# Eric-qi/RDO-PTQ

Measured on AMD Instinct MI355X. Metric: calibration images/sec (Cheng2020 W8A8 task-oriented RDO-PTQ, image-iterations over all units), higher is better.
Workload: dtype f32

## Files before the change

include/rdo_ptq_hip.h:

```cpp
#ifndef RDO_PTQ_HIP_H
#define RDO_PTQ_HIP_H

#include <stdint.h>

#ifdef __cplusplus
extern "C" {
#endif

#define RDO_OK 0
#define RDO_EINVAL (-22)
#define RDO_EHIP (-5)
#define RDO_ENOMEM (-12)

#define RDO_LOG_SLOTS 32

enum {
    RDO_EPI_NONE = 0,
    RDO_EPI_LRELU = 1,
    RDO_EPI_LRELU_BWD = 2,
    RDO_EPI_GDN = 3,
    RDO_EPI_IGDN = 4,
    RDO_EPI_RELU = 5,
    RDO_EPI_RELU_BWD = 6,
    RDO_EPI_GELU = 7,
    RDO_EPI_GELU_BWD = 8
};

typedef struct rdo_conv_desc {
    int32_t B, H, W, Cin;
    int32_t Ho, Wo, Cout;
    int32_t KH, KW, stride, pad;
    int32_t epilogue;
    int32_t square_input;
    int32_t add_residual;
} rdo_conv_desc;

const char* rdo_version(void);
const char* rdo_last_error(void);
int rdo_set_tuning(const char* key, int32_t value);
int rdo_get_tuning(const char* key);

int rdo_conv2d_fwd(const rdo_conv_desc* d, const float* x, const float* w, const float* bias, const float* aux,
                   const float* residual, float* out, float* pre, float* workspace, int64_t workspace_floats,
                   const void* wplanes , void* stream);
int rdo_conv2d_fwd_ksplit(const rdo_conv_desc* d, int has_planes, int64_t workspace_floats);
int rdo_conv2d_fwd_partials(const rdo_conv_desc* d, const float* x, const float* w, const void* wplanes ,
                            float* workspace, int64_t workspace_floats, void* stream);
int rdo_conv2d_fwd_uses_bf16x6(const rdo_conv_desc* d);
int rdo_split_bf16x3_conv(const float* w, int32_t Cout, int32_t KH, int32_t KW, int32_t Cin, void* planes ,
                          void* stream);
int rdo_split_bf16x3(const float* w, int64_t n, void* planes , void* stream);
int rdo_conv2d_fwd_bf16x6(const rdo_conv_desc* d, const float* x, const void* wplanes, const float* bias, const float* aux,
                          const float* residual, float* out, float* pre, float* workspace, int64_t workspace_floats, void* stream);
int rdo_conv2d_fwd_bf16x6_ksplit(const rdo_conv_desc* d);
int64_t rdo_conv2d_fwd_workspace(const rdo_conv_desc* d);

int rdo_conv2d_wgrad_nsplit(const rdo_conv_desc* d);
int rdo_conv2d_wgrad(const rdo_conv_desc* d, const float* x, const float* dy, float* slabs, int nsplit, void* stream);
int rdo_conv2d_wgrad_uses_bf16x6(const rdo_conv_desc* d);
int rdo_reduce_slabs(const float* slabs, int nsplit, int64_t numel, float* out, void* stream);

typedef struct rdo_ada_desc {
    int64_t numel;
    int32_t rows;
    int32_t n_levels;
    int32_t reparam;
    float reparam_bound, reparam_pedestal;
    int32_t KH, KW, Cin;
} rdo_ada_desc;

int rdo_adaround_init_alpha(const rdo_ada_desc* d, const float* w, const float* delta, float* alpha, void* stream);

int rdo_adaround_fwd(const rdo_ada_desc* d, const float* w, const float* alpha, const float* delta, const float* zp,
                     int soft, float* wq, float* wd, void* stream);

typedef struct rdo_sched_row {
    float b;
    float round_on;
    float step_size;
    float bc2_sqrt;
} rdo_sched_row;

int rdo_adaround_step(const rdo_ada_desc* d, const float* w, const float* delta, const float* zp, const float* slabs,
                      int nsplit, float grad_scale, float round_weight, const rdo_sched_row* sched, const int32_t* iter_ptr,
                      float* alpha, float* adam_m, float* adam_v, float* wq, float* wd, float* round_loss_out,
                      void* wq_planes, void* wd_planes, float wq_plane_scale, float wd_plane_scale, void* stream);

typedef struct rdo_ada_step_item {
    rdo_ada_desc d;
    const float *w, *delta, *zp, *slabs ;
    int32_t nsplit;
    float *alpha, *adam_m, *adam_v, *wq, *wd ;
    void *wq_planes , *wd_planes ;
    float* dalpha;
    float wq_plane_scale, wd_plane_scale;
    void *lin_fwd_planes, *lin_bwd_planes;
    float lin_plane_scale;
} rdo_ada_step_item;
int rdo_adaround_step_batch(const rdo_ada_step_item* items, int32_t n, int32_t mode, float grad_scale, float round_weight,
                            const rdo_sched_row* sched, const int32_t* iter_ptr, float* round_loss_out, int32_t* advance_iter,
                            int32_t* iter_shadow ,
                            void* stream);

typedef struct rdo_gather_desc {
    const float *cache_q, *cache_fp;
    const int32_t* idx_table;
    int32_t n_iters, B, batch_offset;
    int64_t per_image;
    int32_t C;
    float prob;
    uint32_t seed;
    float* out;
    void* out_planes;
    float out_scale;
    int32_t* overflow_flag;
} rdo_gather_desc;
int rdo_adaround_step_batch_gather(const rdo_ada_step_item* items, int32_t n, int32_t mode , float grad_scale, float round_weight,
                                   const rdo_sched_row* sched, const int32_t* iter_ptr, float* round_loss_out, int32_t* iter_shadow,
                                   const rdo_gather_desc* next, void* stream);
int rdo_iter_bind_publish(int32_t* publish);

int rdo_unit1x1_supported(int64_t M, int32_t K, int32_t N);
int rdo_unit1x1_nslab(int64_t M, int32_t N);
int rdo_unit1x1_form(int32_t form);
int rdo_unit1x1(const float* x, int64_t M, int32_t K, int32_t N, const float* w, const float* bias, const float* tgt_cache,
                const int32_t* idx_table, const int32_t* iter_ptr, int32_t B, float coef, int32_t act ,
                float* slabs, int32_t nslab, float* loss_out, void* stream);

int rdo_adaround_grad(const rdo_ada_desc* d, const float* w, const float* alpha, const float* delta, const float* zp,
                      const float* slabs, int nsplit, float* dalpha, void* stream);
int rdo_adaround_apply(const rdo_ada_desc* d, const float* w, const float* delta, const float* zp, const float* dalpha,
                       float grad_scale, float round_weight, const rdo_sched_row* sched, const int32_t* iter_ptr,
                       float* alpha, float* adam_m, float* adam_v, float* wq, float* wd, float* round_loss_out,
                       void* wq_planes, void* wd_planes, float wq_plane_scale, float wd_plane_scale, void* stream);

int rdo_uaq_fakequant(const rdo_ada_desc* d, const float* w, const float* delta, const float* zp, float* wq, float* wd,
                      void* stream);
int rdo_uaq_init_minmax(const float* w, int32_t rows, int64_t inner, int32_t n_levels, float* delta, float* zp,
                        void* stream);

int rdo_actquant_perchannel(const float* x, int64_t npix, int32_t C, int32_t n_bits, float* out,
                            float* ws_minmax , void* stream);
int64_t rdo_actquant_workspace(int32_t C);
int rdo_actquant_static(const float* x, int64_t npix, int32_t C, int32_t n_bits, const float* range , float* out,
                        void* stream);
int rdo_actquant_observe(const float* ws_minmax, int32_t C, float* range , void* stream);
int rdo_actquant_search(const float* x, int64_t npix, int32_t C, int32_t n_bits, const float* range ,
                        float* err , float* ws ,
                        void* stream);
int64_t rdo_actquant_search_workspace(int32_t C);
int rdo_actquant_static_bwd(const float* x, const float* g, int64_t npix, int32_t C, int32_t n_bits, const float* range ,
                            float* dx, float* drange ,
                            float* ws , void* stream);
int64_t rdo_actquant_static_bwd_workspace(int32_t C);
int rdo_act_range_step(float* range , const float* grad , const float* obs ,
                       float* m, float* v, int32_t C, int32_t step, float lr, void* stream);

int rdo_gather_qdrop(const float* cache_q, const float* cache_fp, const int32_t* idx_table, const int32_t* iter_ptr,
                     int32_t B, int32_t batch_offset, int64_t per_image, float prob, uint32_t seed, float* out,
                     int32_t* iter_publish , void* stream);

int rdo_lp2_loss_grad(const float* pred, const float* tgt_cache, const int32_t* idx_table, const int32_t* iter_ptr,
                      int32_t B, int64_t per_image, int32_t C, float coef, float* grad, float* loss_out, void* stream);

int rdo_lp_loss_grad(const float* pred, const float* tgt_cache, const int32_t* idx_table, const int32_t* iter_ptr,
                     int32_t B, int64_t per_image, int32_t C, float coef2, float coefp, float p, float* grad,
                     float* loss_out, float* loss_out_p, void* stream);

int rdo_lrelu_fwd(const float* x, int64_t n, float* out, void* stream);
int rdo_lrelu_bwd(const float* g, const float* y, int64_t n, float* out, void* stream);
int rdo_relu_fwd(const float* x, int64_t n, float* out, void* stream);
int rdo_relu_bwd(const float* g, const float* y, int64_t n, float* out, void* stream);
int rdo_pixel_shuffle(const float* x, int32_t B, int32_t H, int32_t W, int32_t C, int32_t r, int32_t inverse, float* out,
                      void* stream);
int rdo_add(const float* a, const float* b, int64_t n, float* out, void* stream);
int rdo_gdn_bwd_t(const float* g, const float* x, const float* norm, int64_t n, int32_t inverse, float* t, void* stream);
int rdo_gdn_bwd_dx(const float* g, const float* x, const float* norm, const float* acc, int64_t n, int32_t inverse,
                   float* dx, void* stream);
int rdo_nchw_to_nhwc(const float* x, int32_t B, int32_t C, int32_t H, int32_t W, int32_t inverse, float* out, void* stream);
int rdo_iter_advance(int32_t* iter_ptr, void* stream);
int rdo_zero_insert(const float* x, int32_t B, int32_t H, int32_t W, int32_t C, int32_t stride, int32_t pad_top, int32_t pad_left,
                    int32_t Ho, int32_t Wo, float* out, void* stream);
int rdo_tconv_expand(const float* w, const int32_t* map, int32_t Cout, int32_t taps, int32_t Cin, int32_t S2, int32_t KK2, float* wphase,
                     void* stream);
int rdo_tconv_fold(const float* slabs_phase, const int32_t* inv, int32_t nsplit, int32_t Cout, int32_t taps, int32_t Cin, int32_t S2,
                   int32_t KK2, float* slabs, void* stream);
int rdo_layer_norm(const float* x, const float* weight, const float* bias, int64_t rows, int32_t C, float eps, float* out,
                   void* stream);

typedef struct rdo_attn_desc {
    int32_t B, H, W, C;
    int32_t heads;
    int32_t window;
    int32_t shift;
    float scale;
} rdo_attn_desc;
int rdo_window_attention_fwd(const rdo_attn_desc* d, const float* qkv, const float* bias, float* out, float* probs, void* stream);
int rdo_window_attention_pv(const rdo_attn_desc* d, const float* qkv, const float* probs, float* out, void* stream);
int rdo_window_attention_bwd(const rdo_attn_desc* d, const float* qkv, const float* bias, const float* dout, float* dqkv, void* stream);
int rdo_layer_norm_bwd(const float* x, const float* gamma, const float* dy, int64_t rows, int32_t C, float eps, float* dx,
                       float* dgamma_slabs, int32_t nslabs, void* stream);
int rdo_add_layer_norm(const float* a, const float* b, const float* weight, const float* bias, int64_t rows, int32_t C, float eps,
                       float* sum_out, float* out, void* stream);
int rdo_layer_norm_bwd_add(const float* x, const float* gamma, const float* dy, const float* add1, const float* add2, int64_t rows,
                           int32_t C, float eps, float* dx, float* dgamma_slabs, int32_t nslabs, void* stream);
int rdo_add3(const float* a, const float* b, const float* c, int64_t n, float* out, void* stream);
int rdo_linear_h2_supported(int64_t M, int32_t K, int32_t N);
int rdo_split_h2_linear(const float* w, int32_t N, int32_t K, float scale, void* planes, void* stream);
int rdo_linear_h2(const float* x, int64_t M, int32_t K, int32_t N, const void* wplanes, float wscale, const float* bias,
                  int32_t square_input , float* out, void* stream);
int rdo_linear_h2_epi(const float* x, int64_t M, int32_t K, int32_t N, const void* wplanes, float wscale, const float* bias,
                      int32_t square_input, int32_t epilogue, float* pre, const float* aux, float* out, void* stream);
int rdo_gelu_fwd(const float* x, int64_t n, float* out, void* stream);
int rdo_gelu_bwd(const float* dy, const float* x, int64_t n, float* dx, void* stream);
int rdo_round(const float* x, int64_t n, float* out, void* stream);

int rdo_factorized_likelihood_fwd(const float* z, const float* params, const float* medians, int64_t n, int32_t C, float* zhat,
                                  float* lik, void* stream);
int rdo_factorized_likelihood_bwd(const float* zhat, const float* params, int64_t n, int32_t C, float grad_scale, float* dz, void* stream);
int rdo_gaussian_likelihood_fwd(const float* y, const float* scales, const float* means , int64_t n,
                                float scale_bound, float* yhat , float* lik, void* stream);
int rdo_gaussian_likelihood_bwd(const float* yhat, const float* scales, const float* means, int64_t n, float scale_bound,
                                float grad_scale, float* dscales, float* dmeans, void* stream);
int rdo_neg_log2_sum(const float* lik, int64_t n, float scale, float* out , void* stream);
int rdo_sq_diff_sum(const float* a, const float* b, int64_t n, float scale, int32_t clamp01_a, float* out ,
                    void* stream);
int rdo_neg_log2_sum_ordered(const float* lik, int64_t n, float scale, float* out , float* ws, void* stream);
int rdo_sq_diff_sum_ordered(const float* a, const float* b, int64_t n, float scale, int32_t clamp01_a, float* out , float* ws,
                            void* stream);
int64_t rdo_ordered_sum_workspace(void);

int rdo_h2_overflow(int reset);
int rdo_h2_bind_flag(int32_t* flag);
int rdo_split_h2(const float* x, int64_t npix, int32_t C, float scale, void* planes , void* stream);
int rdo_split_h2_conv(const float* w, int32_t Cout, int32_t KH, int32_t KW, int32_t Cin, float scale, void* planes ,
                      void* stream);
int rdo_conv2d_fwd_h2_supported(const rdo_conv_desc* d);
int64_t rdo_conv2d_fwd_h2_workspace(const rdo_conv_desc* d);
int rdo_conv2d_fwd_h2(const rdo_conv_desc* d, const void* x_planes, float x_scale, const void* wplanes, float w_scale, const float* bias,
                      const float* aux,
                      const void* aux_planes ,
                      const float* residual, float* out, float* pre, void* out_planes, float out_scale, float* workspace,
                      int64_t workspace_floats, void* stream);
int rdo_conv2d_fwd_h2_tail_supported(const rdo_conv_desc* d);
int rdo_conv2d_fwd_h2_tail(const rdo_conv_desc* d, const void* x_planes, float x_scale, const void* wplanes, float w_scale,
                           const float* bias, const void* residual_planes , float residual_scale, const float* tgt_cache,
                           const int32_t* idx_table, const int32_t* iter_ptr, int32_t B, float coef, int32_t act, void* dpre_planes,
                           float dpre_scale, float* loss_out, void* stream);
int rdo_conv2d_wgrad_h2_supported(const rdo_conv_desc* d);
int rdo_conv2d_wgrad_h2_layer_supported(const rdo_conv_desc* d);
int rdo_conv2d_wgrad_h2(const rdo_conv_desc* d, const void* x_planes, float x_scale, const void* dy_planes, float dy_scale, float* slabs,
                        int nsplit, void* stream);
int rdo_gather_qdrop_h2(const float* cache_q, const float* cache_fp, const int32_t* idx_table, const int32_t* iter_ptr, int32_t B,
                        int32_t batch_offset, int64_t per_image, int32_t C, float prob, uint32_t seed, float* out, void* out_planes,
                        float out_scale, int32_t* iter_publish, void* stream);
int rdo_loss_act_bwd(const float* pre, const float* residual, const void* residual_planes ,
                     float residual_scale, const float* tgt_cache, const int32_t* idx_table, const int32_t* iter_ptr, int32_t B,
                     int64_t per_image, int32_t C, float coef, int32_t act, float* out, float* grad_out, float* dpre, void* dpre_planes,
                     float dpre_scale, float* loss_out, void* stream);
int rdo_loss_act_bwd_splitk(const float* partial, int32_t ksplit, const float* bias , const float* residual,
                            const float* tgt_cache, const int32_t* idx_table, const int32_t* iter_ptr, int32_t B, int64_t per_image,
                            int32_t C, float coef, int32_t act, float* out, float* grad_out, float* dpre, float* loss_out, void* stream);
int rdo_loss_gdn_bwd(const float* x, const float* norm, const float* residual, const float* tgt_cache, const int32_t* idx_table,
                     const int32_t* iter_ptr, int32_t B, int64_t per_image, int32_t C, float coef, int32_t inverse, float* out,
                     float* grad_out, float* t, void* t_planes, float t_scale, float* loss_out, void* stream);
int rdo_gdn_bwd_dx_h2(const float* g, const float* x, const float* norm, const float* acc, int64_t n, int32_t C, int32_t inverse,
                      float* dx, void* dx_planes, float dx_scale, void* stream);
int rdo_pixel_shuffle_h2(const float* x, int32_t B, int32_t H, int32_t W, int32_t C, float* out, void* out_planes, float out_scale,
                         void* stream);
int rdo_pixel_unshuffle2(const float* x, int32_t B, int32_t H, int32_t W, int32_t C, float* out, void* out_planes, float out_scale,
                         void* stream);

typedef struct rdo_plan rdo_plan;
// ... 24 lines not shown
```

rdo-ptq_amd/csrc/adaround.hip:

```cpp
#include "rdo_common.h"
#include "gather_body.h"

namespace {

typedef float f32x4 __attribute__((ext_vector_type(4)));

constexpr float kGamma = -0.1f, kZeta = 1.1f;
constexpr float kBeta1 = 0.9f, kBeta2 = 0.999f, kAdamEps = 1e-8f;

__device__ __forceinline__ float sigmoidf_(float a) { return 1.0f / (1.0f + __expf(-a)); }

__device__ __forceinline__ float pow_u(float u, float p) {
    return (u > 0.f) ? __builtin_amdgcn_exp2f(__builtin_amdgcn_logf(u) * p) : 0.f;
}

struct AdaArgs {
    rdo_ada_desc d;
    const float* w;
    const float* delta;
    const float* zp;
    const float* slabs;
    int nsplit;
    const float* dalpha_in;
    float* dalpha_out;
// ... 110 lines not shown
                s += 4;
            }
            for (; s < a.nsplit; ++s) g4 += *reinterpret_cast<const vec_t*>(sp + (long)s * d.numel);
        }
        vec_t m4 = wv4 * 0.f, v4 = m4, o4 = m4;
        if (a.mode != 1 && !ADA_ABL(8)) {
            m4 = *reinterpret_cast<const vec_t*>(a.m + e0);
            v4 = *reinterpret_cast<const vec_t*>(a.v + e0);
        }
        int rows[W];
        if (inner >= W && d.numel < (1L << 31)) {
            const unsigned row0 = (unsigned)e0 / (unsigned)inner;
            const unsigned rem0 = (unsigned)e0 - row0 * (unsigned)inner;
#pragma unroll
            for (int k = 0; k < W; ++k) rows[k] = (int)(row0 + (rem0 + k >= (unsigned)inner ? 1u : 0u));
        } else {
#pragma unroll
            for (int k = 0; k < W; ++k) rows[k] = (int)((e0 + k) / inner);
        }
#pragma unroll
        for (int k = 0; k < W; ++k) {
            const int row = rows[k];
            const float dl = a.delta[row], z = a.zp[row], wv = wv4[k];
            float al = al4[k];
            const float xf = floorf(wv / dl);
            const float sg = sigmoidf_(al);
            const float hraw = sg * (kZeta - kGamma) + kGamma;
            const float h = fminf(fmaxf(hraw, 0.f), 1.f);
            const float xint = xf + h + z;
            const float pass_h = (hraw >= 0.f && hraw <= 1.f) ? 1.f : 0.f;
            const float dh_da = pass_h * ((kZeta - kGamma) * (sg * (1.f - sg)));
            float g_alpha = g4[k];
            if (a.mode != 2) {
                float g = g4[k];
                if (d.reparam) {
                    const float q = (fminf(fmaxf(xint, 0.f), Lm1) - z) * dl;
                    const float lb = fmaxf(q, d.reparam_bound);
                    const float go = g * (2.f * lb);
                    g = (q >= d.reparam_bound || go < 0.f) ? go : 0.f;
                }
                const float pass_q = (xint >= 0.f && xint <= Lm1) ? 1.f : 0.f;
                g_alpha = (g * dl) * pass_q * dh_da;
            }
            if (a.mode == 1) {
                o4[k] = g_alpha;
                continue;
            }
            float g_total = g_alpha * a.grad_scale;
            if (round_on != 0.f && !ADA_ABL(4)) {
                const float u = fabsf(h - 0.5f) * 2.f;
                const float ub1 = pow_u(u, b - 1.f);
                rl_local += a.round_weight * (1.f - u * ub1);
                const float sgn = (h > 0.5f) ? 1.f : ((h < 0.5f) ? -1.f : 0.f);
                g_total += (-a.round_weight * (b * ub1) * 2.f * sgn) * dh_da;
            }
            float mm = m4[k], vv = v4[k];
            mm = mm + (g_total - mm) * (1.f - kBeta1);
            vv = vv * kBeta2 + (1.f - kBeta2) * g_total * g_total;
            const float denom = sqrtf(vv) / bc2 + kAdamEps;
            al = al - step_size * (mm / denom);
            m4[k] = mm; v4[k] = vv; al4[k] = al;
            const float sg2 = sigmoidf_(al);
            const float h2 = fminf(fmaxf(sg2 * (kZeta - kGamma) + kGamma, 0.f), 1.f);
            float o = (fminf(fmaxf(xf + h2 + z, 0.f), Lm1) - z) * dl;
            if (d.reparam) {
                const float lb = fmaxf(o, d.reparam_bound);
                o = lb * lb - d.reparam_pedestal;
            }
            o4[k] = o;
        }
        if (a.mode == 1) {
            *reinterpret_cast<vec_t*>(a.dalpha_out + e0) = o4;
        } else {
            if (!ADA_ABL(8)) {
                *reinterpret_cast<vec_t*>(a.m + e0) = m4;
                *reinterpret_cast<vec_t*>(a.v + e0) = v4;
            }
            *reinterpret_cast<vec_t*>(a.alpha + e0) = al4;
            if (!ADA_ABL(32)) *reinterpret_cast<vec_t*>(a.wq + e0) = o4;
            if (ADA_ABL(2)) continue;
            if (a.lin_fwd || a.lin_bwd) {
                const int in_ = (int)inner, nr = d.rows;
                const long plane = (long)nr * in_;
                int bad = 0;
#pragma unroll
                for (int k = 0; k < W; ++k) {
                    const int n = rows[k], kk = (int)(e0 + k - (long)n * in_);
                    unsigned short hi, lo;
                    lin_split(o4[k], a.lin_pscale, hi, lo, bad);
                    if (a.lin_fwd) {
                        const long f = lin_frag_index(n, kk, nr >> 4);
                        a.lin_fwd[f] = hi; a.lin_fwd[plane + f] = lo;
                    }
                    if (a.lin_bwd) {
                        const long f = lin_frag_index(kk, n, in_ >> 4);
                        a.lin_bwd[f] = hi; a.lin_bwd[plane + f] = lo;
                    }
                }
                rdo::h2_report(bad, a.ovf);
            }
            if (a.wq_planes && a.wq_pscale > 0.f) {
                int bad = 0;
                if constexpr (W == 4) {
                    typedef unsigned u32x2 __attribute__((ext_vector_type(2)));
                    u32x2 ph, pl;
                    unsigned h, l;
                    rdo::h2_split_pk(o4[0], o4[1], a.wq_pscale, h, l, bad); ph[0] = h; pl[0] = l;
                    rdo::h2_split_pk(o4[2], o4[3], a.wq_pscale, h, l, bad); ph[1] = h; pl[1] = l;
                    const long f0 = d.Cin > 0 ? rdo::frag_index(e0, d.rows, d.KH, d.KW, d.Cin) : e0;
                    *reinterpret_cast<u32x2*>(a.wq_planes + f0) = ph;
                    *reinterpret_cast<u32x2*>(a.wq_planes + d.numel + f0) = pl;
                } else {
#pragma unroll
                    for (int k = 0; k < W; ++k)
                        rdo::h2_split_store(o4[k], a.wq_pscale, a.wq_planes, d.numel,
                                            d.Cin > 0 ? rdo::frag_index(e0 + k, d.rows, d.KH, d.KW, d.Cin) : e0 + k, bad);
                }
                rdo::h2_report(bad, a.ovf);
            } else if (a.wq_planes) {
                if constexpr (W == 4) {
                    typedef unsigned short u16x4 __attribute__((ext_vector_type(4)));
                    u16x4 ph, pm, pl;
#pragma unroll
                    for (int k = 0; k < 4; ++k) {
                        const __bf16 h = (__bf16)o4[k];
                        const float r1 = o4[k] - (float)h;
                        const __bf16 m = (__bf16)r1;
                        const __bf16 l = (__bf16)(r1 - (float)m);
                        ph[k] = __builtin_bit_cast(unsigned short, h);
                        pm[k] = __builtin_bit_cast(unsigned short, m);
                        pl[k] = __builtin_bit_cast(unsigned short, l);
                    }
                    const long f0 = d.Cin > 0 ? rdo::frag_index(e0, d.rows, d.KH, d.KW, d.Cin) : e0;
                    *reinterpret_cast<u16x4*>(a.wq_planes + f0) = ph;
                    *reinterpret_cast<u16x4*>(a.wq_planes + d.numel + f0) = pm;
                    *reinterpret_cast<u16x4*>(a.wq_planes + 2 * d.numel + f0) = pl;
                } else {
#pragma unroll
                    for (int k = 0; k < W; ++k)
                        split3_store(o4[k], a.wq_planes, d.numel, d.Cin > 0 ? rdo::frag_index(e0 + k, d.rows, d.KH, d.KW, d.Cin) : e0 + k);
                }
            }
        }
    }
    if (a.mode != 1 && a.round_loss_out && round_on != 0.f) {
        const float t = rdo::block_sum(rl_local);
        if (threadIdx.x == 0) {
            if (t != 0.f) atomicAdd(a.round_loss_out + (long)it * RDO_LOG_SLOTS + (bid & (RDO_LOG_SLOTS - 1)), t);
        }
    }
}


__device__ __forceinline__ void ada_step_tile_body(const AdaArgs& a, int bid) {
    typedef float vec_t __attribute__((ext_vector_type(4)));
    typedef unsigned u32x2 __attribute__((ext_vector_type(2)));
    typedef unsigned short u16x4 __attribute__((ext_vector_type(4)));
    const rdo_ada_desc d = a.d;
    const int Cin = d.Cin, taps = d.KH * d.KW, nrows = d.rows;
    const int ctiles = (Cin + 31) >> 5;
    const int bid0 = bid;
    const int ct = bid % ctiles; bid /= ctiles;
    const int tap = bid % taps;
    const int rt = bid / taps;
    const int q = threadIdx.x & 7, r = threadIdx.x >> 3;
    const int row = rt * 32 + r, ci = ct * 32 + 4 * q;
    const bool live = row < nrows && ci < Cin;
    const float Lm1 = (float)(d.n_levels - 1);
    const int it = *a.iter_ptr;
    const rdo_sched_row sc = a.sched[it];
    const float b = sc.b, round_on = sc.round_on, step_size = sc.step_size, bc2 = sc.bc2_sqrt;
    float rl_local = 0.f;
    vec_t o4 = {0.f, 0.f, 0.f, 0.f};
    const long e0 = ((long)row * taps + tap) * Cin + ci;
    if (live) {
        const vec_t wv4 = *reinterpret_cast<const vec_t*>(a.w + e0);
        vec_t al4 = *reinterpret_cast<const vec_t*>(a.alpha + e0);
        vec_t g4 = {0.f, 0.f, 0.f, 0.f};
        if (a.mode == 2) {
            g4 = *reinterpret_cast<const vec_t*>(a.dalpha_in + e0);
        } else if (!ADA_ABL(1)) {
            const float* sp = a.slabs + e0;
            int s = 0;
            for (; s + 16 <= a.nsplit; s += 16) {
                vec_t t[16];
#pragma unroll
                for (int u = 0; u < 16; ++u) t[u] = *reinterpret_cast<const vec_t*>(sp + (long)(s + u) * d.numel);
                g4 += (((t[0] + t[1]) + (t[2] + t[3])) + ((t[4] + t[5]) + (t[6] + t[7]))) +
                      (((t[8] + t[9]) + (t[10] + t[11])) + ((t[12] + t[13]) + (t[14] + t[15])));
            }
            for (; s + 8 <= a.nsplit; s += 8) {
                vec_t t[8];
#pragma unroll
                for (int u = 0; u < 8; ++u) t[u] = *reinterpret_cast<const vec_t*>(sp + (long)(s + u) * d.numel);
                g4 += ((t[0] + t[1]) + (t[2] + t[3])) + ((t[4] + t[5]) + (t[6] + t[7]));
            }
            if (s + 4 <= a.nsplit) {
                vec_t t[4];
#pragma unroll
                for (int u = 0; u < 4; ++u) t[u] = *reinterpret_cast<const vec_t*>(sp + (long)(s + u) * d.numel);
                g4 += (t[0] + t[1]) + (t[2] + t[3]);
                s += 4;
            }
            for (; s < a.nsplit; ++s) g4 += *reinterpret_cast<const vec_t*>(sp + (long)s * d.numel);
        }
        vec_t m4 = {0.f, 0.f, 0.f, 0.f}, v4 = m4;
        if (!ADA_ABL(8)) {
            m4 = *reinterpret_cast<const vec_t*>(a.m + e0);
            v4 = *reinterpret_cast<const vec_t*>(a.v + e0);
        }
        const float dl = a.delta[row], z = a.zp[row];
#pragma unroll
        for (int k = 0; k < 4; ++k) {
            float al = al4[k];
            const float xf = floorf(wv4[k] / dl);
            const float sg = sigmoidf_(al);
            const float hraw = sg * (kZeta - kGamma) + kGamma;
            const float h = fminf(fmaxf(hraw, 0.f), 1.f);
            const float xint = xf + h + z;
            const float pass_h = (hraw >= 0.f && hraw <= 1.f) ? 1.f : 0.f;
            const float dh_da = pass_h * ((kZeta - kGamma) * (sg * (1.f - sg)));
            float g_alpha = g4[k];
            if (a.mode != 2) {
                float g = g4[k];
                if (d.reparam) {
                    const float qv = (fminf(fmaxf(xint, 0.f), Lm1) - z) * dl;
                    const float lb = fmaxf(qv, d.reparam_bound);
                    const float go = g * (2.f * lb);
                    g = (qv >= d.reparam_bound || go < 0.f) ? go : 0.f;
                }
                const float pass_q = (xint >= 0.f && xint <= Lm1) ? 1.f : 0.f;
                g_alpha = (g * dl) * pass_q * dh_da;
            }
            float g_total = g_alpha * a.grad_scale;
            if (round_on != 0.f && !ADA_ABL(4)) {
                const float u = fabsf(h - 0.5f) * 2.f;
                const float ub1 = pow_u(u, b - 1.f);
                rl_local += a.round_weight * (1.f - u * ub1);
                const float sgn = (h > 0.5f) ? 1.f : ((h < 0.5f) ? -1.f : 0.f);
                g_total += (-a.round_weight * (b * ub1) * 2.f * sgn) * dh_da;
            }
            float mm = m4[k], vv = v4[k];
            mm = mm + (g_total - mm) * (1.f - kBeta1);
            vv = vv * kBeta2 + (1.f - kBeta2) * g_total * g_total;
            const float denom = sqrtf(vv) / bc2 + kAdamEps;
            al = al - step_size * (mm / denom);
            m4[k] = mm; v4[k] = vv; al4[k] = al;
            const float sg2 = sigmoidf_(al);
            const float h2 = fminf(fmaxf(sg2 * (kZeta - kGamma) + kGamma, 0.f), 1.f);
            float o = (fminf(fmaxf(xf + h2 + z, 0.f), Lm1) - z) * dl;
            if (d.reparam) {
                const float lb = fmaxf(o, d.reparam_bound);
                o = lb * lb - d.reparam_pedestal;
            }
            o4[k] = o;
        }
        if (!ADA_ABL(8)) {
            *reinterpret_cast<vec_t*>(a.m + e0) = m4;
            *reinterpret_cast<vec_t*>(a.v + e0) = v4;
        }
        *reinterpret_cast<vec_t*>(a.alpha + e0) = al4;
        if (!ADA_ABL(32)) *reinterpret_cast<vec_t*>(a.wq + e0) = o4;
        if (!ADA_ABL(2)) {
            int bad = 0;
            if (a.lin_fwd) {
                unsigned hh, ll;
                u32x2 ph, pl;
                rdo::h2_split_pk(o4[0], o4[1], a.lin_pscale, hh, ll, bad); ph[0] = hh; pl[0] = ll;
                rdo::h2_split_pk(o4[2], o4[3], a.lin_pscale, hh, ll, bad); ph[1] = hh; pl[1] = ll;
                const long f = lin_frag_index(row, ci, nrows >> 4);
                *reinterpret_cast<u32x2*>(a.lin_fwd + f) = ph;
                *reinterpret_cast<u32x2*>(a.lin_fwd + (long)nrows * Cin + f) = pl;
            }
            if (a.wq_planes) {
                const long f0 = (Cin & 15) ? e0 : (((((long)(ci >> 4) * taps + tap) * nrows + row) << 4) + (ci & 15));
                if (a.wq_pscale > 0.f) {
                    unsigned hh, ll;
                    u32x2 ph, pl;
                    rdo::h2_split_pk(o4[0], o4[1], a.wq_pscale, hh, ll, bad); ph[0] = hh; pl[0] = ll;
                    rdo::h2_split_pk(o4[2], o4[3], a.wq_pscale, hh, ll, bad); ph[1] = hh; pl[1] = ll;
                    *reinterpret_cast<u32x2*>(a.wq_planes + f0) = ph;
                    *reinterpret_cast<u32x2*>(a.wq_planes + d.numel + f0) = pl;
                } else {
                    u16x4 ph, pm, pl;
#pragma unroll
                    for (int k = 0; k < 4; ++k) {
                        const __bf16 hb = (__bf16)o4[k];
                        const float r1 = o4[k] - (float)hb;
                        const __bf16 mb = (__bf16)r1;
                        const __bf16 lb = (__bf16)(r1 - (float)mb);
                        ph[k] = __builtin_bit_cast(unsigned short, hb);
                        pm[k] = __builtin_bit_cast(unsigned short, mb);
                        pl[k] = __builtin_bit_cast(unsigned short, lb);
                    }
                    *reinterpret_cast<u16x4*>(a.wq_planes + f0) = ph;
                    *reinterpret_cast<u16x4*>(a.wq_planes + d.numel + f0) = pm;
                    *reinterpret_cast<u16x4*>(a.wq_planes + 2 * d.numel + f0) = pl;
                }
            }
            rdo::h2_report(bad, a.ovf);
        }
    }
    __shared__ float tile[32][33];
    if ((a.wd || a.lin_bwd) && !ADA_ABL(16)) {
#pragma unroll
        for (int k = 0; k < 4; ++k) tile[r][4 * q + k] = o4[k];
        __syncthreads();
        const int ci2 = ct * 32 + r, co2 = rt * 32 + 4 * q;
        if (ci2 < Cin && co2 < nrows) {
            vec_t t4;
#pragma unroll
            for (int k = 0; k < 4; ++k) t4[k] = tile[4 * q + k][r];
            const int kh = tap / d.KW, kw = tap - kh * d.KW;
            const int tapf = (d.KH - 1 - kh) * d.KW + (d.KW - 1 - kw);
            const long o = ((long)ci2 * taps + tapf) * nrows + co2;
            if (a.wd) *reinterpret_cast<vec_t*>(a.wd + o) = t4;
            int bad = 0;
            if (a.lin_bwd && !ADA_ABL(2)) {
                unsigned hh, ll;
                u32x2 ph, pl;
                rdo::h2_split_pk(t4[0], t4[1], a.lin_pscale, hh, ll, bad); ph[0] = hh; pl[0] = ll;
                rdo::h2_split_pk(t4[2], t4[3], a.lin_pscale, hh, ll, bad); ph[1] = hh; pl[1] = ll;
                const long f = lin_frag_index(ci2, co2, Cin >> 4);
                *reinterpret_cast<u32x2*>(a.lin_bwd + f) = ph;
                *reinterpret_cast<u32x2*>(a.lin_bwd + (long)nrows * Cin + f) = pl;
            }
            if (a.wd && a.wd_planes && !ADA_ABL(2)) {
                const long f0 = (nrows & 15) ? o : (((((long)(co2 >> 4) * taps + tapf) * Cin + ci2) << 4) + (co2 & 15));
                if (a.wd_pscale > 0.f) {
                    unsigned hh, ll;
                    u32x2 ph, pl;
                    rdo::h2_split_pk(t4[0], t4[1], a.wd_pscale, hh, ll, bad); ph[0] = hh; pl[0] = ll;
                    rdo::h2_split_pk(t4[2], t4[3], a.wd_pscale, hh, ll, bad); ph[1] = hh; pl[1] = ll;
                    *reinterpret_cast<u32x2*>(a.wd_planes + f0) = ph;
                    *reinterpret_cast<u32x2*>(a.wd_planes + d.numel + f0) = pl;
                } else {
                    u16x4 ph, pm, pl;
#pragma unroll
                    for (int k = 0; k < 4; ++k) {
                        const __bf16 hb = (__bf16)t4[k];
                        const float r1 = t4[k] - (float)hb;
                        const __bf16 mb = (__bf16)r1;
                        const __bf16 lb = (__bf16)(r1 - (float)mb);
                        ph[k] = __builtin_bit_cast(unsigned short, hb);
                        pm[k] = __builtin_bit_cast(unsigned short, mb);
                        pl[k] = __builtin_bit_cast(unsigned short, lb);
                    }
                    *reinterpret_cast<u16x4*>(a.wd_planes + f0) = ph;
                    *reinterpret_cast<u16x4*>(a.wd_planes + d.numel + f0) = pm;
                    *reinterpret_cast<u16x4*>(a.wd_planes + 2 * d.numel + f0) = pl;
                }
            }
            rdo::h2_report(bad, a.ovf);
        }
    }
    if (a.round_loss_out && round_on != 0.f) {
        const float t = rdo::block_sum(rl_local);
        if (threadIdx.x == 0) {
            if (t != 0.f) atomicAdd(a.round_loss_out + (long)it * RDO_LOG_SLOTS + (bid0 & (RDO_LOG_SLOTS - 1)), t);
        }
    }
}

inline bool tile_ok(const rdo_ada_desc& d, int mode) {
    return mode != 1 && d.Cin > 0 && d.Cin % 4 == 0 && d.rows % 4 == 0 && (long)d.rows * d.KH * d.KW * d.Cin == d.numel && d.numel < (1L << 31);
}
inline long tile_blocks(const rdo_ada_desc& d) { return rdo::ceil_div(d.rows, 32) * d.KH * d.KW * rdo::ceil_div(d.Cin, 32); }

template <int W>
__global__ __launch_bounds__(256) void ada_step_kernel(AdaArgs a) {
    ada_step_body<W>(a, blockIdx.x, gridDim.x);
}

constexpr int kMaxBatch = 8;
struct AdaBatch {
    int w1_min;
    int32_t* iter_shadow;
    AdaArgs a[kMaxBatch];
    int blk_end[kMaxBatch];
    unsigned char tile[kMaxBatch];
    int n;
    int gather_beg;
    rdo::gq::Gather g;
};
__global__ __launch_bounds__(256) void ada_step_batch_kernel(AdaBatch b) {
    if (b.iter_shadow && blockIdx.x == 0 && threadIdx.x == 0) *b.iter_shadow = *b.a[0].iter_ptr + 1;
    if ((int)blockIdx.x >= b.gather_beg) {
        const int it1 = *b.a[0].iter_ptr + 1;
        if (it1 < b.g.n_iters) {
            if (b.g.planes.p) rdo::gq::gather_h2_body(b.g, it1, (long)blockIdx.x - b.gather_beg, (long)gridDim.x - b.gather_beg);
            else rdo::gq::gather_fp32_body(b.g, it1, (long)blockIdx.x - b.gather_beg, (long)gridDim.x - b.gather_beg);
        }
        return;
    }
    int t = 0;
    while (t + 1 < b.n && (int)blockIdx.x >= b.blk_end[t]) ++t;
    const int beg = t ? b.blk_end[t - 1] : 0;
    if (b.tile[t]) { ada_step_tile_body(b.a[t], (int)blockIdx.x - beg); return; }
    if (b.a[t].nsplit >= b.w1_min && b.a[t].mode != 2) ada_step_body<1>(b.a[t], (long)blockIdx.x - beg, (long)b.blk_end[t] - beg);
    else ada_step_body<4>(b.a[t], (long)blockIdx.x - beg, (long)b.blk_end[t] - beg);
}

__device__ __forceinline__ void wd_transpose_body(const rdo_ada_desc& d, const float* wq, float* wd, unsigned short* wd_planes, float pscale,
                                                  int* ovf, int bid) {
    const int taps = d.KH * d.KW, cdim = d.Cin;
    const int ctiles = (cdim + 31) / 32;
    const int ct = bid % ctiles; bid /= ctiles;
    const int tap = bid % taps;
    const int rt = bid / taps;
    const int tx = threadIdx.x & 31, ty = threadIdx.x >> 5;
    __shared__ float tile[32][33];
#pragma unroll
    for (int k = 0; k < 4; ++k) {
        const int row = rt * 32 + ty + 8 * k, c = ct * 32 + tx;
        if (row < d.rows && c < cdim) tile[ty + 8 * k][tx] = wq[((long)row * taps + tap) * cdim + c];
    }
    __syncthreads();
    const int kh = tap / d.KW, kw = tap - kh * d.KW;
    const int tapf = (d.KH - 1 - kh) * d.KW + (d.KW - 1 - kw);
#pragma unroll
    for (int k = 0; k < 4; ++k) {
        const int ci = ct * 32 + ty + 8 * k, co = rt * 32 + tx;
        if (ci < cdim && co < d.rows) {
            const long o = ((long)ci * taps + tapf) * d.rows + co;
            wd[o] = tile[tx][ty + 8 * k];
            if (wd_planes && pscale > 0.f) {
                int bad = 0;
                rdo::h2_split_store(tile[tx][ty + 8 * k], pscale, wd_planes, d.numel, rdo::frag_index(o, d.Cin, d.KH, d.KW, d.rows), bad);
                rdo::h2_report(bad, ovf);
            } else if (wd_planes) {
                split3_store(tile[tx][ty + 8 * k], wd_planes, d.numel, rdo::frag_index(o, d.Cin, d.KH, d.KW, d.rows));
            }
        }
    }
}
__global__ __launch_bounds__(256) void wd_transpose_kernel(rdo_ada_desc d, const float* wq, float* wd, unsigned short* wd_planes, float pscale,
                                                           int* ovf) {
    wd_transpose_body(d, wq, wd, wd_planes, pscale, ovf, blockIdx.x);
}
__global__ __launch_bounds__(256) void wd_transpose_batch_kernel(AdaBatch b, int32_t* advance) {
    int t = 0;
    while (t + 1 < b.n && (int)blockIdx.x >= b.blk_end[t]) ++t;
    const int beg = t ? b.blk_end[t - 1] : 0;
    if (!ADA_ABL(16)) wd_transpose_body(b.a[t].d, b.a[t].wq, b.a[t].wd, b.a[t].wd_planes, b.a[t].wd_pscale, b.a[t].ovf, (int)blockIdx.x - beg);
    if (advance && blockIdx.x == 0 && threadIdx.x == 0) *advance += 1;
}

__global__ void iter_advance1_kernel(int32_t* it) { *it += 1; }

__global__ __launch_bounds__(256) void ada_fwd_kernel(rdo_ada_desc d, const float* w, const float* alpha, const float* delta,
                                                      const float* zp, int mode , float* wq,
                                                      float* wd) {
    const long inner = d.numel / d.rows;
    const float Lm1 = (float)(d.n_levels - 1);
    for (long e = (long)blockIdx.x * blockDim.x + threadIdx.x; e < d.numel; e += (long)gridDim.x * blockDim.x) {
        const int row = (int)(e / inner);
        const float dl = delta[row], z = zp[row], wv = w[e];
        float xint;
        if (mode == 2) {
            xint = rintf(wv / dl) + z;
        } else {
            const float xf = floorf(wv / dl);
            float h;
            if (mode == 1) {
                h = fminf(fmaxf(sigmoidf_(alpha[e]) * (kZeta - kGamma) + kGamma, 0.f), 1.f);
            } else {
                h = alpha[e] >= 0.f ? 1.f : 0.f;
            }
            xint = xf + h + z;
        }
        emit(d, e, (fminf(fmaxf(xint, 0.f), Lm1) - z) * dl, wq, wd);
    }
}

__global__ __launch_bounds__(256) void ada_init_kernel(rdo_ada_desc d, const float* w, const float* delta, float* alpha) {
    const long inner = d.numel / d.rows;
    for (long e = (long)blockIdx.x * blockDim.x + threadIdx.x; e < d.numel; e += (long)gridDim.x * blockDim.x) {
        const float dl = delta[e / inner];
        const float r = w[e] / dl;
        const float rest = r - floorf(r);
        alpha[e] = -logf((kZeta - kGamma) / (rest - kGamma) - 1.f);
    }
}

__global__ __launch_bounds__(256) void uaq_minmax_kernel(const float* w, long inner, int n_levels, float* delta, float* zp) {
    const float* p = w + (long)blockIdx.x * inner;
    float mn = 0.f, mx = 0.f;
    for (long i = threadIdx.x; i < inner; i += blockDim.x) {
        const float v = p[i];
        mn = fminf(mn, v);
        mx = fmaxf(mx, v);
    }
    for (int o = 32; o > 0; o >>= 1) {
        mn = fminf(mn, __shfl_down(mn, o, 64));
        mx = fmaxf(mx, __shfl_down(mx, o, 64));
    }
    __shared__ float smn[4], smx[4];
    if ((threadIdx.x & 63) == 0) { smn[threadIdx.x >> 6] = mn; smx[threadIdx.x >> 6] = mx; }
    __syncthreads();
    if (threadIdx.x == 0) {
        mn = fminf(fminf(smn[0], smn[1]), fminf(smn[2], smn[3]));
        mx = fmaxf(fmaxf(smx[0], smx[1]), fmaxf(smx[2], smx[3]));
        float dl = (float)(((double)mx - (double)mn) / (double)(n_levels - 1));
        dl = fmaxf(dl, 1e-8f);
        delta[blockIdx.x] = dl;
        zp[blockIdx.x] = rintf(__fmul_rn(__frcp_rn(dl), -mn));
    }
}

__global__ __launch_bounds__(256) void reduce_slabs_kernel(const float* slabs, int nsplit, long numel, float* out) {
    for (long e = (long)blockIdx.x * blockDim.x + threadIdx.x; e < numel; e += (long)gridDim.x * blockDim.x) {
        float g = 0.f;
        for (int s = 0; s < nsplit; ++s) g += slabs[(long)s * numel + e];
        out[e] = g;
    }
}

using rdo::grid_for;

int check_desc(const rdo_ada_desc* d, const char* who) {
    RDO_REQUIRE(d != nullptr, "%s: null descriptor", who);
    RDO_REQUIRE(d->numel > 0 && d->rows > 0 && d->numel % d->rows == 0, "%s: numel %ld not divisible by rows %d", who,
                (long)d->numel, d->rows);
    RDO_REQUIRE(d->n_levels >= 4 && d->n_levels <= 65536, "%s: n_levels %d unsupported", who, d->n_levels);
    if (d->Cin > 0)
        RDO_REQUIRE(d->KH > 0 && d->KW > 0 && (long)d->rows * d->KH * d->KW * d->Cin == d->numel,
                    "%s: conv layout [%d][%d][%d][%d] does not match numel %ld", who, d->rows, d->KH, d->KW, d->Cin,
                    (long)d->numel);
    return RDO_OK;
}

int run_step(AdaArgs a, void* stream) {

    return rdo::dispatch(
        [a](hipStream_t s) {
            if (a.d.numel % 4 == 0)
                hipLaunchKernelGGL(ada_step_kernel<4>, dim3(grid_for(a.d.numel / 4)), dim3(256), 0, s, a);
            else
                hipLaunchKernelGGL(ada_step_kernel<1>, dim3(grid_for(a.d.numel)), dim3(256), 0, s, a);
            if (a.mode != 1 && a.wd && a.d.Cin > 0) {
                const long blocks = rdo::ceil_div(a.d.rows, 32) * a.d.KH * a.d.KW * rdo::ceil_div(a.d.Cin, 32);
                hipLaunchKernelGGL(wd_transpose_kernel, dim3((unsigned)blocks), dim3(256), 0, s, a.d, (const float*)a.wq, a.wd, a.wd_planes, a.wd_pscale,
                                   a.ovf);
            }
            return rdo::check_launch("ada_step");
        },
        stream, "ada_step", 0.0, 4.0 * a.d.numel * ((a.mode == 2 ? 1 : a.nsplit) + 9.0));
}

}

extern "C" {

#ifdef RDO_DIAG
int rdo_diag_ada_ablate(int mask) {
    return hipMemcpyToSymbol(HIP_SYMBOL(g_ada_abl), &mask, sizeof mask) == hipSuccess ? RDO_OK : rdo::set_error(RDO_EHIP, "rdo_diag_ada_ablate");
}
#endif

int rdo_adaround_init_alpha(const rdo_ada_desc* d, const float* w, const float* delta, float* alpha, void* stream) {
    if (int rc = check_desc(d, "rdo_adaround_init_alpha")) return rc;
    RDO_REQUIRE(w && delta && alpha, "rdo_adaround_init_alpha: null pointer");
    const rdo_ada_desc dd = *d;
    return rdo::dispatch(
        [=](hipStream_t s) {
            hipLaunchKernelGGL(ada_init_kernel, dim3(grid_for(dd.numel)), dim3(256), 0, s, dd, w, delta, alpha);
            return rdo::check_launch("ada_init");
        },
        stream);
}

int rdo_adaround_fwd(const rdo_ada_desc* d, const float* w, const float* alpha, const float* delta, const float* zp, int soft,
                     float* wq, float* wd, void* stream) {
    if (int rc = check_desc(d, "rdo_adaround_fwd")) return rc;
    RDO_REQUIRE(w && alpha && delta && zp && wq, "rdo_adaround_fwd: null pointer");
    const rdo_ada_desc dd = *d;
    const int mode = soft ? 1 : 0;
    return rdo::dispatch(
        [=](hipStream_t s) {
            hipLaunchKernelGGL(ada_fwd_kernel, dim3(grid_for(dd.numel)), dim3(256), 0, s, dd, w, alpha, delta, zp, mode, wq, wd);
            return rdo::check_launch("ada_fwd");
        },
        stream);
}

int rdo_uaq_fakequant(const rdo_ada_desc* d, const float* w, const float* delta, const float* zp, float* wq, float* wd,
                      void* stream) {
    if (int rc = check_desc(d, "rdo_uaq_fakequant")) return rc;
    RDO_REQUIRE(w && delta && zp && wq, "rdo_uaq_fakequant: null pointer");
    const rdo_ada_desc dd = *d;
    return rdo::dispatch(
        [=](hipStream_t s) {
            hipLaunchKernelGGL(ada_fwd_kernel, dim3(grid_for(dd.numel)), dim3(256), 0, s, dd, w, (const float*)nullptr, delta, zp,
                               2, wq, wd);
            return rdo::check_launch("uaq_fakequant");
        },
        stream);
}

int rdo_uaq_init_minmax(const float* w, int32_t rows, int64_t inner, int32_t n_levels, float* delta, float* zp, void* stream) {
    RDO_REQUIRE(w && delta && zp && rows > 0 && inner > 0 && n_levels >= 4, "rdo_uaq_init_minmax: bad argument");
    return rdo::dispatch(
        [=](hipStream_t s) {
            hipLaunchKernelGGL(uaq_minmax_kernel, dim3(rows), dim3(256), 0, s, w, (long)inner, n_levels, delta, zp);
            return rdo::check_launch("uaq_minmax");
        },
        stream);
}

int rdo_reduce_slabs(const float* slabs, int nsplit, int64_t numel, float* out, void* stream) {
    RDO_REQUIRE(slabs && out && nsplit >= 1 && numel > 0, "rdo_reduce_slabs: bad argument");
    return rdo::dispatch(
        [=](hipStream_t s) {
            hipLaunchKernelGGL(reduce_slabs_kernel, dim3(grid_for(numel)), dim3(256), 0, s, slabs, nsplit, (long)numel, out);
            return rdo::check_launch("reduce_slabs");
        },
        stream);
}

int rdo_adaround_step(const rdo_ada_desc* d, const float* w, const float* delta, const float* zp, const float* slabs, int nsplit,
                      float grad_scale, float round_weight, const rdo_sched_row* sched, const int32_t* iter_ptr, float* alpha,
                      float* adam_m, float* adam_v, float* wq, float* wd, float* round_loss_out, void* wq_planes, void* wd_planes,
                      float wq_plane_scale, float wd_plane_scale, void* stream) {
    if (int rc = check_desc(d, "rdo_adaround_step")) return rc;
    RDO_REQUIRE(w && delta && zp && slabs && nsplit >= 1 && sched && iter_ptr && alpha && adam_m && adam_v && wq,
                "rdo_adaround_step: null pointer");
    AdaArgs a{};
    a.d = *d; a.w = w; a.delta = delta; a.zp = zp; a.slabs = slabs; a.nsplit = nsplit; a.grad_scale = grad_scale;
    a.round_weight = round_weight; a.sched = sched; a.iter_ptr = iter_ptr; a.alpha = alpha; a.m = adam_m; a.v = adam_v;
    a.wq = wq; a.wd = wd; a.round_loss_out = round_loss_out; a.mode = 0;
    a.wq_planes = static_cast<unsigned short*>(wq_planes);
    a.wd_planes = wd ? static_cast<unsigned short*>(wd_planes) : nullptr;
    a.wq_pscale = wq_plane_scale; a.wd_pscale = wd_plane_scale; a.ovf = rdo::h2_overflow_flag();
    return run_step(a, stream);
}

static int step_batch_impl(const rdo_ada_step_item* items, int32_t n, int32_t mode, float grad_scale, float round_weight,
                           const rdo_sched_row* sched, const int32_t* iter_ptr, float* round_loss_out, int32_t* advance_iter,
                           int32_t* iter_shadow, const rdo_gather_desc* next, void* stream) {
    RDO_REQUIRE(items && n >= 1 && n <= kMaxBatch, "rdo_adaround_step_batch: bad argument (1 <= n <= %d)", kMaxBatch);
    RDO_REQUIRE(mode >= 0 && mode <= 2, "rdo_adaround_step_batch: mode %d (0 fused step, 1 gradient only, 2 apply)", mode);
    RDO_REQUIRE(mode == 1 || (sched && iter_ptr), "rdo_adaround_step_batch: schedule / iteration counter missing");
    RDO_REQUIRE(!(advance_iter && iter_shadow), "rdo_adaround_step_batch: advance_iter and iter_shadow are alternatives");
    RDO_REQUIRE(!iter_shadow || iter_ptr, "rdo_adaround_step_batch: iter_shadow needs iter_ptr");
    AdaBatch b{}, bw{};
    const int w1_min = rdo::tuning(rdo::T_ADA_W1_MIN);
    b.w1_min = bw.w1_min = w1_min;
    int blocks = 0, wblocks = 0;
    double bytes = 0.0;
    for (int i = 0; i < n; ++i) {
        const rdo_ada_step_item& it = items[i];
        if (int rc = check_desc(&it.d, "rdo_adaround_step_batch")) return rc;
        RDO_REQUIRE(it.d.numel % 4 == 0, "rdo_adaround_step_batch: numel %ld of item %d is not a multiple of 4", (long)it.d.numel, i);
        RDO_REQUIRE(it.w && it.delta && it.zp && it.alpha, "rdo_adaround_step_batch: null pointer in item %d", i);
        RDO_REQUIRE(mode == 2 || (it.slabs && it.nsplit >= 1), "rdo_adaround_step_batch: item %d has no gradient slabs", i);
        RDO_REQUIRE(mode == 0 || it.dalpha, "rdo_adaround_step_batch: item %d has no dalpha buffer", i);
        RDO_REQUIRE(mode == 1 || (it.adam_m && it.adam_v && it.wq), "rdo_adaround_step_batch: null optimiser state in item %d", i);
        AdaArgs& a = b.a[i];
        a.d = it.d; a.w = it.w; a.delta = it.delta; a.zp = it.zp; a.slabs = it.slabs; a.nsplit = it.nsplit;
        a.dalpha_in = it.dalpha; a.dalpha_out = it.dalpha;
        a.grad_scale = grad_scale; a.round_weight = round_weight; a.sched = sched; a.iter_ptr = iter_ptr;
        a.alpha = it.alpha; a.m = it.adam_m; a.v = it.adam_v; a.wq = it.wq; a.wd = it.wd; a.round_loss_out = round_loss_out; a.mode = mode;
        a.wq_planes = static_cast<unsigned short*>(it.wq_planes);
        a.wd_planes = it.wd ? static_cast<unsigned short*>(it.wd_planes) : nullptr;
        a.wq_pscale = it.wq_plane_scale; a.wd_pscale = it.wd_plane_scale; a.ovf = rdo::h2_overflow_flag();
        if (mode != 1 && (it.lin_fwd_planes || it.lin_bwd_planes)) {
            RDO_REQUIRE(it.d.rows % 32 == 0 && (it.d.numel / it.d.rows) % 32 == 0 && it.lin_plane_scale > 0.f,
                        "rdo_adaround_step_batch: item %d: Linear planes need rows and inner in blocks of 32 and a positive scale", i);
            a.lin_fwd = static_cast<unsigned short*>(it.lin_fwd_planes);
            a.lin_bwd = static_cast<unsigned short*>(it.lin_bwd_planes);
            a.lin_pscale = it.lin_plane_scale;
        }
        b.tile[i] = tile_ok(it.d, mode) ? 1 : 0;
        blocks += b.tile[i] ? (int)tile_blocks(it.d) : (int)grid_for((it.nsplit >= w1_min && mode != 2) ? it.d.numel : it.d.numel / 4);
        b.blk_end[i] = blocks;
        bytes += 4.0 * it.d.numel * ((mode == 2 ? 1 : it.nsplit) + (mode == 1 ? 3.0 : 9.0));
        if (mode != 1 && it.wd && it.d.Cin > 0 && !b.tile[i]) {
            bw.a[bw.n] = a;
            wblocks += (int)(rdo::ceil_div(it.d.rows, 32) * it.d.KH * it.d.KW * rdo::ceil_div(it.d.Cin, 32));
            bw.blk_end[bw.n++] = wblocks;
        }
    }
    b.n = n;
    b.iter_shadow = iter_shadow;
    b.gather_beg = blocks;
    if (next) {
        RDO_REQUIRE(mode != 1 && iter_ptr, "rdo_adaround_step_batch_gather: the gather rides on a fused step or an apply launch");
        RDO_REQUIRE(next->cache_q && next->cache_fp && next->idx_table && (next->out || next->out_planes) && next->n_iters > 0,
                    "rdo_adaround_step_batch_gather: null pointer in the gather descriptor");
        RDO_REQUIRE(next->B > 0 && next->batch_offset >= 0 && next->per_image > 0 && next->per_image % 4 == 0 &&
                    (long)(next->batch_offset + next->B) * next->per_image < (1L << 32), "rdo_adaround_step_batch_gather: bad gather shape");
        RDO_REQUIRE(!next->out_planes || (next->C > 0 && next->C % 16 == 0 && next->per_image % next->C == 0 && next->out_scale > 0.f),
                    "rdo_adaround_step_batch_gather: the plane form needs C %% 16 == 0 and a positive power-of-two scale");
        RDO_REQUIRE(next->out_planes || next->out, "rdo_adaround_step_batch_gather: no destination");
        RDO_REQUIRE(next->prob >= 0.f && next->prob <= 1.f, "rdo_adaround_step_batch_gather: prob out of [0,1]");
        const double t = floor((double)next->prob * 4294967296.0);
        const unsigned long long thr = (unsigned long long)(t > 4294967296.0 ? 4294967296.0 : t);
        b.g = rdo::gq::Gather{next->cache_q, next->cache_fp, next->idx_table, next->n_iters, next->B, next->batch_offset, (long)next->per_image,
                              next->C, thr, next->seed, next->out,
                              rdo::gq::H2Out{static_cast<unsigned short*>(next->out_planes), next->out_scale,
                                             next->overflow_flag ? reinterpret_cast<int*>(next->overflow_flag) : rdo::h2_overflow_flag()}};
        long gb = rdo::gq::gather_blocks(b.g);
        const long cap = b.g.planes.p ? 8192 : 2048;
        blocks += (int)(gb > cap ? cap : gb);
        bytes += (8.0 + (next->out ? 4.0 : 0.0) + (next->out_planes ? 4.0 : 0.0)) * next->B * (double)next->per_image;
    }
    const char* tag = next ? "ada_step_gather" : "ada_step";
    return rdo::dispatch(
        [=](hipStream_t s) {
            hipLaunchKernelGGL(ada_step_batch_kernel, dim3((unsigned)blocks), dim3(256), 0, s, b);
            if (bw.n > 0)
                hipLaunchKernelGGL(wd_transpose_batch_kernel, dim3((unsigned)wblocks), dim3(256), 0, s, bw, advance_iter);
            else if (advance_iter)
                hipLaunchKernelGGL(iter_advance1_kernel, dim3(1), dim3(1), 0, s, advance_iter);
            return rdo::check_launch("ada_step_batch");
        },
        stream, tag, 0.0, bytes);
}

int rdo_adaround_step_batch(const rdo_ada_step_item* items, int32_t n, int32_t mode, float grad_scale, float round_weight,
                            const rdo_sched_row* sched, const int32_t* iter_ptr, float* round_loss_out, int32_t* advance_iter,
                            int32_t* iter_shadow, void* stream) {
    return step_batch_impl(items, n, mode, grad_scale, round_weight, sched, iter_ptr, round_loss_out, advance_iter, iter_shadow, nullptr, stream);
}

int rdo_adaround_step_batch_gather(const rdo_ada_step_item* items, int32_t n, int32_t mode, float grad_scale, float round_weight,
                                   const rdo_sched_row* sched, const int32_t* iter_ptr, float* round_loss_out, int32_t* iter_shadow,
                                   const rdo_gather_desc* next, void* stream) {
    RDO_REQUIRE(next != nullptr, "rdo_adaround_step_batch_gather: null gather descriptor");
    return step_batch_impl(items, n, mode, grad_scale, round_weight, sched, iter_ptr, round_loss_out, nullptr, iter_shadow, next, stream);
}

int rdo_adaround_grad(const rdo_ada_desc* d, const float* w, const float* alpha, const float* delta, const float* zp,
                      const float* slabs, int nsplit, float* dalpha, void* stream) {
    if (int rc = check_desc(d, "rdo_adaround_grad")) return rc;
    RDO_REQUIRE(w && alpha && delta && zp && slabs && nsplit >= 1 && dalpha, "rdo_adaround_grad: null pointer");
    AdaArgs a{};
    a.d = *d; a.w = w; a.delta = delta; a.zp = zp; a.slabs = slabs; a.nsplit = nsplit; a.alpha = const_cast<float*>(alpha);
    a.dalpha_out = dalpha; a.mode = 1;
    return run_step(a, stream);
}

int rdo_adaround_apply(const rdo_ada_desc* d, const float* w, const float* delta, const float* zp, const float* dalpha,
                       float grad_scale, float round_weight, const rdo_sched_row* sched, const int32_t* iter_ptr, float* alpha,
                       float* adam_m, float* adam_v, float* wq, float* wd, float* round_loss_out, void* wq_planes, void* wd_planes,
                       float wq_plane_scale, float wd_plane_scale, void* stream) {
    if (int rc = check_desc(d, "rdo_adaround_apply")) return rc;
    RDO_REQUIRE(w && delta && zp && dalpha && sched && iter_ptr && alpha && adam_m && adam_v && wq,
                "rdo_adaround_apply: null pointer");
    AdaArgs a{};
    a.d = *d; a.w = w; a.delta = delta; a.zp = zp; a.dalpha_in = dalpha; a.grad_scale = grad_scale;
    a.round_weight = round_weight; a.sched = sched; a.iter_ptr = iter_ptr; a.alpha = alpha; a.m = adam_m; a.v = adam_v;
    a.wq = wq; a.wd = wd; a.round_loss_out = round_loss_out; a.mode = 2;
    a.wq_planes = static_cast<unsigned short*>(wq_planes);
    a.wd_planes = wd ? static_cast<unsigned short*>(wd_planes) : nullptr;
    a.wq_pscale = wq_plane_scale; a.wd_pscale = wd_plane_scale; a.ovf = rdo::h2_overflow_flag();
    return run_step(a, stream);
}

}
```

rdo-ptq_amd/csrc/conv_wgrad.hip:

```cpp
#include <utility>

#include "rdo_common.h"

namespace {

typedef float f32x16 __attribute__((ext_vector_type(16)));
typedef float f32x4 __attribute__((ext_vector_type(4)));

constexpr int PK = 32;

struct WgArgs {
    const float* x;
    const float* dy;
    float* slabs;
    int B, H, W, Cin, Ho, Wo, Cout, KH, KW, stride, pad;
    int M, mchunk, nsplit;
    int tiles_co, tiles_ci;
    int square_input;
};

template <int TCO, int TCI, bool VEC>
__global__ __launch_bounds__(256) void conv_wgrad_kernel(WgArgs a) {
    constexpr int WCO = TCO / 2, WCI = TCI / 2;
    constexpr int TM = WCO / 32, TN = WCI / 32;
// ... 84 lines not shown
            if (a.square_input) v = v * v;
            *reinterpret_cast<f32x4*>(Xs + buf * PK * TCI + srow * TCI + 4 * (sq + 8 * (j - YQ))) = v;
        }
    };
    auto for_each_quad = [&](auto&& f) {
        [&]<int... J>(std::integer_sequence<int, J...>) { (f(std::integral_constant<int, J>{}), ...); }
        (std::make_integer_sequence<int, NQ>{});
    };

    if (nsteps > 0) {
        decode(0);
        for_each_quad([&](auto jc) { load_quad(jc); });
        for_each_quad([&](auto jc) { store_quad(jc, 0); });
        decode(nsteps > 1 ? 1 : 0);
        for_each_quad([&](auto jc) { load_quad(jc); });
    }
    __syncthreads();

    for (int s = 0; s < nsteps; ++s) {
        const int buf = s & 1;
        const float* Y = Ys + buf * PK * TCO;
        const float* X = Xs + buf * PK * TCI;
        float fa[2][TM], fb[2][TN];
        auto read_frags = [&](int kk, int set) {
            const int prow = 2 * kk + lh;
#pragma unroll
            for (int i = 0; i < TM; ++i) fa[set][i] = Y[prow * TCO + wco0 + i * 32 + li];
#pragma unroll
            for (int j = 0; j < TN; ++j) fb[set][j] = X[prow * TCI + wci0 + j * 32 + li];
        };
        read_frags(0, 0);
        decode(s + 2 < nsteps ? s + 2 : nsteps - 1);
        [&]<int... SL>(std::integer_sequence<int, SL...>) {
            (([&] {
                 if constexpr (SL + 1 < PK / 2) read_frags(SL + 1, (SL + 1) & 1);
#pragma unroll
                 for (int i = 0; i < TM; ++i)
#pragma unroll
                     for (int j = 0; j < TN; ++j)
                         acc[i][j] = __builtin_amdgcn_mfma_f32_32x32x2f32(fa[SL & 1][i], fb[SL & 1][j], acc[i][j], 0, 0, 0);
                 if constexpr (SL < NQ) {
                     store_quad(std::integral_constant<int, SL>{}, buf ^ 1);
                     load_quad(std::integral_constant<int, SL>{});
                 }
                 __builtin_amdgcn_sched_barrier(0);
             }()),
             ...);
        }
        (std::make_integer_sequence<int, PK / 2>{});
        __syncthreads();
    }

    const long wsize = (long)a.Cout * a.KH * a.KW * a.Cin;
    float* slab = a.slabs + (long)chunk * wsize;
    const int taps = a.KH * a.KW;
#pragma unroll
    for (int j = 0; j < TN; ++j) {
        const int ci = ci0 + wci0 + j * 32 + li;
        if (ci >= a.Cin) continue;
#pragma unroll
        for (int i = 0; i < TM; ++i)
#pragma unroll
            for (int r = 0; r < 16; ++r) {
                const int co = co0 + wco0 + i * 32 + (r & 3) + 8 * (r >> 2) + 4 * lh;
                if (co < a.Cout) slab[((long)co * taps + tap) * a.Cin + ci] = acc[i][j][r];
            }
    }
}

template <int TCO, int TCI, bool VEC>
int launch(WgArgs a, hipStream_t s) {
    constexpr size_t lds = (size_t)2 * PK * (TCO + TCI) * sizeof(float);
    auto kern = conv_wgrad_kernel<TCO, TCI, VEC>;
    static rdo::PerDevice attr_set;
    if (!attr_set.done()) {
        if (hipFuncSetAttribute(reinterpret_cast<const void*>(kern), hipFuncAttributeMaxDynamicSharedMemorySize, (int)lds) !=
            hipSuccess)
            return rdo::set_error(RDO_EHIP, "hipFuncSetAttribute(conv_wgrad, %zu B LDS) failed", lds);
        attr_set.mark();
    }
    a.tiles_co = (int)rdo::ceil_div(a.Cout, TCO);
    a.tiles_ci = (int)rdo::ceil_div(a.Cin, TCI);
    dim3 grid((unsigned)a.nsplit, (unsigned)(a.KH * a.KW * a.tiles_co * a.tiles_ci));
    hipLaunchKernelGGL(kern, grid, dim3(256), lds, s, a);
    return rdo::check_launch("conv_wgrad");
}

int g_force_big = -1, g_force_ns = -1;

inline bool one_tile_many_pixels(const rdo_conv_desc* d) {
    return d->KH == 1 && d->KW == 1 && d->Cout >= 160 && d->Cout <= 192 && d->Cin >= 160 && d->Cin <= 192 &&
           (long)d->B * d->Ho * d->Wo >= 16384;
}

inline bool big_tiles(const rdo_conv_desc* d) {
    if (g_force_big >= 0) return g_force_big != 0;
    const long M = (long)d->B * d->Ho * d->Wo;
    const long big_tiles_total = (long)d->KH * d->KW * rdo::ceil_div(d->Cout, 192) * rdo::ceil_div(d->Cin, 192);
    const long min_m = big_tiles_total >= 32 ? 1024 : 4096;
    if (d->Cout >= 160 && d->Cin >= 160 && M >= min_m && big_tiles_total >= 3) return true;
    if (d->Cout >= 160 && d->Cin >= 160 && M >= 16384 && big_tiles_total == 2) return true;
    return one_tile_many_pixels(d);
}

inline int tiles_total(const rdo_conv_desc* d) {
    const int t = big_tiles(d) ? 192 : 64;
    return d->KH * d->KW * (int)rdo::ceil_div(d->Cout, t) * (int)rdo::ceil_div(d->Cin, t);
}

}

int rdo_launch_wgrad_x6(const rdo_conv_desc* d, const float* x, const float* dy, float* slabs, int nsplit, int mchunk, hipStream_t s);
bool rdo_linear_wgrad_h2_ok(const rdo_conv_desc* d, const float* x, const float* dy);
int rdo_launch_linear_wgrad_h2(const rdo_conv_desc* d, const float* x, const float* dy, float* slabs, int nsplit, int mchunk, hipStream_t s);
bool rdo_conv_is_thin(const rdo_conv_desc* d, bool forward);
int rdo_launch_thin_wgrad(const rdo_conv_desc* d, const float* x, const float* dy, float* slabs, int nsplit, hipStream_t s);
bool rdo_conv_is_thincout(const rdo_conv_desc* d, bool forward);
int rdo_thincout_patches(const rdo_conv_desc* d);
int rdo_launch_thincout_wgrad(const rdo_conv_desc* d, const float* x, const float* dy, float* slabs, hipStream_t s);

extern "C" int rdo_conv2d_wgrad_uses_bf16x6(const rdo_conv_desc* d) {
    const bool enabled = rdo::tuning(rdo::T_CONV_X6) != 0;
    if (!d || !enabled || g_force_big == 0) return 0;
    const bool fits = (double)d->B * d->H * d->W * d->Cin * 4.0 < 4.0e9 && (double)d->B * d->Ho * d->Wo * d->Cout * 4.0 < 4.0e9;
    return big_tiles(d) && fits && d->Wo % 4 == 0 && d->Wo >= 16 && d->Cin % 4 == 0 && d->Cout % 4 == 0;
}

extern "C" void rdo_debug_force_wgrad_choice(int big, int nsplit) {
    g_force_big = big;
    g_force_ns = nsplit;
}

extern "C" int rdo_conv2d_wgrad_nsplit(const rdo_conv_desc* d) {
    if (!d) return 1;
    if (g_force_big < 0 && rdo_conv_is_thincout(d, false)) return rdo_thincout_patches(d);
    if (g_force_ns >= 1) return g_force_ns;
    const long M = (long)d->B * d->Ho * d->Wo;
    if (rdo_conv_is_thin(d, false)) {
        const long per = d->KH * d->KW * d->Cin > 4 ? 256 : 512;
        const long cap = d->KH * d->KW * d->Cin > 4 ? 256 : 128;
        const long ns = M / per;
        return (int)(ns < 1 ? 1 : (ns > cap ? cap : ns));
    }
    const long target = big_tiles(d) ? 256 : 1024;
    long ns = target / tiles_total(d);
    const long max_by_m = rdo::ceil_div(M, 128);
    if (ns > max_by_m) ns = max_by_m;
    if (ns < 1) ns = 1;
    const long cap = (g_force_big < 0 && one_tile_many_pixels(d)) ? 256 : ((g_force_big != 0 && rdo_linear_wgrad_h2_ok(d, nullptr, nullptr)) ? 128 : 64);
    if (ns > cap) ns = cap;
    return (int)ns;
}

extern "C" int rdo_conv2d_wgrad(const rdo_conv_desc* d, const float* x, const float* dy, float* slabs, int nsplit,
                                void* stream) {
    RDO_REQUIRE(d && x && dy && slabs, "rdo_conv2d_wgrad: null argument");
    RDO_REQUIRE(nsplit >= 1, "rdo_conv2d_wgrad: nsplit < 1");
    RDO_REQUIRE((long)d->B * d->H * d->W * d->Cin < (1L << 31) && (long)d->B * d->Ho * d->Wo * d->Cout < (1L << 31),
                "rdo_conv2d_wgrad: tensors of 2^31 or more elements are not supported (32-bit staging offsets)");
    WgArgs a;
    a.x = x; a.dy = dy; a.slabs = slabs;
    a.B = d->B; a.H = d->H; a.W = d->W; a.Cin = d->Cin; a.Ho = d->Ho; a.Wo = d->Wo; a.Cout = d->Cout;
    a.KH = d->KH; a.KW = d->KW; a.stride = d->stride; a.pad = d->pad;
    a.M = d->B * d->Ho * d->Wo;
    a.nsplit = nsplit;
    a.mchunk = (int)(rdo::ceil_div(rdo::ceil_div(a.M, nsplit), PK) * PK);
    a.square_input = d->square_input;
    a.tiles_co = a.tiles_ci = 0;
    const bool vec = (d->Cin % 4 == 0) && (d->Cout % 4 == 0) &&
                     ((reinterpret_cast<uintptr_t>(x) | reinterpret_cast<uintptr_t>(dy)) % 16 == 0);
    const bool big = big_tiles(d);
    if (g_force_big < 0 && rdo_conv_is_thincout(d, false) && nsplit == rdo_thincout_patches(d)) {
        const rdo_conv_desc dd = *d;
        return rdo::dispatch([=](hipStream_t s) { return rdo_launch_thincout_wgrad(&dd, x, dy, slabs, s); }, stream, "conv_thincout_wgrad",
                             2.0 * a.M * (double)a.Cout * a.Cin * 9.0,
                             4.0 * ((double)a.B * a.H * a.W * a.Cin + (double)a.M * a.Cout + (double)nsplit * a.Cout * 9.0 * a.Cin));
    }
    if (rdo_conv_is_thin(d, false)) {
        const rdo_conv_desc dd = *d;
        return rdo::dispatch([=](hipStream_t s) { return rdo_launch_thin_wgrad(&dd, x, dy, slabs, nsplit, s); }, stream,
                             "conv_thin_wgrad", 2.0 * a.M * (double)a.Cout * a.Cin * a.KH * a.KW,
                             4.0 * ((double)a.B * a.H * a.W * a.Cin + (double)a.M * a.Cout + (double)nsplit * a.Cout * a.KH * a.KW * a.Cin));
    }
    if (g_force_big != 0 && rdo_linear_wgrad_h2_ok(d, x, dy) && (long)nsplit * a.mchunk >= a.M) {
        const rdo_conv_desc dd = *d;
        const int mchunk = a.mchunk;
        return rdo::dispatch([=](hipStream_t s) { return rdo_launch_linear_wgrad_h2(&dd, x, dy, slabs, nsplit, mchunk, s); }, stream,
                             "linear_wgrad_h2", 2.0 * a.M * (double)a.Cout * a.Cin,
                             4.0 * ((double)a.M * a.Cin + (double)a.M * a.Cout + (double)nsplit * a.Cout * a.Cin));
    }
    if (vec && rdo_conv2d_wgrad_uses_bf16x6(d)) {
        const rdo_conv_desc dd = *d;
        const int mchunk = a.mchunk;
        return rdo::dispatch([=](hipStream_t s) { return rdo_launch_wgrad_x6(&dd, x, dy, slabs, nsplit, mchunk, s); }, stream,
                             "conv_wgrad_x6_192x192", 2.0 * a.M * (double)a.Cout * a.Cin * a.KH * a.KW,
                             4.0 * ((double)a.B * a.H * a.W * a.Cin + (double)a.M * a.Cout + (double)nsplit * a.Cout * a.KH * a.KW * a.Cin));
    }
    return rdo::dispatch(
        [a, vec, big](hipStream_t s) {
            if (big) return vec ? launch<192, 192, true>(a, s) : launch<192, 192, false>(a, s);
            return vec ? launch<64, 64, true>(a, s) : launch<64, 64, false>(a, s);
        },
        stream, big ? "conv_wgrad_192x192" : "conv_wgrad_64x64", 2.0 * a.M * (double)a.Cout * a.Cin * a.KH * a.KW,
        4.0 * ((double)a.B * a.H * a.W * a.Cin + (double)a.M * a.Cout + (double)nsplit * a.Cout * a.KH * a.KW * a.Cin));
}
```

rdo-ptq_amd/hipops/_lib.py:

```python
import ctypes as C
import os

_HERE = os.path.dirname(os.path.abspath(__file__))
LIB_PATH = os.path.join(os.path.dirname(_HERE), "lib", "librdoptq_hip.so")

EPI_NONE, EPI_LRELU, EPI_LRELU_BWD, EPI_GDN, EPI_IGDN, EPI_RELU, EPI_RELU_BWD, EPI_GELU, EPI_GELU_BWD = range(9)
LOG_SLOTS = 32


class ConvDesc(C.Structure):
    _fields_ = [(n, C.c_int32) for n in ("B", "H", "W", "Cin", "Ho", "Wo", "Cout", "KH", "KW", "stride", "pad", "epilogue",
                                         "square_input", "add_residual")]


class AdaDesc(C.Structure):
    _fields_ = [("numel", C.c_int64), ("rows", C.c_int32), ("n_levels", C.c_int32), ("reparam", C.c_int32),
                ("reparam_bound", C.c_float), ("reparam_pedestal", C.c_float), ("KH", C.c_int32), ("KW", C.c_int32),
                ("Cin", C.c_int32)]


class AdaStepItem(C.Structure):
    _fields_ = [("d", AdaDesc), ("w", C.c_void_p), ("delta", C.c_void_p), ("zp", C.c_void_p), ("slabs", C.c_void_p),
                ("nsplit", C.c_int32), ("alpha", C.c_void_p), ("adam_m", C.c_void_p), ("adam_v", C.c_void_p), ("wq", C.c_void_p),
                ("wd", C.c_void_p), ("wq_planes", C.c_void_p), ("wd_planes", C.c_void_p), ("dalpha", C.c_void_p),
                ("wq_plane_scale", C.c_float), ("wd_plane_scale", C.c_float),
                ("lin_fwd_planes", C.c_void_p), ("lin_bwd_planes", C.c_void_p), ("lin_plane_scale", C.c_float)]


class GatherDesc(C.Structure):
    _fields_ = [("cache_q", C.c_void_p), ("cache_fp", C.c_void_p), ("idx_table", C.c_void_p), ("n_iters", C.c_int32), ("B", C.c_int32),
                ("batch_offset", C.c_int32), ("per_image", C.c_int64), ("C", C.c_int32), ("prob", C.c_float), ("seed", C.c_uint32),
                ("out", C.c_void_p), ("out_planes", C.c_void_p), ("out_scale", C.c_float), ("overflow_flag", C.c_void_p)]


class AttnDesc(C.Structure):
    _fields_ = [(n, C.c_int32) for n in ("B", "H", "W", "C", "heads", "window", "shift")] + [("scale", C.c_float)]


class SchedRow(C.Structure):
    _fields_ = [("b", C.c_float), ("round_on", C.c_float), ("step_size", C.c_float), ("bc2_sqrt", C.c_float)]


P = C.c_void_p
_SIGS = {
    "rdo_version": (C.c_char_p, []),
    "rdo_last_error": (C.c_char_p, []),
    "rdo_set_tuning": (C.c_int, [C.c_char_p, C.c_int32]),
    "rdo_get_tuning": (C.c_int, [C.c_char_p]),
    "rdo_conv2d_fwd": (C.c_int, [C.POINTER(ConvDesc), P, P, P, P, P, P, P, P, C.c_int64, P, P]),
    "rdo_conv2d_fwd_uses_bf16x6": (C.c_int, [C.POINTER(ConvDesc)]),
    "rdo_split_bf16x3": (C.c_int, [P, C.c_int64, P, P]),
    "rdo_split_bf16x3_conv": (C.c_int, [P, C.c_int32, C.c_int32, C.c_int32, C.c_int32, P, P]),
    "rdo_conv2d_fwd_bf16x6": (C.c_int, [C.POINTER(ConvDesc), P, P, P, P, P, P, P, P, C.c_int64, P]),
    "rdo_conv2d_fwd_bf16x6_ksplit": (C.c_int, [C.POINTER(ConvDesc)]),
    "rdo_conv2d_fwd_workspace": (C.c_int64, [C.POINTER(ConvDesc)]),
    "rdo_conv2d_wgrad_nsplit": (C.c_int, [C.POINTER(ConvDesc)]),
    "rdo_conv2d_wgrad": (C.c_int, [C.POINTER(ConvDesc), P, P, P, C.c_int, P]),
    "rdo_conv2d_wgrad_uses_bf16x6": (C.c_int, [C.POINTER(ConvDesc)]),
    "rdo_reduce_slabs": (C.c_int, [P, C.c_int, C.c_int64, P, P]),
    "rdo_adaround_init_alpha": (C.c_int, [C.POINTER(AdaDesc), P, P, P, P]),
    "rdo_adaround_fwd": (C.c_int, [C.POINTER(AdaDesc), P, P, P, P, C.c_int, P, P, P]),
    "rdo_adaround_step": (C.c_int, [C.POINTER(AdaDesc), P, P, P, P, C.c_int, C.c_float, C.c_float, P, P, P, P, P, P, P, P, P, P, C.c_float, C.c_float, P]),
    "rdo_adaround_step_batch": (C.c_int, [C.POINTER(AdaStepItem), C.c_int32, C.c_int32, C.c_float, C.c_float, P, P, P, P, P, P]),
    "rdo_adaround_step_batch_gather": (C.c_int, [C.POINTER(AdaStepItem), C.c_int32, C.c_int32, C.c_float, C.c_float, P, P, P, P, C.POINTER(GatherDesc), P]),
    "rdo_iter_bind_publish": (C.c_int, [P]),
    "rdo_unit1x1_supported": (C.c_int, [C.c_int64, C.c_int32, C.c_int32]),
    "rdo_unit1x1_nslab": (C.c_int, [C.c_int64, C.c_int32]),
    "rdo_unit1x1_form": (C.c_int, [C.c_int32]),
    "rdo_unit1x1": (C.c_int, [P, C.c_int64, C.c_int32, C.c_int32, P, P, P, P, P, C.c_int32, C.c_float, C.c_int32, P, C.c_int32, P, P]),
    "rdo_adaround_grad": (C.c_int, [C.POINTER(AdaDesc), P, P, P, P, P, C.c_int, P, P]),
    "rdo_adaround_apply": (C.c_int, [C.POINTER(AdaDesc), P, P, P, P, C.c_float, C.c_float, P, P, P, P, P, P, P, P, P, P, C.c_float, C.c_float, P]),
    "rdo_uaq_fakequant": (C.c_int, [C.POINTER(AdaDesc), P, P, P, P, P, P]),
    "rdo_uaq_init_minmax": (C.c_int, [P, C.c_int32, C.c_int64, C.c_int32, P, P, P]),
    "rdo_actquant_perchannel": (C.c_int, [P, C.c_int64, C.c_int32, C.c_int32, P, P, P]),
    "rdo_actquant_workspace": (C.c_int64, [C.c_int32]),
    "rdo_actquant_static": (C.c_int, [P, C.c_int64, C.c_int32, C.c_int32, P, P, P]),
    "rdo_actquant_observe": (C.c_int, [P, C.c_int32, P, P]),
    "rdo_actquant_search": (C.c_int, [P, C.c_int64, C.c_int32, C.c_int32, P, P, P, P]),
    "rdo_actquant_search_workspace": (C.c_int64, [C.c_int32]),
    "rdo_actquant_static_bwd": (C.c_int, [P, P, C.c_int64, C.c_int32, C.c_int32, P, P, P, P, P]),
    "rdo_actquant_static_bwd_workspace": (C.c_int64, [C.c_int32]),
    "rdo_act_range_step": (C.c_int, [P, P, P, P, P, C.c_int32, C.c_int32, C.c_float, P]),
    "rdo_gather_qdrop": (C.c_int, [P, P, P, P, C.c_int32, C.c_int32, C.c_int64, C.c_float, C.c_uint32, P, P, P]),
    "rdo_lp2_loss_grad": (C.c_int, [P, P, P, P, C.c_int32, C.c_int64, C.c_int32, C.c_float, P, P, P]),
    "rdo_lp_loss_grad": (C.c_int, [P, P, P, P, C.c_int32, C.c_int64, C.c_int32, C.c_float, C.c_float, C.c_float, P, P, P, P]),
    "rdo_lrelu_fwd": (C.c_int, [P, C.c_int64, P, P]),
    "rdo_lrelu_bwd": (C.c_int, [P, P, C.c_int64, P, P]),
    "rdo_relu_fwd": (C.c_int, [P, C.c_int64, P, P]),
    "rdo_window_attention_fwd": (C.c_int, [C.POINTER(AttnDesc), P, P, P, P, P]),
    "rdo_window_attention_pv": (C.c_int, [C.POINTER(AttnDesc), P, P, P, P]),
    "rdo_window_attention_bwd": (C.c_int, [C.POINTER(AttnDesc), P, P, P, P, P]),
    "rdo_layer_norm_bwd": (C.c_int, [P, P, P, C.c_int64, C.c_int32, C.c_float, P, P, C.c_int32, P]),
    "rdo_add_layer_norm": (C.c_int, [P, P, P, P, C.c_int64, C.c_int32, C.c_float, P, P, P]),
    "rdo_layer_norm_bwd_add": (C.c_int, [P, P, P, P, P, C.c_int64, C.c_int32, C.c_float, P, P, C.c_int32, P]),
    "rdo_add3": (C.c_int, [P, P, P, C.c_int64, P, P]),
    "rdo_linear_h2_supported": (C.c_int, [C.c_int64, C.c_int32, C.c_int32]),
    "rdo_split_h2_linear": (C.c_int, [P, C.c_int32, C.c_int32, C.c_float, P, P]),
    "rdo_linear_h2": (C.c_int, [P, C.c_int64, C.c_int32, C.c_int32, P, C.c_float, P, C.c_int32, P, P]),
    "rdo_linear_h2_epi": (C.c_int, [P, C.c_int64, C.c_int32, C.c_int32, P, C.c_float, P, C.c_int32, C.c_int32, P, P, P, P]),
    "rdo_gelu_fwd": (C.c_int, [P, C.c_int64, P, P]),
    "rdo_gelu_bwd": (C.c_int, [P, P, C.c_int64, P, P]),
    "rdo_round": (C.c_int, [P, C.c_int64, P, P]),
    "rdo_ssim_level": (C.c_int, [P, P, C.c_int32, C.c_int32, C.c_int32, C.POINTER(C.c_float), C.c_float, C.c_float, P, P, P]),
    "rdo_avg_pool2": (C.c_int, [P, C.c_int32, C.c_int32, C.c_int32, P, P]),
    "rdo_ssim_level_bwd": (C.c_int, [P, P, C.c_int32, C.c_int32, C.c_int32, C.POINTER(C.c_float), C.c_float, C.c_float, P, P, P, P]),
    "rdo_avg_pool2_bwd": (C.c_int, [P, C.c_int32, C.c_int32, C.c_int32, P, P]),
    "rdo_relu_bwd": (C.c_int, [P, P, C.c_int64, P, P]),
    "rdo_pixel_shuffle": (C.c_int, [P, C.c_int32, C.c_int32, C.c_int32, C.c_int32, C.c_int32, C.c_int32, P, P]),
    "rdo_add": (C.c_int, [P, P, C.c_int64, P, P]),
    "rdo_gdn_bwd_t": (C.c_int, [P, P, P, C.c_int64, C.c_int32, P, P]),
    "rdo_gdn_bwd_dx": (C.c_int, [P, P, P, P, C.c_int64, C.c_int32, P, P]),
    "rdo_nchw_to_nhwc": (C.c_int, [P, C.c_int32, C.c_int32, C.c_int32, C.c_int32, C.c_int32, P, P]),
    "rdo_iter_advance": (C.c_int, [P, P]),
    "rdo_zero_insert": (C.c_int, [P] + [C.c_int32] * 9 + [P, P]),
    "rdo_tconv_expand": (C.c_int, [P, P, C.c_int32, C.c_int32, C.c_int32, C.c_int32, C.c_int32, P, P]),
    "rdo_tconv_fold": (C.c_int, [P, P, C.c_int32, C.c_int32, C.c_int32, C.c_int32, C.c_int32, C.c_int32, P, P]),
    "rdo_layer_norm": (C.c_int, [P, P, P, C.c_int64, C.c_int32, C.c_float, P, P]),
    "rdo_factorized_likelihood_fwd": (C.c_int, [P, P, P, C.c_int64, C.c_int32, P, P, P]),
    "rdo_factorized_likelihood_bwd": (C.c_int, [P, P, C.c_int64, C.c_int32, C.c_float, P, P]),
    "rdo_gaussian_likelihood_fwd": (C.c_int, [P, P, P, C.c_int64, C.c_float, P, P, P]),
    "rdo_gaussian_likelihood_bwd": (C.c_int, [P, P, P, C.c_int64, C.c_float, C.c_float, P, P, P]),
    "rdo_neg_log2_sum": (C.c_int, [P, C.c_int64, C.c_float, P, P]),
    "rdo_sq_diff_sum": (C.c_int, [P, P, C.c_int64, C.c_float, C.c_int32, P, P]),
    "rdo_neg_log2_sum_ordered": (C.c_int, [P, C.c_int64, C.c_float, P, P, P]),
    "rdo_sq_diff_sum_ordered": (C.c_int, [P, P, C.c_int64, C.c_float, C.c_int32, P, P, P]),
    "rdo_ordered_sum_workspace": (C.c_int64, []),
    "rdo_h2_overflow": (C.c_int, [C.c_int]),
    "rdo_h2_bind_flag": (C.c_int, [C.c_void_p]),
    "rdo_split_h2": (C.c_int, [P, C.c_int64, C.c_int32, C.c_float, P, P]),
    "rdo_split_h2_conv": (C.c_int, [P, C.c_int32, C.c_int32, C.c_int32, C.c_int32, C.c_float, P, P]),
    "rdo_conv2d_fwd_h2_workspace": (C.c_int64, [C.POINTER(ConvDesc)]),
    "rdo_conv2d_fwd_h2_supported": (C.c_int, [C.POINTER(ConvDesc)]),
    "rdo_conv2d_fwd_h2": (C.c_int, [C.POINTER(ConvDesc), P, C.c_float, P, C.c_float, P, P, P, P, P, P, P, C.c_float, P, C.c_int64, P]),
    "rdo_conv2d_wgrad_h2_supported": (C.c_int, [C.POINTER(ConvDesc)]),
    "rdo_conv2d_wgrad_h2_layer_supported": (C.c_int, [C.POINTER(ConvDesc)]),
    "rdo_conv2d_wgrad_h2": (C.c_int, [C.POINTER(ConvDesc), P, C.c_float, P, C.c_float, P, C.c_int, P]),
    "rdo_conv2d_fwd_h2_tail_supported": (C.c_int, [C.POINTER(ConvDesc)]),
    "rdo_conv2d_fwd_h2_tail": (C.c_int, [C.POINTER(ConvDesc), P, C.c_float, P, C.c_float, P, P, C.c_float, P, P, P, C.c_int32, C.c_float, C.c_int32, P,
                                         C.c_float, P, P]),
    "rdo_conv2d_fwd_ksplit": (C.c_int, [C.POINTER(ConvDesc), C.c_int, C.c_int64]),
    "rdo_conv2d_fwd_partials": (C.c_int, [C.POINTER(ConvDesc), P, P, P, P, C.c_int64, P]),
    "rdo_loss_act_bwd_splitk": (C.c_int, [P, C.c_int32, P, P, P, P, P, C.c_int32, C.c_int64, C.c_int32, C.c_float, C.c_int32, P, P, P, P, P]),
    "rdo_gather_qdrop_h2": (C.c_int, [P, P, P, P, C.c_int32, C.c_int32, C.c_int64, C.c_int32, C.c_float, C.c_uint32, P, P, C.c_float, P, P]),
    "rdo_loss_act_bwd": (C.c_int, [P, P, P, C.c_float, P, P, P, C.c_int32, C.c_int64, C.c_int32, C.c_float, C.c_int32, P, P, P, P, C.c_float, P, P]),
    "rdo_loss_gdn_bwd": (C.c_int, [P, P, P, P, P, P, C.c_int32, C.c_int64, C.c_int32, C.c_float, C.c_int32, P, P, P, P, C.c_float, P, P]),
    "rdo_gdn_bwd_dx_h2": (C.c_int, [P, P, P, P, C.c_int64, C.c_int32, C.c_int32, P, P, C.c_float, P]),
    "rdo_pixel_shuffle_h2": (C.c_int, [P, C.c_int32, C.c_int32, C.c_int32, C.c_int32, P, P, C.c_float, P]),
    "rdo_pixel_unshuffle2": (C.c_int, [P, C.c_int32, C.c_int32, C.c_int32, C.c_int32, P, P, C.c_float, P]),
    "rdo_plan_create": (P, []),
    "rdo_plan_destroy": (None, [P]),
    "rdo_plan_begin_record": (C.c_int, [P]),
    "rdo_plan_end_record": (C.c_int, [P]),
    "rdo_plan_suspend_record": (C.c_int, [C.c_int]),
    "rdo_plan_num_ops": (C.c_int, [P]),
    "rdo_plan_run": (C.c_int, [P, C.c_int, C.c_int, P]),
    "rdo_plan_prepare": (C.c_int, [P, C.c_int]),
    "rdo_plan_run_then": (C.c_int, [P, P, C.c_int, P]),
    "rdo_plan_op_info": (C.c_int, [P, C.c_int, C.POINTER(C.c_char_p), C.POINTER(C.c_double), C.POINTER(C.c_double)]),
    "rdo_plan_profile": (C.c_int, [P, C.POINTER(C.c_float), P]),
}
EXPORTS = tuple(_SIGS)

_lib = None


def lib():
    global _lib
    if _lib is None:
        if not os.path.exists(LIB_PATH):
            raise RuntimeError(f"{LIB_PATH} not found: build it with `python __graft_entry__.py` or "
                               f"`make -C rdo-ptq_amd/csrc` (no CPU fallback exists)")
        import torch
        h = C.CDLL(LIB_PATH)
        for name, (res, args) in _SIGS.items():
            fn = getattr(h, name)
            fn.restype, fn.argtypes = res, args
        _lib = h
    return _lib


def check(rc, what=""):
    if rc != 0:
        raise RuntimeError(f"librdoptq_hip {what} failed ({rc}): {lib().rdo_last_error().decode()}")
```

rdo-ptq_amd/hipops/ops.py:

```python
import ctypes as C
import math
import threading

import torch

from . import _lib as L


class H2:
    __slots__ = ("t", "scale", "flag")

    def __init__(self, t, scale, flag=None):
        self.t, self.scale = t, float(scale)
        self.flag = flag
        m, e = math.frexp(self.scale)
        if not (self.scale > 0 and m == 0.5):
            raise ValueError(f"H2 scale must be a positive power of two, got {scale}")

    @property
    def device(self):
        return self.t.device


def _ptr(t):
# ... 50 lines not shown
    co, kh, kw, ci = w.shape
    L.check(L.lib().rdo_split_bf16x3_conv(_ptr(w), co, kh, kw, ci, _ptr(planes), _stream()), "rdo_split_bf16x3_conv")
    return planes


def split_bf16x3_linear(w, planes=None):
    planes = torch.empty((3,) + tuple(w.shape), device=w.device, dtype=torch.int16) if planes is None else planes
    L.check(L.lib().rdo_split_bf16x3(_ptr(w), w.numel(), _ptr(planes), _stream()), "rdo_split_bf16x3")
    return planes


def conv2d_fwd(x, w, bias=None, stride=1, pad=0, epilogue=L.EPI_NONE, aux=None, residual=None, square_input=False,
               out=None, pre=None, wplanes=None):
    d = conv_desc(x.shape, w.shape, stride, pad, epilogue, square_input, residual is not None)
    if out is None:
        out = torch.empty((d.B, d.Ho, d.Wo, d.Cout), device=x.device, dtype=torch.float32)
    need = int(L.lib().rdo_conv2d_fwd_workspace(C.byref(d)))
    ws = _scratch(x.device, need) if need else None
    L.check(L.lib().rdo_conv2d_fwd(C.byref(d), _ptr(x), _ptr(w), _ptr(bias), _ptr(aux), _ptr(residual), _ptr(out), _ptr(pre),
                                   _ptr(ws), ws.numel() if ws is not None else 0, _ptr(wplanes), _stream()), "rdo_conv2d_fwd")
    return out


SCRATCH_FLOATS = 1 << 22


def conv_fwd_ksplit(x_shape, w_shape, stride, pad, has_planes, device):
    d = conv_desc(x_shape, w_shape, stride, pad)
    need = int(L.lib().rdo_conv2d_fwd_workspace(C.byref(d)))
    return int(L.lib().rdo_conv2d_fwd_ksplit(C.byref(d), int(bool(has_planes)), max(need, SCRATCH_FLOATS))), need


def conv2d_fwd_partials(x, w, stride=1, pad=0, wplanes=None):
    d = conv_desc(x.shape, w.shape, stride, pad)
    ks, need = conv_fwd_ksplit(tuple(x.shape), tuple(w.shape), stride, pad, wplanes is not None, x.device)
    ws = _scratch(x.device, need)
    L.check(L.lib().rdo_conv2d_fwd_partials(C.byref(d), _ptr(x), _ptr(w), _ptr(wplanes), _ptr(ws), ws.numel(), _stream()),
            "rdo_conv2d_fwd_partials")
    return ws, ks


def loss_act_bwd_splitk(partial, ksplit, bias, out_shape, residual, tgt_cache, idx_table, iter_ptr, coef, act, loss_log, out=None, grad_out=None,
                        dpre=None):
    B = out_shape[0]
    per_image = 1
    for v in out_shape[1:]:
        per_image *= int(v)
    L.check(L.lib().rdo_loss_act_bwd_splitk(_ptr(partial), int(ksplit), _ptr(bias), _ptr(residual), _ptr(tgt_cache), _ptr(idx_table),
                                            _ptr(iter_ptr), B, per_image, int(out_shape[-1]), coef, int(act), _ptr(out), _ptr(grad_out),
                                            _ptr(dpre), _ptr(loss_log), _stream()), "rdo_loss_act_bwd_splitk")


def wgrad_nsplit(x_shape, w_shape, stride, pad):
    d = conv_desc(x_shape, w_shape, stride, pad)
    return int(L.lib().rdo_conv2d_wgrad_nsplit(C.byref(d)))


def wgrad_uses_bf16x6(x_shape, w_shape, stride, pad):
    d = conv_desc(x_shape, w_shape, stride, pad)
    return bool(L.lib().rdo_conv2d_wgrad_uses_bf16x6(C.byref(d)))


def conv2d_wgrad(x, dy, w_shape, stride=1, pad=0, square_input=False, slabs=None):
    d = conv_desc(x.shape, w_shape, stride, pad, square_input=square_input)
    ns = int(L.lib().rdo_conv2d_wgrad_nsplit(C.byref(d))) if slabs is None else slabs.shape[0]
    if slabs is None:
        slabs = torch.empty((ns,) + tuple(w_shape), device=x.device, dtype=torch.float32)
    L.check(L.lib().rdo_conv2d_wgrad(C.byref(d), _ptr(x), _ptr(dy), _ptr(slabs), ns, _stream()), "rdo_conv2d_wgrad")
    return slabs


def reduce_slabs(slabs, out=None):
    ns = slabs.shape[0]
    numel = slabs[0].numel()
    if out is None:
        out = torch.empty(slabs.shape[1:], device=slabs.device, dtype=torch.float32)
    L.check(L.lib().rdo_reduce_slabs(_ptr(slabs), ns, numel, _ptr(out), _stream()), "rdo_reduce_slabs")
    return out


def ada_desc(w, n_levels=256, reparam=None, conv_layout=True):
    if w.dim() == 4:
        rows, KH, KW, Cin = w.shape
    else:
        rows, Cin = w.shape
        KH = KW = 1
    if not conv_layout:
        KH = KW = Cin = 0
    bound, ped = (reparam if reparam is not None else (0.0, 0.0))
    return L.AdaDesc(w.numel(), rows, n_levels, int(reparam is not None), bound, ped, KH, KW, Cin)


def adaround_init_alpha(d, w, delta, alpha=None):
    alpha = torch.empty_like(w) if alpha is None else alpha
    L.check(L.lib().rdo_adaround_init_alpha(C.byref(d), _ptr(w), _ptr(delta), _ptr(alpha), _stream()), "rdo_adaround_init_alpha")
    return alpha


def adaround_fwd(d, w, alpha, delta, zp, soft, wq=None, wd=None):
    wq = torch.empty_like(w) if wq is None else wq
    L.check(L.lib().rdo_adaround_fwd(C.byref(d), _ptr(w), _ptr(alpha), _ptr(delta), _ptr(zp), int(soft), _ptr(wq), _ptr(wd),
                                     _stream()), "rdo_adaround_fwd")
    return wq


def uaq_fakequant(d, w, delta, zp, wq=None, wd=None):
    wq = torch.empty_like(w) if wq is None else wq
    L.check(L.lib().rdo_uaq_fakequant(C.byref(d), _ptr(w), _ptr(delta), _ptr(zp), _ptr(wq), _ptr(wd), _stream()),
            "rdo_uaq_fakequant")
    return wq


def uaq_init_minmax(w, n_levels):
    rows = w.shape[0]
    delta = torch.empty(rows, device=w.device, dtype=torch.float32)
    zp = torch.empty_like(delta)
    L.check(L.lib().rdo_uaq_init_minmax(_ptr(w), rows, w.numel() // rows, n_levels, _ptr(delta), _ptr(zp), _stream()),
            "rdo_uaq_init_minmax")
    return delta, zp


def adaround_step(d, w, delta, zp, slabs, grad_scale, round_weight, sched, iter_ptr, alpha, m, v, wq, wd, round_log,
                  wq_planes=None, wd_planes=None):
    _bind_out(None)
    L.check(L.lib().rdo_adaround_step(C.byref(d), _ptr(w), _ptr(delta), _ptr(zp), _ptr(slabs), slabs.shape[0], grad_scale,
                                      round_weight, _ptr(sched), _ptr(iter_ptr), _ptr(alpha), _ptr(m), _ptr(v), _ptr(wq),
                                      _ptr(wd), _ptr(round_log), _ptr(wq_planes), _ptr(wd_planes), _pscale(wq_planes), _pscale(wd_planes),
                                      _stream()), "rdo_adaround_step")


def unit1x1_supported(M, K, N):
    return bool(L.lib().rdo_unit1x1_supported(int(M), int(K), int(N)))


def unit1x1_nslab(M, N):
    return int(L.lib().rdo_unit1x1_nslab(int(M), int(N)))


def unit1x1_form(form):
    return int(L.lib().rdo_unit1x1_form(int(form)))


def unit1x1(x, w, bias, tgt_cache, idx_table, iter_ptr, coef, act, loss_log, slabs):
    K, N = int(x.shape[-1]), int(w.shape[0])
    M = x.numel() // K
    L.check(L.lib().rdo_unit1x1(_ptr(x), M, K, N, _ptr(w), _ptr(bias), _ptr(tgt_cache), _ptr(idx_table), _ptr(iter_ptr), int(x.shape[0]),
                                float(coef), int(act), _ptr(slabs), int(slabs.shape[0]), _ptr(loss_log), _stream()), "rdo_unit1x1")


def iter_bind_publish(word):
    return bool(L.lib().rdo_iter_bind_publish(_ptr(word)))


def adaround_step_batch(items, grad_scale, round_weight, sched, iter_ptr, round_log, advance_iter=None, mode=0, iter_shadow=None, gather=None):
    _bind_out(None)
    arr = (L.AdaStepItem * len(items))()
    dp = lambda t: None if t is None else _ptr(t).value
    for k, it in enumerate(items):
        a = arr[k]
        a.d = it["d"]
        a.w, a.delta, a.zp, a.slabs = dp(it["w"]), dp(it["delta"]), dp(it["zp"]), dp(it["slabs"])
        a.nsplit = it["slabs"].shape[0] if it.get("slabs") is not None else 0
        a.alpha, a.adam_m, a.adam_v, a.wq, a.wd = dp(it["alpha"]), dp(it["m"]), dp(it["v"]), dp(it["wq"]), dp(it.get("wd"))
        a.wq_planes, a.wd_planes = dp(it.get("wq_planes")), dp(it.get("wd_planes"))
        a.wq_plane_scale, a.wd_plane_scale = _pscale(it.get("wq_planes")), _pscale(it.get("wd_planes"))
        a.dalpha = dp(it.get("dalpha"))
        lf, lb = it.get("lin_fwd"), it.get("lin_bwd")
        a.lin_fwd_planes, a.lin_bwd_planes = dp(lf), dp(lb)
        a.lin_plane_scale = float((lf if lf is not None else lb).scale) if (lf is not None or lb is not None) else 0.0
    if gather is not None:
        if advance_iter is not None:
            raise ValueError("adaround_step_batch: the gather form moves the counter by hand-over (iter_shadow), not advance_iter")
        cq, pl = gather["cache_q"], gather.get("out_planes")
        g = L.GatherDesc()
        g.cache_q, g.cache_fp, g.idx_table = dp(cq), dp(gather["cache_fp"]), dp(gather["idx_table"])
        g.n_iters, g.B, g.batch_offset = int(gather["idx_table"].shape[0]), int(gather["B"]), int(gather.get("batch_offset", 0))
        g.per_image, g.C, g.prob, g.seed = cq[0].numel(), int(cq.shape[-1]), float(gather["prob"]), int(gather["seed"])
        g.out, g.out_planes, g.out_scale = dp(gather.get("out")), dp(pl), (float(pl.scale) if pl is not None else 0.0)
        g.overflow_flag = dp(getattr(pl, "flag", None))
        L.check(L.lib().rdo_adaround_step_batch_gather(arr, len(items), int(mode), grad_scale, round_weight, _ptr(sched), _ptr(iter_ptr),
                                                       _ptr(round_log), _ptr(iter_shadow), C.byref(g), _stream()), "rdo_adaround_step_batch_gather")
        return
    L.check(L.lib().rdo_adaround_step_batch(arr, len(items), int(mode), grad_scale, round_weight, _ptr(sched), _ptr(iter_ptr), _ptr(round_log),
                                            _ptr(advance_iter), _ptr(iter_shadow), _stream()), "rdo_adaround_step_batch")


def adaround_grad(d, w, alpha, delta, zp, slabs, dalpha):
    L.check(L.lib().rdo_adaround_grad(C.byref(d), _ptr(w), _ptr(alpha), _ptr(delta), _ptr(zp), _ptr(slabs), slabs.shape[0],
                                      _ptr(dalpha), _stream()), "rdo_adaround_grad")


def adaround_apply(d, w, delta, zp, dalpha, grad_scale, round_weight, sched, iter_ptr, alpha, m, v, wq, wd, round_log,
                   wq_planes=None, wd_planes=None):
    _bind_out(None)
    L.check(L.lib().rdo_adaround_apply(C.byref(d), _ptr(w), _ptr(delta), _ptr(zp), _ptr(dalpha), grad_scale, round_weight,
                                       _ptr(sched), _ptr(iter_ptr), _ptr(alpha), _ptr(m), _ptr(v), _ptr(wq), _ptr(wd),
                                       _ptr(round_log), _ptr(wq_planes), _ptr(wd_planes), _pscale(wq_planes), _pscale(wd_planes), _stream()),
            "rdo_adaround_apply")


def set_tuning(key, value):
    prev = int(L.lib().rdo_get_tuning(key.encode()))
    L.check(L.lib().rdo_set_tuning(key.encode(), int(value)), f"rdo_set_tuning({key})")
    return prev


def actquant_perchannel(x, out=None, ws=None, n_bits=8):
    Cc = x.shape[-1]
    npix = x.numel() // Cc
    out = torch.empty_like(x) if out is None else out
    need = int(L.lib().rdo_actquant_workspace(Cc))
    if ws is None or ws.numel() < need:
        ws = torch.empty(need, device=x.device, dtype=torch.float32)
    L.check(L.lib().rdo_actquant_perchannel(_ptr(x), npix, Cc, int(n_bits), _ptr(out), _ptr(ws), _stream()), "rdo_actquant_perchannel")
    return out


ACT_SEARCH_CANDIDATES = 10


def _act_range_check(x, rng, what):
    Cc = x.shape[-1]
    if rng.numel() != 2 * Cc:
        raise ValueError(f"{what}: the range holds {rng.numel() // 2} channels, the tensor has {Cc}")
    return Cc, x.numel() // Cc


def act_range_init(channels, device):
    r = torch.empty(2 * int(channels), device=device, dtype=torch.float32)
    r[:channels] = float("inf")
    r[channels:] = float("-inf")
    return r


def actquant_observe(x, rng, out=None, n_bits=8):
    Cc, npix = _act_range_check(x, rng, "actquant_observe")
    ws = torch.empty(int(L.lib().rdo_actquant_workspace(Cc)), device=x.device, dtype=torch.float32)
    out = actquant_perchannel(x, out=out, ws=ws, n_bits=n_bits)
    L.check(L.lib().rdo_actquant_observe(_ptr(ws), Cc, _ptr(rng), _stream()), "rdo_actquant_observe")
    return out


def actquant_static(x, rng, out=None, n_bits=8):
    Cc, npix = _act_range_check(x, rng, "actquant_static")
    out = torch.empty_like(x) if out is None else out
    L.check(L.lib().rdo_actquant_static(_ptr(x), npix, Cc, int(n_bits), _ptr(rng), _ptr(out), _stream()), "rdo_actquant_static")
    return out


def actquant_search(x, rng, err, n_bits=8, ws=None):
    Cc, npix = _act_range_check(x, rng, "actquant_search")
    if tuple(err.shape) != (Cc, ACT_SEARCH_CANDIDATES):
        raise ValueError(f"actquant_search: err must be [{Cc}, {ACT_SEARCH_CANDIDATES}], got {tuple(err.shape)}")
    need = int(L.lib().rdo_actquant_search_workspace(Cc))
    if ws is None or ws.numel() < need:
        ws = torch.empty(need, device=x.device, dtype=torch.float32)
    L.check(L.lib().rdo_actquant_search(_ptr(x), npix, Cc, int(n_bits), _ptr(rng), _ptr(err), _ptr(ws), _stream()), "rdo_actquant_search")
    return err


def actquant_static_bwd(x, g, rng, drange, dx=None, n_bits=8, ws=None):
    Cc, npix = _act_range_check(x, rng, "actquant_static_bwd")
    if g.shape != x.shape or drange.numel() != 2 * Cc:
        raise ValueError(f"actquant_static_bwd: g {tuple(g.shape)} / drange [{drange.numel()}] do not match x {tuple(x.shape)}")
    dx = torch.empty_like(x) if dx is None else dx
    need = int(L.lib().rdo_actquant_static_bwd_workspace(Cc))
    if ws is None or ws.numel() < need:
        ws = torch.empty(need, device=x.device, dtype=torch.float32)
    L.check(L.lib().rdo_actquant_static_bwd(_ptr(x), _ptr(g), npix, Cc, int(n_bits), _ptr(rng), _ptr(dx), _ptr(drange), _ptr(ws), _stream()),
            "rdo_actquant_static_bwd")
    return dx


def act_range_step(rng, grad, obs, m, v, step, lr):
    n = rng.numel()
    if n % 2 or any(t.numel() != n for t in (grad, obs, m, v)):
        raise ValueError(f"act_range_step: range, grad, obs, m and v must all hold 2C = {n} floats")
    L.check(L.lib().rdo_act_range_step(_ptr(rng), _ptr(grad), _ptr(obs), _ptr(m), _ptr(v), n // 2, int(step), float(lr), _stream()),
            "rdo_act_range_step")
    return rng


def gather_qdrop(cache_q, cache_fp, idx_table, iter_ptr, B, prob, seed, out, batch_offset=0, iter_publish=None):
    per_image = cache_q[0].numel()
    L.check(L.lib().rdo_gather_qdrop(_ptr(cache_q), _ptr(cache_fp), _ptr(idx_table), _ptr(iter_ptr), B, int(batch_offset), per_image,
                                     prob, seed,
                                     _ptr(out), _ptr(iter_publish), _stream()), "rdo_gather_qdrop")
    return out


def lp2_loss_grad(pred, tgt_cache, idx_table, iter_ptr, coef, grad, loss_log):
    B = pred.shape[0]
    per_image = pred[0].numel()
    L.check(L.lib().rdo_lp2_loss_grad(_ptr(pred), _ptr(tgt_cache), _ptr(idx_table), _ptr(iter_ptr), B, per_image,
                                      pred.shape[-1], coef, _ptr(grad), _ptr(loss_log), _stream()), "rdo_lp2_loss_grad")
    return grad


def lp_loss_grad(pred, tgt_cache, idx_table, iter_ptr, coef2, coefp, p, grad, loss_log, loss_log_p=None):
    B = pred.shape[0]
    per_image = pred[0].numel()
    L.check(L.lib().rdo_lp_loss_grad(_ptr(pred), _ptr(tgt_cache), _ptr(idx_table), _ptr(iter_ptr), B, per_image,
                                     pred.shape[-1], coef2, coefp, p, _ptr(grad), _ptr(loss_log), _ptr(loss_log_p), _stream()),
            "rdo_lp_loss_grad")
    return grad


def lrelu(x, out=None):
    out = torch.empty_like(x) if out is None else out
    L.check(L.lib().rdo_lrelu_fwd(_ptr(x), x.numel(), _ptr(out), _stream()), "rdo_lrelu_fwd")
    return out


def lrelu_bwd(g, y, out=None):
    out = torch.empty_like(g) if out is None else out
    L.check(L.lib().rdo_lrelu_bwd(_ptr(g), _ptr(y), g.numel(), _ptr(out), _stream()), "rdo_lrelu_bwd")
    return out


def relu(x, out=None):
    out = torch.empty_like(x) if out is None else out
    L.check(L.lib().rdo_relu_fwd(_ptr(x), x.numel(), _ptr(out), _stream()), "rdo_relu_fwd")
    return out


def relu_bwd(g, y, out=None):
    out = torch.empty_like(g) if out is None else out
    L.check(L.lib().rdo_relu_bwd(_ptr(g), _ptr(y), g.numel(), _ptr(out), _stream()), "rdo_relu_bwd")
    return out


def add(a, b, out=None):
# ... 631 lines not shown
```

rdo-ptq_amd/quantization/engine.py:

```python
import math
import os
from collections import OrderedDict

import torch

from hipops import _lib as L
from hipops import ops
from hipops.plan import Plan

from . import dp
from .quant_layer import QuantModule
from .quantizer import AdaRoundQuantizer, from_rows, to_rows

UNIT_KINDS = ("layer", "rb", "rbws", "rbu", "rstb")


class DpStallError(RuntimeError):
    """The captured data-parallel loop stopped making progress (`UnitEngine._hb_wait`): a collective inside the graph hangs."""


class IdxStream:
    _spec = None

    @classmethod
# ... 66 lines not shown
        elif qm.kind == "tconv":
            self.w = to_rows(w, tconv=True).flip(1, 2).contiguous()
        else:
            self.w = to_rows(w)
        dev = self.w.device
        self.rows = self.w.shape[0]
        self.channel_wise = bool(wq.channel_wise)
        self.delta = wq.delta.reshape(-1).to(dev).expand(self.rows).contiguous()
        self.zp = wq.zero_point.reshape(-1).to(dev).expand(self.rows).contiguous()
        self.n_levels = wq.n_levels
        if self.is_ln:
            self.desc = ops.ada_desc(self.w, self.n_levels, conv_layout=False)
            self.stride, self.pad, self.K = 1, 0, 1
            self.w4 = tuple(self.w.shape)
            self.bias = None if qm.bias is None else qm.bias.detach().contiguous()
        elif qm.kind == "linear":
            self.stride, self.pad, self.K = 1, 0, 1
            self.desc = ops.ada_desc(self.w, self.n_levels)
            self.w4 = tuple(self.w.shape)
            self.bias = None if qm.bias is None else qm.bias.detach().contiguous()
        elif self.is_gdn:
            self.inverse = bool(qm.fwd_kwargs["inverse"])
            self.beta, reparam = qm.gdn_constants()
            self.beta = self.beta.to(dev).contiguous()
            self.desc = ops.ada_desc(self.w, self.n_levels, reparam=reparam)
            self.stride, self.pad, self.K = 1, 0, 1
            self.w4 = (self.rows, 1, 1, self.rows)
            self.bias = None
        else:
            if qm.kind == "tconv":
                kw = qm.fwd_kwargs
                if kw["groups"] != 1 or tuple(kw["dilation"]) != (1, 1):
                    raise NotImplementedError("calibration engine: grouped / dilated transposed convolutions")
                self.tconv = (int(kw["stride"][0]), int(kw["padding"][0]), int(kw["output_padding"][0]))
                self.stride, self.pad = 1, 0
            else:
                self.stride, self.pad = qm.conv_geometry()
            self.K = self.w.shape[1]
            self.desc = ops.ada_desc(self.w, self.n_levels)
            self.w4 = tuple(self.w.shape)
            self.bias = None if qm.bias is None else qm.bias.detach().contiguous()
        lv = torch.maximum(self.zp.abs(), (self.n_levels - 1 - self.zp).abs()) * self.delta
        wb = float(lv.max())
        if self.is_gdn:
            wb = max(wb, float(self.desc.reparam_bound)) ** 2
        self.wscale = ops.pow2_scale(wb)
        self.alpha = torch.empty_like(self.w)
        self.m = torch.zeros_like(self.w)
        self.v = torch.zeros_like(self.w)
        self.wq = torch.empty_like(self.w)
        self.wd = torch.empty_like(self.w) if (need_dgrad or self.is_gdn) else None
        ops.adaround_init_alpha(self.desc, self.w, self.delta, self.alpha)
        ops.adaround_fwd(self.desc, self.w, self.alpha, self.delta, self.zp, True, self.wq, self.wd)
        self.slabs = None
        self.tc_phase = self.wp = self.wp_planes = self.wp_h2 = self.slabs_p = self.bias_p = None
        if self.tconv is not None:
            s_, p_, op_ = self.tconv
            self.tc_phase = ops.TconvPhase.get(self.K, s_, p_, op_, True, dev) if os.environ.get("RDO_TCONV_PHASE", "1") != "0" else None
            if self.tc_phase is not None:
                self.wp4 = self.tc_phase.w_shape(self.rows, self.w4[3])
                self.wp = torch.empty(self.wp4, device=dev, dtype=torch.float32)
                self.bias_p = None if self.bias is None else self.bias.repeat_interleave(self.tc_phase.S2).contiguous()
                self.expand_phase()
        self.wq_planes = self.wd_planes = None
        self.lin_fwd = self.lin_bwd = None

    def lin_planes(self, fwd: bool):
        if self.qm.kind not in ("linear", "gdn") and not (self.qm.kind == "conv" and self.K == 1):
            raise RuntimeError("lin_planes: a Linear, a 1x1 conv or the 1x1 pool of a GDN")
        co, _, _, ci = self.w4
        if fwd:
            if self.lin_fwd is None:
                self.lin_fwd = ops.H2(torch.empty((2, ci // 32, co // 16, 64, 8), device=self.w.device, dtype=torch.int16), self.wscale)
            return self.lin_fwd
        if self.lin_bwd is None:
            self.lin_bwd = ops.H2(torch.empty((2, co // 32, ci // 16, 64, 8), device=self.w.device, dtype=torch.int16), self.wscale)
        return self.lin_bwd

    def enable_planes(self, fwd: bool, dgrad: bool, h2: bool = False):
        def alloc(like, cur):
            if cur is not None:
                if isinstance(cur, ops.H2) != h2:
                    raise RuntimeError(f"calibration engine: op '{self.name}' needs its weight planes in two formats")
                return cur
            if h2:
                return ops.H2(torch.empty((2,) + tuple(like.shape), device=like.device, dtype=torch.int16), self.wscale)
            return torch.empty((3,) + tuple(like.shape), device=like.device, dtype=torch.int16)
        if fwd:
            self.wq_planes = alloc(self.wq, self.wq_planes)
        if dgrad and self.wd is not None:
            self.wd_planes = alloc(self.wd, self.wd_planes)

    def expand_phase(self):
        ops.tconv_expand(self.wq4(), self.tc_phase, out=self.wp)
        if self.wp_planes is not None:
            ops.split_bf16x3(self.wp, self.wp_planes)
        if self.wp_h2 is not None:
            ops.split_h2_conv(self.wp, planes=self.wp_h2)

    def refresh_planes(self):
        if self.lin_fwd is not None:
            ops.split_h2_linear(self.wq4(), planes=self.lin_fwd)
        if self.lin_bwd is not None:
            ops.split_h2_linear(self.wd4(), planes=self.lin_bwd)
        if self.wp_planes is not None:
            ops.split_bf16x3(self.wp, self.wp_planes)
        if self.wp_h2 is not None:
            ops.split_h2_conv(self.wp, planes=self.wp_h2)
        for planes, w4 in ((self.wq_planes, self.wq4), (self.wd_planes, self.wd4)):
            if isinstance(planes, ops.H2):
                ops.split_h2_conv(w4(), planes=planes)
            elif planes is not None:
                ops.split_bf16x3(w4(), planes)

    def wq4(self):
        return self.wq.reshape(self.w4)

    def wd4(self):
        co, kh, kw, ci = self.w4
        return self.wd.reshape(ci, kh, kw, co)

    def numel(self):
        return self.w.numel()


class UnitEngine:
    def __init__(self, kind, modules, cache_q, cache_fp, cache_out, *, batch_size, iters, weight=0.01, b_range=(20, 2),
                 warmup=0.2, input_prob=0.5, lr=1e-3, seed=0, idx_table=None, include_act_func=True, group=None,
                 use_graph=True, force_dp_split=False, task_p=2.0, batch_offset=0, dp_overlap=None, fuse_tail=True, batch_step=True, use_h2=True, rd=None):
        if kind not in UNIT_KINDS:
            raise NotImplementedError(f"calibration engine: unit kind '{kind}'")
        for t in (cache_q, cache_fp, cache_out):
            if not (t.is_cuda and t.dtype == torch.float32 and t.is_contiguous() and t.dim() == 4):
                raise RuntimeError("calibration engine: caches must be contiguous fp32 NHWC CUDA tensors")
        self.kind, self.mods = kind, modules
        self.cq, self.cf, self.co = cache_q, cache_fp, cache_out
        self.B, self.iters = int(batch_size), int(iters)
        self.task_p = float(task_p)
        self.weight, self.input_prob, self.seed = float(weight), float(input_prob), int(seed) & 0xFFFFFFFF
        self.include_act = include_act_func
        self.use_graph = use_graph
        self.batch_offset = int(batch_offset)
        self.dp_overlap = None if dp_overlap is None else bool(dp_overlap)
        if os.environ.get("RDO_USE_H2") is not None:
            use_h2 = os.environ["RDO_USE_H2"] != "0"
        self.use_h2 = bool(use_h2)
        self.P = {}
        self.batch_step = bool(batch_step)
        self.fuse_splitk = os.environ.get("RDO_FUSE_SPLITK", "1") != "0"
        self.fuse_h2_tail = os.environ.get("RDO_H2_TAIL", "1") != "0"
        self.fold_iter = os.environ.get("RDO_FOLD_ITER", "1") != "0"
        self.fold_gather = os.environ.get("RDO_GATHER_IN_STEP", "1") != "0"
        self._next_gather = None
        self.rd = rd
        if rd is not None:
            metric = rd.get("metric", "mse")
            if metric not in ("mse", "ms-ssim"):
                raise ValueError(f"loss_mode='rd': unknown metric {metric!r} ('mse' or 'ms-ssim')")
            if metric == "ms-ssim" and min(rd["cali"].shape[-2:]) <= 160:
                raise ValueError(f"loss_mode='rd' with metric 'ms-ssim' needs calibration crops with both sides above 160 pixels (five "
                                 f"scales of an 11-tap window); got {tuple(rd['cali'].shape[-2:])}")
            if not include_act_func:
                raise NotImplementedError("calibration engine: loss_mode='rd' substitutes the unit's module OUTPUT (after its fused "
                                          "activation); include_act_func=False optimises the pre-activation and cannot be combined with it")
            fuse_tail = use_h2 = False
            self.use_h2 = False
        self.fuse_tail = bool(fuse_tail)
        self.dev = cache_q.device
        n = cache_q.shape[0]
        if idx_table is None and self.B > n:
            self.B = n
        if idx_table is None:
            idx_table = IdxStream.take(n, self.B, self.iters)
        idx_table = torch.as_tensor(idx_table).to(torch.int32)
        if tuple(idx_table.shape) != (self.iters, self.B):
            raise ValueError(f"idx_table must be [{self.iters},{self.B}], got {tuple(idx_table.shape)}")
        if int(idx_table.max()) >= n or int(idx_table.min()) < 0:
            raise ValueError("idx_table refers to images outside the cache")
        self.idx = idx_table.to(self.dev).contiguous()
        self.sched = ops.make_sched(self.iters, warmup, b_range, lr, self.dev)
        self._it2 = torch.zeros(2, dtype=torch.int32, device=self.dev)
        self.it, self.it_shadow = self._it2[0:1], self._it2[1:2]
        self.loss_log = torch.zeros(self.iters, L.LOG_SLOTS, device=self.dev)
        self.task_log = torch.zeros(self.iters, L.LOG_SLOTS, device=self.dev)
        self._task_is_rec = False
        self.round_log = torch.zeros(self.iters, L.LOG_SLOTS, device=self.dev)
        self.group = group
        self.world = 1
        if group is not None or (torch.distributed.is_available() and torch.distributed.is_initialized()):
            self.world = torch.distributed.get_world_size(group)
        self.split = self.world > 1 or force_dp_split
        self.dp_path = None
        self._dp_graph, self._dp_graph_failed = None, False
        self.dp_fallbacks = 0
        self._hb_dev = self._hb_host = None
        self._hb_issued = 0
        self.rd_path = None
        self._rd_graph, self._rd_graph_failed = None, False
        self._ovf = torch.zeros(2 * self.OVF_PAIRS, dtype=torch.int32, device=self.dev)
        self._ovf_slot = {}
        self.h2_restarts = 0
        self._done = 0
        self._ovf_checked = -1
        with ops.h2_flag(self._ovf[0:2]):
            self._build_ops()
            self._alloc()
            self.forms = {}
            self.scales = {}
            self._amax = {}
            self._probing = False
            self._probe_scales()
            self._record()
            for op in self.ops.values():
                op.refresh_planes()
            self._prime()

    def _build_ops(self):
        m, k = self.mods, self.kind
        o = OrderedDict()
        if k == "layer":
            o["layer"] = _Op("layer", m["layer"], False)
        elif k == "rb":
            o["conv1"] = _Op("conv1", m["conv1"], False)
            o["conv2"] = _Op("conv2", m["conv2"], True)
            if m.get("skip") is not None:
                o["skip"] = _Op("skip", m["skip"], False)
        elif k == "rbws":
            o["conv1"] = _Op("conv1", m["conv1"], False)
            o["conv2"] = _Op("conv2", m["conv2"], True)
            o["gdn"] = _Op("gdn", m["gdn"], False)
            if m.get("skip") is not None:
                o["skip"] = _Op("skip", m["skip"], False)
        elif k == "rbu":
            o["subpel_conv"] = _Op("subpel_conv", m["subpel_conv"], False)
            o["conv"] = _Op("conv", m["conv"], True)
            o["igdn"] = _Op("igdn", m["igdn"], False)
            o["upsample"] = _Op("upsample", m["upsample"], False)
        for op in o.values():
            if op.need_dgrad and (op.stride != 1 or 2 * op.pad != op.K - 1):
                raise NotImplementedError("calibration engine: dgrad is built for stride-1 'same' convolutions only")
        self.ops = o
        late = {"rb": "conv1", "rbws": "conv1", "rbu": "subpel_conv"}.get(k)
        overlap = self.dp_overlap
        if overlap is None and late is not None:
            lo = o[late]
            ho, wo = self._out_hw(lo, self.cq.shape[1], self.cq.shape[2])
            overlap = 2.0 * self.B * ho * wo * lo.numel() >= self.DP_OVERLAP_MIN_FLOP
        self._late = late if (self.split and overlap and self.rd is None) else None
        if self.split:
            self.bucket = dp.GradBucket(OrderedDict((n, op.numel()) for n, op in o.items()), late=self._late, device=self.dev, group=self.group)
            for n, op in o.items():
                op.dalpha = self.bucket.view(n)

    def _buf(self, *shape):
        return torch.empty(shape, device=self.dev, dtype=torch.float32)

    def _out_hw(self, op, H, W):
        return (H + 2 * op.pad - op.K) // op.stride + 1, (W + 2 * op.pad - op.K) // op.stride + 1

    def _alloc(self):
        B = self.B
        _, H, W, Cin = self.cq.shape
        self.x_in = self._buf(B, H, W, Cin)
        o, t = self.ops, {}
        if self.kind == "layer":
            op = o["layer"]
            if op.tc_phase is not None:
                s_ = op.tc_phase.stride
                Ho, Wo = H * s_, W * s_
                t["yp"] = self._buf(B, H, W, op.wp4[0])
                t["dyp"] = self._buf(B, H, W, op.wp4[0])
            elif op.tconv is not None:
                s_, p_, op_ = op.tconv
                q_ = op.K - 1 - p_
                if q_ < 0:
                    raise NotImplementedError("calibration engine: transposed conv with padding > kernel_size - 1")
                Hu, Wu = (H - 1) * s_ + 1 + 2 * q_ + op_, (W - 1) * s_ + 1 + 2 * q_ + op_
                t["xu"] = self._buf(B, Hu, Wu, Cin)
                self.tc_geom = (s_, q_, Hu, Wu)
                Ho, Wo = Hu - op.K + 1, Wu - op.K + 1
            elif op.is_gdn:
                Ho, Wo = H, W
                t["norm"] = self._buf(B, H, W, Cin)
                t["t"] = self._buf(B, H, W, Cin)
            else:
                Ho, Wo = self._out_hw(op, H, W)
            t["y"] = self._buf(B, Ho, Wo, op.rows)
            t["dy"] = self._buf(B, Ho, Wo, op.rows)
            t["dpre"] = self._buf(B, Ho, Wo, op.rows)
        elif self.kind == "rb":
            C = o["conv1"].rows
            for n_ in ("h1", "pre2", "out", "dout", "dpre2", "dh1"):
                t[n_] = self._buf(B, H, W, C)
            if "skip" in o:
                t["sk"] = self._buf(B, H, W, C)
        elif self.kind == "rbws":
            c1 = o["conv1"]
            Ho, Wo = self._out_hw(c1, H, W)
            C = c1.rows
            for n_ in ("h1", "c2", "norm", "out", "dout", "t", "acc", "dc2", "dh1"):
                t[n_] = self._buf(B, Ho, Wo, C)
            if "skip" in o:
                t["sk"] = self._buf(B, Ho, Wo, C)
        elif self.kind == "rbu":
            sp = o["subpel_conv"]
            C4 = sp.rows
            r = int(self.mods["upscale"])
            C = C4 // (r * r)
            t["sp"] = self._buf(B, H, W, C4)
            t["h1"] = self._buf(B, H * r, W * r, C)
            t["up"] = self._buf(B, H, W, C4)
            t["ups"] = self._buf(B, H * r, W * r, C)
            for n_ in ("c", "norm", "out", "dout", "t", "acc", "dc", "dh1"):
                t[n_] = self._buf(B, H * r, W * r, C)
            t["dsp"] = self._buf(B, H, W, C4)
            t["dup"] = self._buf(B, H, W, C4)
            self.r = r
        self.t = t
        for op in self.ops.values():
            op.slabs = None

    def _slabs(self, op, x_shape):
        ns = ops.wgrad_nsplit(tuple(x_shape), op.w4, op.stride, op.pad)
        op.slabs = self._buf(ns, *op.w4)
        return op.slabs

    lin_conv = os.environ.get("RDO_CONV1X1_LIN_H2", "1") != "0"

    def _lin_conv_ok(self, op, x):
        if not (self.lin_conv and not self._probing and op.qm.kind == "conv" and op.K == 1 and op.stride == 1 and op.pad == 0 and op.tconv is None):
            return False
        C = x.shape[-1]
        rows = math.prod(x.shape[:-1])
        return rows >= self.LIN_GDN_MIN_ROWS and ops.linear_h2_supported(rows, C, op.w4[0])

    unit1x1 = int(os.environ.get("RDO_UNIT1X1", "2"))

    def _unit1x1_ok(self, op, x):
        if not (self.unit1x1 and self.fused and self.include_act and self.kind == "layer" and op.qm.kind == "conv" and op.K == 1
                and op.stride == 1 and op.pad == 0 and op.tconv is None and not op.is_gdn):
            return False
        M, K = math.prod(x.shape[:-1]), x.shape[-1]
        return (self.unit1x1 == 2 or M <= 4096 or K <= 96) and ops.unit1x1_supported(M, K, op.w4[0])

    def _conv(self, op, x, out, epilogue=L.EPI_NONE, aux=None, residual=None, pre=None, square=False, bias=True):
        x, out = _act_of(x), _act_of(out)
        b = (op.beta if op.is_gdn else op.bias) if bias else None
        if x.planes is not None:
            op.enable_planes(True, False, h2=True)
            return ops.conv2d_fwd_h2(x.planes, x.shape, op.w4, op.wq_planes, b, op.stride, op.pad, epilogue=epilogue, aux=_f32(aux),
                                     residual=_f32(residual), out=out.f32, pre=_f32(pre), out_planes=out.planes)
        if epilogue == L.EPI_NONE and aux is None and residual is None and pre is None and not square and self._lin_conv_ok(op, x):
            return ops.linear_h2(x.f32.view(-1, x.shape[-1]), op.lin_planes(True), b, out=out.f32.view(-1, out.shape[-1]))
        if ops.uses_bf16x6(x.shape, op.w4, op.stride, op.pad):
            op.enable_planes(True, False)
        y = ops.conv2d_fwd(x.f32, op.wq4(), b, op.stride, op.pad, epilogue=epilogue, aux=_f32(aux), residual=_f32(residual),
                           square_input=square, out=out.f32, pre=_f32(pre), wplanes=op.wq_planes)
        if out.planes is not None:
            ops.split_h2(out.f32, out.planes)
        return y

    def _wgrad_into(self, slabs, x, dy, w4, stride, pad, square=False):
        x, dy = _act_of(x), _act_of(dy)
        if x.planes is not None and dy.planes is not None:
            ops.conv2d_wgrad_h2(x.planes, x.shape, dy.planes, w4, stride, pad, slabs=slabs)
        else:
            ops.conv2d_wgrad(x.f32, dy.f32, w4, stride, pad, square_input=square, slabs=slabs)

    def _wgrad(self, op, x, dy, square=False):
        if op.slabs is None:
            self._slabs(op, x.shape)
        self._wgrad_into(op.slabs, x, dy, op.w4, op.stride, op.pad, square)

    def _dgrad(self, op, dy, out, epilogue=L.EPI_NONE, aux=None):
        dy, out = _act_of(dy), _act_of(out)
        wd4, pad = tuple(op.wd4().shape), op.K - 1 - op.pad
        if dy.planes is not None:
            op.enable_planes(False, True, h2=True)
            return ops.conv2d_fwd_h2(dy.planes, dy.shape, wd4, op.wd_planes, None, 1, pad, epilogue=epilogue, aux=_f32(aux),
                                     aux_planes=_planes_only(aux), out=out.f32, out_planes=out.planes)
        if ops.uses_bf16x6(dy.shape, wd4, 1, pad):
            op.enable_planes(False, True)
        return ops.conv2d_fwd(dy.f32, op.wd4(), None, 1, pad, epilogue=epilogue, aux=_f32(aux), out=out.f32, wplanes=op.wd_planes)

    LIN_GDN_MIN_ROWS = int(os.environ.get("RDO_GDN_LIN_MIN_ROWS", 4096))
    lin_gdn = os.environ.get("RDO_GDN_LIN_H2", "1") != "0"

    def _gdn_lin_ok(self, g, x):
        C = x.shape[-1]
        rows = math.prod(x.shape[:-1])
        return (self.lin_gdn and not self._probing and rows >= self.LIN_GDN_MIN_ROWS and g.w4[0] == C and ops.linear_h2_supported(rows, C, C))

    def _gdn_pool(self, g, x, norm):
        if self._gdn_lin_ok(g, x):
            C = x.shape[-1]
            return ops.linear_h2(x.view(-1, C), g.lin_planes(True), g.beta, out=norm.view(-1, C), square_input=True)
        return self._conv(g, x, norm, square=True)

    def _gdn_acc(self, g, tbuf, acc):
        tbuf = _act_of(tbuf)
        if tbuf.planes is None and self._gdn_lin_ok(g, tbuf):
            C = tbuf.shape[-1]
            return ops.linear_h2(tbuf.f32.view(-1, C), g.lin_planes(False), None, out=acc.view(-1, C))
        return self._dgrad(g, tbuf, acc)

    def _tconv_forward(self, op, x, y, epilogue=L.EPI_NONE):
        ph, x = op.tc_phase, _act_of(x)
        if x.planes is not None:
            if op.wp_h2 is None:
                op.wp_h2 = ops.H2(torch.empty((2,) + tuple(op.wp4), device=self.dev, dtype=torch.int16), op.wscale)
            ops.conv2d_fwd_h2(x.planes, x.shape, op.wp4, op.wp_h2, op.bias_p, 1, ph.pad, epilogue=epilogue, out=self.t["yp"])
        else:
            if ops.uses_bf16x6(x.shape, op.wp4, 1, ph.pad) and op.wp_planes is None:
                op.wp_planes = torch.empty((3,) + tuple(op.wp4), device=self.dev, dtype=torch.int16)
            ops.conv2d_fwd(x.f32, op.wp, op.bias_p, 1, ph.pad, epilogue=epilogue, out=self.t["yp"], wplanes=op.wp_planes)
        self._shuffle(self.t["yp"], ph.stride, y)

    def _tconv_wgrad(self, op, x, dy):
        ph, dyp = op.tc_phase, self._act("dyp")
        self._unshuffle(dy, ph.stride, dyp)
        if op.slabs is None:
            ns = ops.wgrad_nsplit(tuple(x.shape), op.wp4, 1, ph.pad)
            op.slabs_p = self._buf(ns, *op.wp4)
            op.slabs = self._buf(ns, *op.w4)
        self._wgrad_into(op.slabs_p, x, dyp, op.wp4, 1, ph.pad)
        ops.tconv_fold(op.slabs_p, ph, op.rows, op.w4[3], out=op.slabs)

    def _after_step(self, lin_done=False):
        for op in self.ops.values():
            if op.tc_phase is not None:
                op.expand_phase()
            if lin_done:
                continue
            if op.lin_fwd is not None:
                ops.split_h2_linear(op.wq4(), planes=op.lin_fwd)
            if op.lin_bwd is not None:
                ops.split_h2_linear(op.wd4(), planes=op.lin_bwd)

    def _loss(self, pred, grad):
        if self.rd is not None:
            ops.lp2_loss_grad(pred, self.co, self.idx, self.it, 1.0, grad, self.loss_log)
            self._rd_pred = pred
            self.g_task = torch.zeros_like(pred)
            self.plan_rd = self._next_plan()
            ops.add(grad, self.g_task, out=grad)
            return
        if self.task_p == 2.0:
            self._task_is_rec = True
            ops.lp2_loss_grad(pred, self.co, self.idx, self.it, 2.0, grad, self.loss_log)
        else:
            ops.lp_loss_grad(pred, self.co, self.idx, self.it, 1.0, 1.0, self.task_p, grad, self.loss_log, self.task_log)

    @property
    def fused(self):
        return self.task_p == 2.0 and self.fuse_tail

    def _shuffle(self, x, r, out):
        out = _act_of(out)
        if out.planes is not None or (r == 2 and x.shape[-1] % 16 == 0):
            return ops.pixel_shuffle_h2(x, out=out.f32, out_planes=out.planes)
        return ops.pixel_shuffle(x, r, out.f32)

    def _unshuffle(self, x, r, out):
        x, out = _f32(x), _act_of(out)
        if out.planes is not None or (r == 2 and x.shape[-1] % 4 == 0):
            return ops.pixel_unshuffle2(x, out.f32, out_planes=out.planes)
        return ops.pixel_unshuffle(x, r, out.f32)

    def _tail_act(self, pre, res, act, dpre, gout=None):
        dpre = _act_of(dpre)
        self._task_is_rec = True
        ops.loss_act_bwd(_f32(pre), _f32(res), self.co, self.idx, self.it, 2.0, act, self.loss_log, grad_out=gout, dpre=dpre.f32, dpre_planes=dpre.planes,
                         residual_planes=_planes_only(res))

    def _conv_tail(self, op, x, pre, res, act, dpre, gout=None):
        x = _act_of(x)
        if x.planes is not None and pre is None:
            op.enable_planes(True, False, h2=True)
            self._task_is_rec = True
            ops.conv2d_fwd_h2_tail(x.planes, x.shape, op.w4, op.wq_planes, op.bias, op.stride, op.pad, res.planes, self.co, self.idx, self.it,
                                   2.0, act, dpre.planes, self.loss_log)
            return
        if x.planes is not None or self._lin_conv_ok(op, x):
            self._conv(op, x, pre)
            self._tail_act(pre, res, act, dpre, gout=gout)
            return
        x, res = x.f32, _f32(res)
        if ops.uses_bf16x6(tuple(x.shape), op.w4, op.stride, op.pad):
            op.enable_planes(True, False)
        ks, _ = ops.conv_fwd_ksplit(tuple(x.shape), op.w4, op.stride, op.pad, op.wq_planes is not None, self.dev)
        if self.fuse_splitk and ks >= 2 and not op.is_gdn and pre.shape[-1] % 4 == 0:
            ws, ks = ops.conv2d_fwd_partials(x, op.wq4(), op.stride, op.pad, wplanes=op.wq_planes)
            self._task_is_rec = True
            ops.loss_act_bwd_splitk(ws, ks, op.bias, tuple(pre.shape), res, self.co, self.idx, self.it, 2.0, act, self.loss_log,
                                    grad_out=gout, dpre=_f32(dpre))
            return
        self._conv(op, x, pre)
        self._tail_act(pre, res, act, dpre, gout=gout)

    def _tail_gdn(self, x, norm, res, inverse, gout, tbuf):
        tbuf = _act_of(tbuf)
        self._task_is_rec = True
        ops.loss_gdn_bwd(x, norm, _f32(res), self.co, self.idx, self.it, 2.0, inverse, self.loss_log, gout, t=tbuf.f32, t_planes=tbuf.planes)

    DP_OVERLAP_MIN_FLOP = 30e9
    H2_MIN_OUT = int(os.environ.get("RDO_H2_MIN_OUT", 4096 * 192))
    h2_lean = os.environ.get("RDO_H2_LEAN", "1") != "0"
    layer_h2 = os.environ.get("RDO_LAYER_H2", "1") != "0"

    OVF_PAIRS = 8

    PLANES_AS = {"dyp": "dpre"}

    def _act(self, name):
        buf = self.x_in if name == "x" else self.t[name]
        form = self.forms.get(name, F32)
        if form == ABSENT:
            return None
        planes = None
        if form & PLANES:
            pname = self.PLANES_AS.get(name, name)
            if pname not in self.P:
                k = self._ovf_slot.setdefault(pname, 1 + len(self._ovf_slot))
                self.P[pname] = ops.h2_empty(buf.shape, self.dev, self.scales[pname], flag=self._ovf[2 * k:2 * k + 2])
            planes = self.P[pname]
        return Act(name, buf.shape, buf if form & F32 else None, planes)

    def _conv_ok_h2(self, op, x_shape, dgrad=False):
        if dgrad:
            w4, stride, pad = tuple(op.wd4().shape), 1, op.K - 1 - op.pad
        else:
            w4, stride, pad = op.w4, op.stride, op.pad
        if not ops.conv_h2_supported(tuple(x_shape), w4, stride, pad):
            return False
        d = ops.conv_desc(tuple(x_shape), w4, stride, pad)
        return d.B * d.Ho * d.Wo * d.Cout >= self.H2_MIN_OUT

    def _plan_h2(self):
        o, k = self.ops, self.kind
        if not (self.use_h2 and self.fused):
            return None
        xs = tuple(self.x_in.shape)
        if k == "layer":
            op = o["layer"]
            if (op.tc_phase is not None and op.tc_phase.stride == 2 and xs[-1] % 16 == 0 and ops.conv_h2_supported(xs, op.wp4, 1, op.tc_phase.pad)
                    and ops.wgrad_h2_supported(xs, op.wp4, 1, op.tc_phase.pad) and xs[0] * xs[1] * xs[2] * op.wp4[0] >= self.H2_MIN_OUT):
                return "tconv"
            if (self.layer_h2 and op.tconv is None and not op.is_gdn and op.qm.kind == "conv" and op.K > 1 and xs[-1] % 16 == 0
                    and "dpre" in self.t and self._conv_ok_h2(op, xs) and ops.wgrad_h2_layer_supported(xs, op.w4, op.stride, op.pad)):
                return "layer"
            return None
        if k == "rb" and "skip" not in o:
            c1, c2 = o["conv1"], o["conv2"]
            hs = tuple(self.t["h1"].shape)
            if (self._conv_ok_h2(c1, xs) and self._conv_ok_h2(c2, hs) and self._conv_ok_h2(c2, hs, dgrad=True)
                    and ops.wgrad_h2_supported(xs, c1.w4, c1.stride, c1.pad) and ops.wgrad_h2_supported(hs, c2.w4, 1, c2.pad)):
                return "rb"
        if k in ("rbws", "rbu"):
            cv, g = (o["conv2"], o["gdn"]) if k == "rbws" else (o["conv"], o["igdn"])
            hs = tuple(self.t["h1"].shape)
            if (hs[-1] % 16 == 0 and (k != "rbu" or self.r == 2) and self._conv_ok_h2(cv, hs) and self._conv_ok_h2(cv, hs, dgrad=True)
                    and ops.wgrad_h2_supported(hs, cv.w4, 1, cv.pad)):
                return k
        return None

    def _forms(self, plan, widest=False):
        o, t = self.ops, self.t
        lean = PLANES if self.h2_lean else BOTH
        if plan == "layer":
            return {"x": PLANES, "dpre": PLANES}
        if plan == "tconv":
            return {"x": PLANES, "dyp": PLANES}
        if plan == "rb":
            c2 = o["conv2"]
            one = self.fuse_h2_tail and ops.conv_h2_tail_supported(tuple(t["h1"].shape), c2.w4, c2.stride, c2.pad)
            return {"x": lean, "h1": lean, "pre2": ABSENT if one else F32, "dpre2": PLANES, "dh1": PLANES}
        rbu = plan == "rbu"
        xs, hs = tuple(self.x_in.shape), tuple(t["h1"].shape)
        first, g = ((o["subpel_conv"], o["upsample"]), o["igdn"]) if rbu else ((o["conv1"],), o["gdn"])
        x_h2 = widest or (xs[-1] % 16 == 0 and all(self._conv_ok_h2(c, xs) and ops.wgrad_h2_supported(xs, c.w4, c.stride, c.pad) for c in first))
        g_h2 = widest or (self._conv_ok_h2(g, hs, dgrad=True) and not self._gdn_lin_ok(g, t["h1"]))
        f = {"x": BOTH if x_h2 else F32, "h1": lean if (rbu or x_h2) else BOTH, "t": BOTH if g_h2 else F32, "dc" if rbu else "dc2": PLANES}
        if rbu:
            f.update(dup=PLANES if x_h2 else F32, dsp=PLANES if x_h2 else F32)
        else:
            f["dh1"] = PLANES if x_h2 else F32
        return f

    def _fb_layer(self):
        op, t = self.ops["layer"], self.t
        x, dpre = self._act("x"), self._act("dpre")
        self._gather(x)
        if op.is_gdn:
            x = x.f32
            if self.fused:
                self._gdn_pool(op, x, t["norm"])
                self._tail_gdn(x, t["norm"], None, op.inverse, t["dy"], t["t"])
            else:
                self._conv(op, x, t["y"], epilogue=L.EPI_IGDN if op.inverse else L.EPI_GDN, aux=x, pre=t["norm"], square=True)
                self._loss(t["y"], t["dy"])
                ops.gdn_bwd_t(t["dy"], x, t["norm"], op.inverse, t["t"])
            self._wgrad(op, x, t["t"], square=True)
            return
        if op.tconv is not None and op.tc_phase is None:
            s_, q_, Hu, Wu = self.tc_geom
            x = _act_of(ops.zero_insert(x.f32, s_, q_, q_, Hu, Wu, out=t["xu"]))
        epi = op.qm.fused_epilogue() if self.include_act else None
        if epi is None and self.include_act and type(op.qm.activation_function).__name__ != "StraightThrough":
            raise NotImplementedError("calibration engine: only LeakyReLU(0.01) or ReLU may be fused into a layer unit")
        act = {None: ops.ACT_NONE, L.EPI_LRELU: ops.ACT_LRELU, L.EPI_RELU: ops.ACT_RELU}[epi]
        phase = op.tc_phase is not None
        if self._unit1x1_ok(op, x):
            if op.slabs is None:
                op.slabs = self._buf(ops.unit1x1_nslab(math.prod(x.shape[:-1]), op.w4[0]), *op.w4)
            self._task_is_rec = True
            ops.unit1x1(x.f32, op.wq4(), op.bias, self.co, self.idx, self.it, 2.0, act, self.loss_log, op.slabs)
        elif self.fused and phase:
            self._tconv_forward(op, x, t["y"])
            self._tail_act(t["y"], None, act, t["dpre"])
            self._tconv_wgrad(op, x, t["dpre"])
        elif self.fused:
            self._conv_tail(op, x, t["y"], None, act, dpre)
            self._wgrad(op, x, dpre)
        else:
            if phase:
                self._tconv_forward(op, x, t["y"], epilogue=L.EPI_NONE if epi is None else epi)
            else:
                self._conv(op, x, t["y"], epilogue=L.EPI_NONE if epi is None else epi)
            self._loss(t["y"], t["dy"])
            g = t["dy"]
            if epi is not None:
                (ops.lrelu_bwd if epi == L.EPI_LRELU else ops.relu_bwd)(t["dy"], t["y"], t["dpre"])
                g = t["dpre"]
            (self._tconv_wgrad if phase else self._wgrad)(op, x, g)

    def _fb_rb(self):
        o, t = self.ops, self.t
        c1, c2, skip = o["conv1"], o["conv2"], o.get("skip")
        x, h1, dpre2, dh1 = self._act("x"), self._act("h1"), self._act("dpre2"), self._act("dh1")
        self._gather(x)
        self._conv(c1, x, h1, epilogue=L.EPI_LRELU)
        res = x
        if skip is not None:
            self._conv(skip, x, t["sk"])
            res = t["sk"]
        if self.fused:
            self._conv_tail(c2, h1, self._act("pre2"), res, ops.ACT_LRELU, dpre2, gout=t["dout"] if skip is not None else None)
        else:
            self._conv(c2, h1, t["out"], epilogue=L.EPI_LRELU, residual=res, pre=t["pre2"])
            self._loss(t["out"], t["dout"])
            ops.lrelu_bwd(t["dout"], t["pre2"], t["dpre2"])
        if skip is not None:
            self._wgrad(skip, x, t["dout"])
        self._wgrad(c2, h1, dpre2)
        self._dgrad(c2, dpre2, dh1, epilogue=L.EPI_LRELU_BWD, aux=h1)
        self._split_point()
        self._wgrad(c1, x, dh1)

    def _fb_gdn_block(self):
        o, t = self.ops, self.t
        rbu = self.kind == "rbu"
        if rbu:
            first, cv, g, side, r = o["subpel_conv"], o["conv"], o["igdn"], o["upsample"], self.r
        else:
            first, cv, g, side = o["conv1"], o["conv2"], o["gdn"], o.get("skip")
        h1, dc, tt, x = self._act("h1"), self._act("dc" if rbu else "dc2"), self._act("t"), self._act("x")
        c = t["c" if rbu else "c2"]
        side_first = self.h2_plan is not None
        self._gather(x)
        if rbu:
            self._conv(first, x, t["sp"], epilogue=L.EPI_LRELU)
            if side_first:
                self._conv(side, x, t["up"])
            self._shuffle(t["sp"], r, h1)
            if side_first:
                self._shuffle(t["up"], r, t["ups"])
            self._conv(cv, h1, c)
            if not side_first:
                self._conv(side, x, t["up"])
                self._shuffle(t["up"], r, t["ups"])
            res = t["ups"]
        else:
            self._conv(first, x, h1, epilogue=L.EPI_LRELU)
            if side is not None and side_first:
                self._conv(side, x.f32, t["sk"])
            self._conv(cv, h1, c)
            if side is not None and not side_first:
                self._conv(side, x.f32, t["sk"])
            res = x if side is None else t["sk"]
        if self.fused:
            self._gdn_pool(g, c, t["norm"])
            self._tail_gdn(c, t["norm"], res, rbu, t["dout"], tt)
        else:
            self._conv(g, c, t["out"], epilogue=L.EPI_IGDN if rbu else L.EPI_GDN, aux=c, residual=res, pre=t["norm"], square=True)
            self._loss(t["out"], t["dout"])
        if rbu:
            dup = self._act("dup")
            self._unshuffle(t["dout"], r, dup)
            self._wgrad(side, x, dup)
        elif side is not None:
            self._wgrad(side, x.f32, t["dout"])
        if not self.fused:
            ops.gdn_bwd_t(t["dout"], c, t["norm"], rbu, tt.f32)
        self._gdn_acc(g, tt, t["acc"])
        if dc.planes is not None or c.numel() % 4 == 0:
            ops.gdn_bwd_dx_h2(t["dout"], c, t["norm"], t["acc"], rbu, dx=dc.f32, dx_planes=dc.planes)
        else:
            ops.gdn_bwd_dx(t["dout"], c, t["norm"], t["acc"], rbu, dc.f32)
        self._wgrad(g, c, tt.f32, square=True)
        self._wgrad(cv, h1, dc)
        dh1 = self._act("dh1")
        self._dgrad(cv, dc, dh1, epilogue=L.EPI_LRELU_BWD, aux=h1)
        if rbu:
            dsp = self._act("dsp")
            self._unshuffle(dh1, r, dsp)
            self._split_point()
            self._wgrad(first, x, dsp)
        else:
            self._split_point()
            self._wgrad(first, x, dh1)

    def _probe_amax(self, names):
        saved = ops.set_tuning("conv_x6", 0)
        self._probing = True
        try:
            self._forward_backward()
        finally:
            self._probing = False
            ops.set_tuning("conv_x6", saved)
        return torch.stack([(self.x_in if n == "x" else self.t[n]).abs().max() for n in names]).cpu()

    def _set_weights(self, soft):
        for op in self.ops.values():
            ops.adaround_fwd(op.desc, op.w, op.alpha, op.delta, op.zp, bool(soft), op.wq, op.wd)
            if op.tc_phase is not None:
                op.expand_phase()

    def _probe_scales(self):
        plan = self._plan_h2()
        if plan is None:
            return
        names = [self.PLANES_AS.get(n, n) for n, f in self._forms(plan, widest=True).items() if f & PLANES]
        amax = self._probe_amax(names)
        self._set_weights(soft=False)
        try:
            amax = torch.maximum(amax, self._probe_amax(names))
        finally:
            self._set_weights(soft=True)
        self._clear_probe()
        if self.world > 1:
            a = amax.to(self.dev)
            a = torch.where(torch.isfinite(a), a, torch.full_like(a, float("inf")))
            torch.distributed.all_reduce(a, op=torch.distributed.ReduceOp.MAX, group=self.group)
            amax = a.cpu()
        if not torch.isfinite(amax).all():
            raise RuntimeError("calibration engine: non-finite activations in the probe iteration")
        if bool((amax <= 0).any()):
            import logging
            logging.getLogger("rdo_ptq.engine").warning(
                "unit with an all-zero tensor in both probe iterations (%s): no fp16 plane scale can be derived, running it on fp32 activations",
                [n for n, a in zip(names, amax) if float(a) <= 0])
            self.use_h2 = False
            return
        self._amax = {n: float(a) for n, a in zip(names, amax)}
        self.scales = {n: ops.pow2_scale(a) for n, a in self._amax.items()}

    def _clear_probe(self):
        self.loss_log.zero_(); self.task_log.zero_(); self.round_log.zero_(); self._it2.zero_()
        for op in self.ops.values():
            op.slabs = None

    H2_POLL = int(os.environ.get("RDO_H2_POLL", 512))

    H2_RESTARTS = 2

    def _overflowed(self):
        if not self.P:
            return False
        v = self._ovf.clone()
        if self.world > 1:
            torch.distributed.all_reduce(v, op=torch.distributed.ReduceOp.MAX, group=self.group)
        self._ovf_seen = v.cpu().tolist()
        return any(self._ovf_seen)

    def _recover(self):
        import logging
        lg = logging.getLogger("rdo_ptq.engine")
        seen = self._ovf_seen
        self.h2_restarts += 1
        grown = {}
        for name, k in self._ovf_slot.items():
            if seen[2 * k]:
                grown[name] = ops.overflow_magnitude(seen[2 * k]) / self.scales[name] / self._amax[name]
        if self.h2_restarts <= self.H2_RESTARTS and grown and not (seen[0] or seen[1]):
            r = max(grown.values())
            for name, k in self._ovf_slot.items():
                if name in grown or seen[2 * k + 1]:
                    self._amax[name] *= 8.0 * grown.get(name, r)
            self.scales = {n: ops.pow2_scale(a) for n, a in self._amax.items()}
            lg.warning("calibration unit outgrew the fp16 range of its H2 planes within %d iterations (%s): restarting it with scales %s",
                       self._done, {n: f"x{g:.3g}" for n, g in grown.items()}, self.scales)
        else:
            self.use_h2 = False
            lg.warning("calibration unit left the fp16 range of its H2 planes%s: restarting it on fp32 activations",
                       " again" if self.h2_restarts > 1 else " with non-finite values")
        for op in self.ops.values():
            ops.adaround_init_alpha(op.desc, op.w, op.delta, op.alpha)
            op.m.zero_(); op.v.zero_()
            op.wq_planes = op.wd_planes = op.wp_h2 = op.wp_planes = op.lin_fwd = op.lin_bwd = None
        self._set_weights(soft=True)
        self.P, self._ovf_slot = {}, {}
        self._clear_probe()
        self._ovf.zero_()
        self._done = 0
        self._ovf_checked = -1
        self._dp_graph = self._rd_graph = None
        self._record()
        for op in self.ops.values():
            op.refresh_planes()
        self._prime()

    def _check_overflow(self):
        self.dp_drain()
        if self._ovf_checked == self._done:
            return
        while self._overflowed():
            if not self.use_h2:
                raise RuntimeError("calibration engine: an H2 overflow word is raised on the fp32-activation path (library fault)")
            target = self._done
            with ops.h2_flag(self._ovf[0:2]):
                self._recover()
            self.run(target)
            torch.cuda.synchronize()
        self._ovf_checked = self._done

    def sync_overflow(self):
        self._check_overflow()

    def _forward_backward(self):
        self.h2_plan = None if self._probing else self._plan_h2()
        self.forms = {} if self.h2_plan is None else self._forms(self.h2_plan)
        {"layer": self._fb_layer, "rb": self._fb_rb, "rbws": self._fb_gdn_block, "rbu": self._fb_gdn_block}[self.kind]()

    def _items(self, opl):
        return [dict(d=op.desc, w=op.w, delta=op.delta, zp=op.zp, slabs=op.slabs, alpha=op.alpha, m=op.m, v=op.v, wq=op.wq, wd=op.wd,
                     wq_planes=op.wq_planes, wd_planes=op.wd_planes, dalpha=getattr(op, "dalpha", None),
                     lin_fwd=op.lin_fwd, lin_bwd=op.lin_bwd) for op in opl]

    STEP_BATCH = 8

    def _batchable(self, opl):
        return self.batch_step and len(opl) >= 1 and all(op.numel() % 4 == 0 for op in opl)

    def _step_batches(self, opl, scale, mode):
        for i in range(0, len(opl), self.STEP_BATCH):
            last = i + self.STEP_BATCH >= len(opl)
            if self._folded:
                it, kw = self.it_shadow, dict(iter_shadow=self.it if last else None, gather=self._next_gather if last else None)
            elif self._handover:
                it, kw = self.it, dict(iter_shadow=self.it_shadow if i == 0 else None)
            else:
                it, kw = self.it, dict(advance_iter=self.it if last else None)
            ops.adaround_step_batch(self._items(opl[i:i + self.STEP_BATCH]), scale, self.weight, self.sched, it, self.round_log, mode=mode, **kw)

    @property
    def _handover(self):
        return self.fold_iter and self._batchable(list(self.ops.values()))

    @property
    def _folded(self):
        return self.fold_gather and self._handover and self.rd is None

    def _it_src(self):
        return self.it_shadow if (self._handover and not self._folded) else self.it

    def _it_pub(self):
        return self.it if (self._handover and not self._folded) else None

    def _gather(self, x):
        x = _act_of(x)
        g = dict(cache_q=self.cq, cache_fp=self.cf, idx_table=self.idx, B=self.B, batch_offset=self.batch_offset,
                 prob=self.input_prob, seed=self.seed, out=x.f32, out_planes=x.planes)
        if self._folded and not self._probing:
            self._next_gather = g
        else:
            self._gather_now(g, self._it_src(), self._it_pub())

    def _gather_now(self, g, it, publish=None):
        if g["out_planes"] is not None:
            ops.gather_qdrop_h2(self.cq, self.cf, self.idx, it, self.B, self.input_prob, self.seed, g["out"], g["out_planes"], self.batch_offset,
                                iter_publish=publish)
        else:
            ops.gather_qdrop(self.cq, self.cf, self.idx, it, self.B, self.input_prob, self.seed, g["out"], self.batch_offset, iter_publish=publish)

    def _prime(self):
        if self._next_gather is not None:
            self.it_shadow.copy_(self.it)
            self._gather_now(self._next_gather, self.it)

    def _grad_ops(self, names):
        opl = [self.ops[n] for n in names]
        if self._batchable(opl):
            for i in range(0, len(opl), self.STEP_BATCH):
                ops.adaround_step_batch(self._items(opl[i:i + self.STEP_BATCH]), 1.0, self.weight, self.sched, self.it, self.round_log, mode=1)
            return
        for op in opl:
            ops.adaround_grad(op.desc, op.w, op.alpha, op.delta, op.zp, op.slabs, op.dalpha)

    def _step_ops(self, apply=False):
        opl = list(self.ops.values())
        scale = self.bucket.scale if apply else 1.0
        if self._batchable(opl):
            self._step_batches(opl, scale, 2 if apply else 0)
            self._after_step(lin_done=True)
            return
        for op in opl:
            (ops.adaround_apply if apply else ops.adaround_step)(
                op.desc, op.w, op.delta, op.zp, op.dalpha if apply else op.slabs, scale, self.weight, self.sched, self.it,
                op.alpha, op.m, op.v, op.wq, op.wd, self.round_log, op.wq_planes, op.wd_planes)
        ops.iter_advance(self.it)
        self._after_step()

    def _next_plan(self):
        self._rec_ctx.__exit__(None, None, None)
        plan = Plan()
        self._rec_ctx = plan.record()
        self._rec_ctx.__enter__()
        return plan

    def _split_point(self):
        if self._probing or self._late is None or self.plan_a2 is not None:
            return
        self._grad_ops([n for n in self.ops if n != self._late])
        self.plan_a2 = self._next_plan()

    def _record(self):
        self.plan_a = Plan()
        self.plan_a2 = self.plan_b = self.plan_rd = None
        self._rec_ctx = self.plan_a.record()
        self._rec_ctx.__enter__()
        self._next_gather = None
        try:
            if self._folded:
                ops.iter_bind_publish(self.it_shadow)
            self._forward_backward()
            if self._folded and (ops.iter_bind_publish(None) or self._next_gather is None):
                raise RuntimeError("calibration engine: the folded gather needs exactly one loss / tail launch and one gather per iteration")
            if not self.split:
                self._step_ops()
            elif self.plan_a2 is not None:
                self._grad_ops([self._late])
            else:
                self._grad_ops(list(self.ops))
        finally:
            ops.iter_bind_publish(None)
            self._rec_ctx.__exit__(None, None, None)
            self._rec_ctx = None
        if self.split:
            self.plan_b = Plan()
            with self.plan_b.record():
                self._step_ops(apply=True)

    def run(self, n_iters=None, idle=None):
        done = self._done
        n = self.iters - done if n_iters is None else int(n_iters)
        if n < 0 or done + n > self.iters:
            raise ValueError(f"cannot run {n} iterations: {done} of {self.iters} already done")
        target = done + n
        with ops.h2_flag(self._ovf[0:2]):
            while self._done < target:
                k = target - self._done
                if self.P and self.H2_POLL > 0:
                    k = min(k, self.H2_POLL)
                if not (self.P and self.H2_POLL > 0) and idle is not None:
                    k = min(k, max(64, (target - done) // 16))
                if self.plan_rd is not None:
                    self._run_rd(k)
                elif not self.split:
                    self.plan_a.run(k, graph=self.use_graph)
                else:
                    self._run_dp(k)
                self._done += k
                if idle is not None:
                    idle()
                if self._done < target and self.P and self.H2_POLL > 0:
                    self.dp_drain()
                if self._done < target and self._overflowed():
                    self._recover()
        return n

    def prepare(self, n_iters=None):
        if self.use_graph and not self.split and self.plan_rd is None:
            n = self.iters - self._done if n_iters is None else int(n_iters)
            k = min(n, self.H2_POLL) if (self.P and self.H2_POLL > 0) else n
            self.plan_a.prepare(k)
            if n % k:
                self.plan_a.prepare(n % k)

    def _dp_iteration(self, graph, first=True, last=True):
        if first:
            self.plan_a.run(1, graph=graph)
        self.bucket.reduce(between=None if self.plan_a2 is None else (lambda: self.plan_a2.run(1, graph=graph)))
        if last:
            self.plan_b.run(1, graph=graph)
        else:
            self.plan_b.run_then(self.plan_a, graph=graph)

    DP_GRAPH_BACKENDS = ("nccl",)
    DP_HB_BATCH = 32
    DP_STALL_S = float(os.environ.get("RDO_DP_STALL_S", 120))

    def _dp_capture(self):
        if self._hb_dev is None:
            self._hb_dev = torch.zeros(1, dtype=torch.int64, device=self.dev)
            self._hb_host = torch.zeros(1, dtype=torch.int64).pin_memory()
        g = torch.cuda.CUDAGraph()
        with torch.cuda.graph(g):
            self._dp_iteration(False)
            self._hb_dev.add_(1)
            self._hb_host.copy_(self._hb_dev, non_blocking=True)
        return g

    def _hb_wait(self, target):
        import time
        if self._hb_host is None or target <= 0:
            return
        seen, t_last = int(self._hb_host[0]), time.monotonic()
        while seen < target:
            time.sleep(0.0005)
            now = int(self._hb_host[0])
            if now != seen:
                seen, t_last = now, time.monotonic()
            elif time.monotonic() - t_last > self.DP_STALL_S:
                raise DpStallError(f"rank {self._rank()}: the captured data-parallel loop made no progress for {self.DP_STALL_S:.0f} s "
                                   f"({seen} of {self._hb_issued} replays completed) -- a collective inside the graph hangs")

    def dp_drain(self):
        if self._dp_graph is not None:
            self._hb_wait(self._hb_issued)

    def _run_dp(self, n):
        import logging
        dist = torch.distributed
        comm = self.world > 1 or (dist.is_available() and dist.is_initialized())
        want = (self.use_graph and os.environ.get("RDO_DP_GRAPH", "1") == "1" and comm
                and dist.get_backend(self.group) in self.DP_GRAPH_BACKENDS)
        if want and self._dp_graph is None and not self._dp_graph_failed and n > 1:
            self._dp_iteration(False)
            n -= 1
            ok, g = 1, None
            try:
                g = self._dp_capture()
            except Exception as e:
                logging.warning("rank %s: data-parallel iteration could not be captured into a graph (%s)", self._rank(), e)
                ok = 0
                torch.cuda.synchronize()
            if comm:
                flag = torch.tensor([ok], device=self.dev, dtype=torch.int32)
                dist.all_reduce(flag, op=dist.ReduceOp.MIN, group=self.group)
                ok = int(flag.item())
            if ok:
                self._dp_graph, self._hb_issued = g, 0
                self._hb_dev.zero_()
                self._hb_host.zero_()
            else:
                self._dp_graph_failed = True
                self.dp_fallbacks += 1
                del g
        path = "graph" if self._dp_graph is not None else "host"
        if self.dp_path != path:
            self.dp_path = path
            logging.getLogger("rdo_ptq.dp").info("rank %s: data-parallel loop = %s (world %d)", self._rank(), path, self.world)
        if self._dp_graph is not None:
            for _ in range(n):
                self._dp_graph.replay()
                self._hb_issued += 1
                if self._hb_issued % self.DP_HB_BATCH == 0:
                    self._hb_wait(self._hb_issued - self.DP_HB_BATCH)
            return
        merge = self.use_graph and os.environ.get("RDO_DP_MERGE", "1") != "0"
        for i in range(n):
            self._dp_iteration(self.use_graph, first=(i == 0 or not merge), last=(i == n - 1 or not merge))

    def _rank(self):
        dist = torch.distributed
        return dist.get_rank(self.group) if (dist.is_available() and dist.is_initialized()) else 0

    def _rd_iteration(self, graph):
        self.plan_a.run(1, graph=graph)
        self._rd_tail()
        self.plan_rd.run(1, graph=graph)
        if self.split:
            self.bucket.reduce()
            self.plan_b.run(1, graph=graph)
# ... 238 lines not shown
```

Measured before the change: 20470.

## Fuse conv weight-gradient MFMA into AdaRound step kernel for single-conv layers

Adds a kernel that computes the conv weight gradient tile with MFMA 32x32x2 f32 into shared memory and feeds it straight into the AdaRound/Adam step, skipping the separate wgrad launch and its slab round-trip through global memory. Gather blocks for the next iteration now wait on an atomic counter, so they only start after all step blocks have consumed their inputs. The path is enabled by default for fused, unsplit layer-kind conv units. In exchange it adds a spin-wait inter-block dependency and limits the split count per tile, which may reduce parallelism for large M.

```diff
diff --git a/include/rdo_ptq_hip.h b/include/rdo_ptq_hip.h
--- a/include/rdo_ptq_hip.h
+++ b/include/rdo_ptq_hip.h
@@ -119,6 +119,13 @@
                                    const rdo_sched_row* sched, const int32_t* iter_ptr, float* round_loss_out, int32_t* iter_shadow,
                                    const rdo_gather_desc* next, void* stream);
 int rdo_iter_bind_publish(int32_t* publish);
+
+int rdo_wgrad_adaround_step_supported(const rdo_conv_desc* d);
+int rdo_wgrad_adaround_step(const rdo_conv_desc* d, const float* x, const float* dy, const rdo_ada_step_item* item, float grad_scale,
+                            float round_weight, const rdo_sched_row* sched, const int32_t* iter_ptr, float* round_loss_out,
+                            int32_t* advance_iter, int32_t* iter_shadow, const rdo_gather_desc* next ,
+                            int32_t* sync ,
+                            void* stream);
 
 int rdo_unit1x1_supported(int64_t M, int32_t K, int32_t N);
 int rdo_unit1x1_nslab(int64_t M, int32_t N);
diff --git a/rdo-ptq_amd/csrc/adaround.hip b/rdo-ptq_amd/csrc/adaround.hip
--- a/rdo-ptq_amd/csrc/adaround.hip
+++ b/rdo-ptq_amd/csrc/adaround.hip
@@ -286,64 +286,97 @@
 }
 
 
-__device__ __forceinline__ void ada_step_tile_body(const AdaArgs& a, int bid) {
+struct TileLoads {
+    int it;
+    rdo_sched_row sc;
+    float dl, z;
+    f32x4 w4, al4, m4, v4;
+};
+struct TilePos {
+    int ct, tap, rt, q, r, row, ci;
+    bool live;
+    long e0;
+};
+__device__ __forceinline__ TilePos ada_tile_pos(const rdo_ada_desc& d, int bid) {
+    TilePos p;
+    const int taps = d.KH * d.KW, ctiles = (d.Cin + 31) >> 5;
+    p.ct = bid % ctiles; bid /= ctiles;
+    p.tap = bid % taps;
+    p.rt = bid / taps;
+    p.q = threadIdx.x & 7; p.r = threadIdx.x >> 3;
+    p.row = p.rt * 32 + p.r; p.ci = p.ct * 32 + 4 * p.q;
+    p.live = p.row < d.rows && p.ci < d.Cin;
+    p.e0 = ((long)p.row * taps + p.tap) * d.Cin + p.ci;
+    return p;
+}
+__device__ __forceinline__ TileLoads ada_tile_loads(const AdaArgs& a, int bid) {
+    const TilePos p = ada_tile_pos(a.d, bid);
+    TileLoads L;
+    L.it = *a.iter_ptr;
+    L.sc = a.sched[L.it];
+    L.dl = L.z = 0.f;
+    L.w4 = L.al4 = L.m4 = L.v4 = f32x4{0.f, 0.f, 0.f, 0.f};
+    if (p.live) {
+        L.w4 = *reinterpret_cast<const f32x4*>(a.w + p.e0);
+        L.al4 = *reinterpret_cast<const f32x4*>(a.alpha + p.e0);
+        if (!ADA_ABL(8)) {
+            L.m4 = *reinterpret_cast<const f32x4*>(a.m + p.e0);
+            L.v4 = *reinterpret_cast<const f32x4*>(a.v + p.e0);
+        }
+        L.dl = a.delta[p.row]; L.z = a.zp[p.row];
+    }
+    return L;
+}
+
+template <class Slab>
+__device__ __forceinline__ void ada_tile_step(const AdaArgs& a, int bid, const TileLoads& L, Slab slab) {
     typedef float vec_t __attribute__((ext_vector_type(4)));
     typedef unsigned u32x2 __attribute__((ext_vector_type(2)));
     typedef unsigned short u16x4 __attribute__((ext_vector_type(4)));
     const rdo_ada_desc d = a.d;
     const int Cin = d.Cin, taps = d.KH * d.KW, nrows = d.rows;
-    const int ctiles = (Cin + 31) >> 5;
     const int bid0 = bid;
-    const int ct = bid % ctiles; bid /= ctiles;
-    const int tap = bid % taps;
-    const int rt = bid / taps;
-    const int q = threadIdx.x & 7, r = threadIdx.x >> 3;
-    const int row = rt * 32 + r, ci = ct * 32 + 4 * q;
-    const bool live = row < nrows && ci < Cin;
+    const TilePos p = ada_tile_pos(d, bid);
+    const int ct = p.ct, tap = p.tap, rt = p.rt, q = p.q, r = p.r, row = p.row, ci = p.ci;
+    const bool live = p.live;
     const float Lm1 = (float)(d.n_levels - 1);
-    const int it = *a.iter_ptr;
-    const rdo_sched_row sc = a.sched[it];
-    const float b = sc.b, round_on = sc.round_on, step_size = sc.step_size, bc2 = sc.bc2_sqrt;
+    const int it = L.it;
+    const float b = L.sc.b, round_on = L.sc.round_on, step_size = L.sc.step_size, bc2 = L.sc.bc2_sqrt;
     float rl_local = 0.f;
     vec_t o4 = {0.f, 0.f, 0.f, 0.f};
-    const long e0 = ((long)row * taps + tap) * Cin + ci;
+    const long e0 = p.e0;
     if (live) {
-        const vec_t wv4 = *reinterpret_cast<const vec_t*>(a.w + e0);
-        vec_t al4 = *reinterpret_cast<const vec_t*>(a.alpha + e0);
+        const vec_t wv4 = L.w4;
+        vec_t al4 = L.al4;
         vec_t g4 = {0.f, 0.f, 0.f, 0.f};
         if (a.mode == 2) {
             g4 = *reinterpret_cast<const vec_t*>(a.dalpha_in + e0);
         } else if (!ADA_ABL(1)) {
-            const float* sp = a.slabs + e0;
             int s = 0;
             for (; s + 16 <= a.nsplit; s += 16) {
                 vec_t t[16];
 #pragma unroll
-                for (int u = 0; u < 16; ++u) t[u] = *reinterpret_cast<const vec_t*>(sp + (long)(s + u) * d.numel);
+                for (int u = 0; u < 16; ++u) t[u] = slab(s + u);
                 g4 += (((t[0] + t[1]) + (t[2] + t[3])) + ((t[4] + t[5]) + (t[6] + t[7]))) +
                       (((t[8] + t[9]) + (t[10] + t[11])) + ((t[12] + t[13]) + (t[14] + t[15])));
             }
             for (; s + 8 <= a.nsplit; s += 8) {
                 vec_t t[8];
 #pragma unroll
-                for (int u = 0; u < 8; ++u) t[u] = *reinterpret_cast<const vec_t*>(sp + (long)(s + u) * d.numel);
+                for (int u = 0; u < 8; ++u) t[u] = slab(s + u);
                 g4 += ((t[0] + t[1]) + (t[2] + t[3])) + ((t[4] + t[5]) + (t[6] + t[7]));
             }
             if (s + 4 <= a.nsplit) {
                 vec_t t[4];
 #pragma unroll
-                for (int u = 0; u < 4; ++u) t[u] = *reinterpret_cast<const vec_t*>(sp + (long)(s + u) * d.numel);
+                for (int u = 0; u < 4; ++u) t[u] = slab(s + u);
                 g4 += (t[0] + t[1]) + (t[2] + t[3]);
                 s += 4;
             }
-            for (; s < a.nsplit; ++s) g4 += *reinterpret_cast<const vec_t*>(sp + (long)s * d.numel);
-        }
-        vec_t m4 = {0.f, 0.f, 0.f, 0.f}, v4 = m4;
-        if (!ADA_ABL(8)) {
-            m4 = *reinterpret_cast<const vec_t*>(a.m + e0);
-            v4 = *reinterpret_cast<const vec_t*>(a.v + e0);
-        }
-        const float dl = a.delta[row], z = a.zp[row];
+            for (; s < a.nsplit; ++s) g4 += slab(s);
+        }
+        vec_t m4 = L.m4, v4 = L.v4;
+        const float dl = L.dl, z = L.z;
 #pragma unroll
         for (int k = 0; k < 4; ++k) {
             float al = al4[k];
@@ -496,6 +529,13 @@
     }
 }
 
+__device__ __forceinline__ void ada_step_tile_body(const AdaArgs& a, int bid) {
+    const TilePos p = ada_tile_pos(a.d, bid);
+    const float* sp = a.slabs + p.e0;
+    const long numel = a.d.numel;
+    ada_tile_step(a, bid, ada_tile_loads(a, bid), [sp, numel](int s) { return *reinterpret_cast<const f32x4*>(sp + (long)s * numel); });
+}
+
 inline bool tile_ok(const rdo_ada_desc& d, int mode) {
     return mode != 1 && d.Cin > 0 && d.Cin % 4 == 0 && d.rows % 4 == 0 && (long)d.rows * d.KH * d.KW * d.Cin == d.numel && d.numel < (1L << 31);
 }
@@ -517,14 +557,17 @@
     int gather_beg;
     rdo::gq::Gather g;
 };
+__device__ __forceinline__ void next_gather_blocks(const rdo::gq::Gather& g, const int32_t* iter_ptr, int gather_beg) {
+    const int it1 = *iter_ptr + 1;
+    if (it1 < g.n_iters) {
+        if (g.planes.p) rdo::gq::gather_h2_body(g, it1, (long)blockIdx.x - gather_beg, (long)gridDim.x - gather_beg);
+        else rdo::gq::gather_fp32_body(g, it1, (long)blockIdx.x - gather_beg, (long)gridDim.x - gather_beg);
+    }
+}
 __global__ __launch_bounds__(256) void ada_step_batch_kernel(AdaBatch b) {
     if (b.iter_shadow && blockIdx.x == 0 && threadIdx.x == 0) *b.iter_shadow = *b.a[0].iter_ptr + 1;
     if ((int)blockIdx.x >= b.gather_beg) {
-        const int it1 = *b.a[0].iter_ptr + 1;
-        if (it1 < b.g.n_iters) {
-            if (b.g.planes.p) rdo::gq::gather_h2_body(b.g, it1, (long)blockIdx.x - b.gather_beg, (long)gridDim.x - b.gather_beg);
-            else rdo::gq::gather_fp32_body(b.g, it1, (long)blockIdx.x - b.gather_beg, (long)gridDim.x - b.gather_beg);
-        }
+        next_gather_blocks(b.g, b.a[0].iter_ptr, b.gather_beg);
         return;
     }
     int t = 0;
@@ -533,6 +576,102 @@
     if (b.tile[t]) { ada_step_tile_body(b.a[t], (int)blockIdx.x - beg); return; }
     if (b.a[t].nsplit >= b.w1_min && b.a[t].mode != 2) ada_step_body<1>(b.a[t], (long)blockIdx.x - beg, (long)b.blk_end[t] - beg);
     else ada_step_body<4>(b.a[t], (long)blockIdx.x - beg, (long)b.blk_end[t] - beg);
+}
+
+struct WgStep {
+    AdaArgs a;
+    const float* x;
+    const float* dy;
+    int B, H, W, Ho, Wo, stride, pad, M, mchunk;
+    int32_t* iter_shadow;
+    int gather_beg;
+    int32_t* sync;
+    rdo::gq::Gather g;
+};
+constexpr int kWgStepMaxSplit = 8;
+__global__ __launch_bounds__(256) void wgrad_step_kernel(WgStep p) {
+    typedef float f32x16 __attribute__((ext_vector_type(16)));
+    if (p.iter_shadow && blockIdx.x == 0 && threadIdx.x == 0) *p.iter_shadow = *p.a.iter_ptr + 1;
+    if ((int)blockIdx.x >= p.gather_beg) {
+        if (*p.a.iter_ptr + 1 < p.g.n_iters) {
+            if (threadIdx.x == 0) {
+                while (__hip_atomic_load(p.sync, __ATOMIC_RELAXED, __HIP_MEMORY_SCOPE_AGENT) < p.gather_beg) __builtin_amdgcn_s_sleep(32);
+                const int ngather = (int)gridDim.x - p.gather_beg;
+                if (__hip_atomic_fetch_add(p.sync + 1, 1, __ATOMIC_RELAXED, __HIP_MEMORY_SCOPE_AGENT) == ngather - 1) {
+                    __hip_atomic_store(p.sync, 0, __ATOMIC_RELAXED, __HIP_MEMORY_SCOPE_AGENT);
+                    __hip_atomic_store(p.sync + 1, 0, __ATOMIC_RELAXED, __HIP_MEMORY_SCOPE_AGENT);
+                }
+            }
+            __syncthreads();
+            next_gather_blocks(p.g, p.a.iter_ptr, p.gather_beg);
+        }
+        return;
+    }
+    extern __shared__ float gs[];
+    const AdaArgs& a = p.a;
+    const int bid = blockIdx.x;
+    const TileLoads L = ada_tile_loads(a, bid);
+    const TilePos tp = ada_tile_pos(a.d, bid);
+    const int lane = threadIdx.x & 63, wave = threadIdx.x >> 6, li = lane & 31, lh = lane >> 5;
+    const int Cin = a.d.Cin, Cout = a.d.rows;
+    const int kh = tp.tap / a.d.KW, kw = tp.tap - kh * a.d.KW;
+    const int HoWo = p.Ho * p.Wo;
+    const float* dyp = p.dy + tp.rt * 32 + li;
+    const float* xp = p.x + tp.ct * 32 + li;
+    for (int c = wave; c < a.nsplit; c += 4) {
+        const int mbeg = c * p.mchunk;
+        const int mend = min(p.M, mbeg + p.mchunk);
+        const int nsteps = mend > mbeg ? (mend - mbeg + 31) >> 5 : 0;
+        f32x16 acc;
+#pragma unroll
+        for (int r = 0; r < 16; ++r) acc[r] = 0.f;
+        float fa0[16], fb0[16], fa1[16], fb1[16];
+        auto load = [&](int s, float (&fa)[16], float (&fb)[16]) {
+            const int m = mbeg + 32 * s + li;
+            int xo = -1;
+            if (m < mend) {
+                const int b = m / HoWo;
+                const int rem = m - b * HoWo;
+                const int ho = rem / p.Wo, wo = rem - ho * p.Wo;
+                const int hi = ho * p.stride - p.pad + kh, wi = wo * p.stride - p.pad + kw;
+                if ((unsigned)hi < (unsigned)p.H && (unsigned)wi < (unsigned)p.W) xo = ((b * p.H + hi) * p.W + wi) * Cin;
+            }
+            const int m0 = mbeg + 32 * s + lh;
+#pragma unroll
+            for (int k = 0; k < 16; ++k) {
+                const int mk = m0 + 2 * k;
+                const int xk = __shfl(xo, 2 * k + lh, 64);
+                const bool oky = mk < mend, okx = xk >= 0;
+                const float yv = dyp[oky ? mk * Cout : 0];
+                const float xv = xp[okx ? xk : 0];
+                fa[k] = oky ? yv : 0.f;
+                fb[k] = okx ? xv : 0.f;
+            }
+        };
+        auto mfma = [&](const float (&fa)[16], const float (&fb)[16]) {
+#pragma unroll
+            for (int k = 0; k < 16; ++k) acc = __builtin_amdgcn_mfma_f32_32x32x2f32(fa[k], fb[k], acc, 0, 0, 0);
+        };
+        if (nsteps > 0) load(0, fa0, fb0);
+        for (int s = 0; s < nsteps; s += 2) {
+            if (s + 1 < nsteps) load(s + 1, fa1, fb1);
+            mfma(fa0, fb0);
+            if (s + 1 < nsteps) {
+                if (s + 2 < nsteps) load(s + 2, fa0, fb0);
+                mfma(fa1, fb1);
+            }
+        }
+        float* g = gs + (long)c * (32 * 33) + li;
+#pragma unroll
+        for (int r = 0; r < 16; ++r) g[((r & 3) + 8 * (r >> 2) + 4 * lh) * 33] = acc[r];
+    }
+    __syncthreads();
+    if (p.sync && threadIdx.x == 0 && L.it + 1 < p.g.n_iters) __hip_atomic_fetch_add(p.sync, 1, __ATOMIC_RELAXED, __HIP_MEMORY_SCOPE_AGENT);
+    const float* gt = gs + tp.r * 33 + 4 * tp.q;
+    ada_tile_step(a, bid, L, [gt](int s) {
+        const float* t = gt + s * (32 * 33);
+        return f32x4{t[0], t[1], t[2], t[3]};
+    });
 }
 
 __device__ __forceinline__ void wd_transpose_body(const rdo_ada_desc& d, const float* wq, float* wd, unsigned short* wd_planes, float pscale,
@@ -684,6 +823,9 @@
 
 }
 
+bool rdo_wgrad_is_generic64(const rdo_conv_desc* d);
+int rdo_wgrad_mchunk(long M, int nsplit);
+
 extern "C" {
 
 #ifdef RDO_DIAG
@@ -767,6 +909,28 @@
     a.wd_planes = wd ? static_cast<unsigned short*>(wd_planes) : nullptr;
     a.wq_pscale = wq_plane_scale; a.wd_pscale = wd_plane_scale; a.ovf = rdo::h2_overflow_flag();
     return run_step(a, stream);
+}
+
+static int make_gather(const rdo_gather_desc* next, rdo::gq::Gather& g, int& blocks, double& bytes) {
+    RDO_REQUIRE(next->cache_q && next->cache_fp && next->idx_table && (next->out || next->out_planes) && next->n_iters > 0,
+                "rdo_adaround_step_batch_gather: null pointer in the gather descriptor");
+    RDO_REQUIRE(next->B > 0 && next->batch_offset >= 0 && next->per_image > 0 && next->per_image % 4 == 0 &&
+                (long)(next->batch_offset + next->B) * next->per_image < (1L << 32), "rdo_adaround_step_batch_gather: bad gather shape");
+    RDO_REQUIRE(!next->out_planes || (next->C > 0 && next->C % 16 == 0 && next->per_image % next->C == 0 && next->out_scale > 0.f),
+                "rdo_adaround_step_batch_gather: the plane form needs C %% 16 == 0 and a positive power-of-two scale");
+    RDO_REQUIRE(next->out_planes || next->out, "rdo_adaround_step_batch_gather: no destination");
+    RDO_REQUIRE(next->prob >= 0.f && next->prob <= 1.f, "rdo_adaround_step_batch_gather: prob out of [0,1]");
+    const double t = floor((double)next->prob * 4294967296.0);
+    const unsigned long long thr = (unsigned long long)(t > 4294967296.0 ? 4294967296.0 : t);
+    g = rdo::gq::Gather{next->cache_q, next->cache_fp, next->idx_table, next->n_iters, next->B, next->batch_offset, (long)next->per_image,
+                        next->C, thr, next->seed, next->out,
+                        rdo::gq::H2Out{static_cast<unsigned short*>(next->out_planes), next->out_scale,
+                                       next->overflow_flag ? reinterpret_cast<int*>(next->overflow_flag) : rdo::h2_overflow_flag()}};
+    const long gb = rdo::gq::gather_blocks(g);
+    const long cap = g.planes.p ? 8192 : 2048;
+    blocks += (int)(gb > cap ? cap : gb);
+    bytes += (8.0 + (next->out ? 4.0 : 0.0) + (next->out_planes ? 4.0 : 0.0)) * next->B * (double)next->per_image;
+    return RDO_OK;
 }
 
 static int step_batch_impl(const rdo_ada_step_item* items, int32_t n, int32_t mode, float grad_scale, float round_weight,
@@ -820,24 +984,7 @@
     b.gather_beg = blocks;
     if (next) {
         RDO_REQUIRE(mode != 1 && iter_ptr, "rdo_adaround_step_batch_gather: the gather rides on a fused step or an apply launch");
-        RDO_REQUIRE(next->cache_q && next->cache_fp && next->idx_table && (next->out || next->out_planes) && next->n_iters > 0,
-                    "rdo_adaround_step_batch_gather: null pointer in the gather descriptor");
-        RDO_REQUIRE(next->B > 0 && next->batch_offset >= 0 && next->per_image > 0 && next->per_image % 4 == 0 &&
-                    (long)(next->batch_offset + next->B) * next->per_image < (1L << 32), "rdo_adaround_step_batch_gather: bad gather shape");
-        RDO_REQUIRE(!next->out_planes || (next->C > 0 && next->C % 16 == 0 && next->per_image % next->C == 0 && next->out_scale > 0.f),
-                    "rdo_adaround_step_batch_gather: the plane form needs C %% 16 == 0 and a positive power-of-two scale");
-        RDO_REQUIRE(next->out_planes || next->out, "rdo_adaround_step_batch_gather: no destination");
-        RDO_REQUIRE(next->prob >= 0.f && next->prob <= 1.f, "rdo_adaround_step_batch_gather: prob out of [0,1]");
-        const double t = floor((double)next->prob * 4294967296.0);
-        const unsigned long long thr = (unsigned long long)(t > 4294967296.0 ? 4294967296.0 : t);
-        b.g = rdo::gq::Gather{next->cache_q, next->cache_fp, next->idx_table, next->n_iters, next->B, next->batch_offset, (long)next->per_image,
-                              next->C, thr, next->seed, next->out,
-                              rdo::gq::H2Out{static_cast<unsigned short*>(next->out_planes), next->out_scale,
-                                             next->overflow_flag ? reinterpret_cast<int*>(next->overflow_flag) : rdo::h2_overflow_flag()}};
-        long gb = rdo::gq::gather_blocks(b.g);
-        const long cap = b.g.planes.p ? 8192 : 2048;
-        blocks += (int)(gb > cap ? cap : gb);
-        bytes += (8.0 + (next->out ? 4.0 : 0.0) + (next->out_planes ? 4.0 : 0.0)) * next->B * (double)next->per_image;
+        if (int rc = make_gather(next, b.g, blocks, bytes)) return rc;
     }
     const char* tag = next ? "ada_step_gather" : "ada_step";
     return rdo::dispatch(
@@ -863,6 +1010,64 @@
                                    const rdo_gather_desc* next, void* stream) {
     RDO_REQUIRE(next != nullptr, "rdo_adaround_step_batch_gather: null gather descriptor");
     return step_batch_impl(items, n, mode, grad_scale, round_weight, sched, iter_ptr, round_loss_out, nullptr, iter_shadow, next, stream);
+}
+
+int rdo_wgrad_adaround_step_supported(const rdo_conv_desc* d) {
+    if (!d || d->B <= 0 || d->H <= 0 || d->W <= 0 || d->Ho <= 0 || d->Wo <= 0 || d->Cin <= 0 || d->Cout <= 0 || d->KH <= 0 || d->KW <= 0) return 0;
+    if (d->Cin % 32 != 0 || d->Cout % 32 != 0 || d->square_input) return 0;
+    if ((long)d->B * d->H * d->W * d->Cin >= (1L << 31) || (long)d->B * d->Ho * d->Wo * d->Cout >= (1L << 31) ||
+        (long)d->Cout * d->KH * d->KW * d->Cin >= (1L << 31))
+        return 0;
+    return rdo_wgrad_is_generic64(d) && rdo_conv2d_wgrad_nsplit(d) <= kWgStepMaxSplit;
+}
+
+int rdo_wgrad_adaround_step(const rdo_conv_desc* d, const float* x, const float* dy, const rdo_ada_step_item* item, float grad_scale,
+                            float round_weight, const rdo_sched_row* sched, const int32_t* iter_ptr, float* round_loss_out,
+                            int32_t* advance_iter, int32_t* iter_shadow, const rdo_gather_desc* next, int32_t* sync, void* stream) {
+    RDO_REQUIRE(d && x && dy && item && sched && iter_ptr, "rdo_wgrad_adaround_step: null argument");
+    RDO_REQUIRE(!next || sync, "rdo_wgrad_adaround_step: the gather form needs the two sync words");
+    RDO_REQUIRE(rdo_wgrad_adaround_step_supported(d), "rdo_wgrad_adaround_step: shape not supported (rdo_wgrad_adaround_step_supported)");
+    RDO_REQUIRE(!(advance_iter && iter_shadow), "rdo_wgrad_adaround_step: advance_iter and iter_shadow are alternatives");
+    RDO_REQUIRE(!(next && advance_iter), "rdo_wgrad_adaround_step: the gather form moves the counter by hand-over (iter_shadow)");
+    const rdo_ada_step_item& it = *item;
+    if (int rc = check_desc(&it.d, "rdo_wgrad_adaround_step")) return rc;
+    RDO_REQUIRE(it.d.rows == d->Cout && it.d.KH == d->KH && it.d.KW == d->KW && it.d.Cin == d->Cin && !it.d.reparam,
+                "rdo_wgrad_adaround_step: the weight [%d][%d][%d][%d] is not this conv's", it.d.rows, it.d.KH, it.d.KW, it.d.Cin);
+    RDO_REQUIRE(it.w && it.delta && it.zp && it.alpha && it.adam_m && it.adam_v && it.wq, "rdo_wgrad_adaround_step: null pointer in the item");
+    WgStep p{};
+    AdaArgs& a = p.a;
+    a.d = it.d; a.w = it.w; a.delta = it.delta; a.zp = it.zp; a.slabs = nullptr;
+    a.nsplit = rdo_conv2d_wgrad_nsplit(d);
+    a.grad_scale = grad_scale; a.round_weight = round_weight; a.sched = sched; a.iter_ptr = iter_ptr;
+    a.alpha = it.alpha; a.m = it.adam_m; a.v = it.adam_v; a.wq = it.wq; a.wd = it.wd; a.round_loss_out = round_loss_out; a.mode = 0;
+    a.wq_planes = static_cast<unsigned short*>(it.wq_planes);
+    a.wd_planes = it.wd ? static_cast<unsigned short*>(it.wd_planes) : nullptr;
+    a.wq_pscale = it.wq_plane_scale; a.wd_pscale = it.wd_plane_scale; a.ovf = rdo::h2_overflow_flag();
+    if (it.lin_fwd_planes || it.lin_bwd_planes) {
+        RDO_REQUIRE(it.lin_plane_scale > 0.f, "rdo_wgrad_adaround_step: Linear planes need a positive scale");
+        a.lin_fwd = static_cast<unsigned short*>(it.lin_fwd_planes);
+        a.lin_bwd = static_cast<unsigned short*>(it.lin_bwd_planes);
+        a.lin_pscale = it.lin_plane_scale;
+    }
+    p.x = x; p.dy = dy;
+    p.B = d->B; p.H = d->H; p.W = d->W; p.Ho = d->Ho; p.Wo = d->Wo; p.stride = d->stride; p.pad = d->pad;
+    p.M = d->B * d->Ho * d->Wo;
+    p.mchunk = rdo_wgrad_mchunk(p.M, a.nsplit);
+    p.iter_shadow = iter_shadow;
+    p.sync = next ? sync : nullptr;
+    int blocks = (int)tile_blocks(it.d);
+    p.gather_beg = blocks;
+    double bytes = 4.0 * ((double)d->B * d->H * d->W * d->Cin + (double)p.M * d->Cout) + 36.0 * it.d.numel;
+    if (next)
+        if (int rc = make_gather(next, p.g, blocks, bytes)) return rc;
+    const size_t lds = (size_t)a.nsplit * 32 * 33 * sizeof(float);
+    return rdo::dispatch(
+        [=](hipStream_t s) {
+            hipLaunchKernelGGL(wgrad_step_kernel, dim3((unsigned)blocks), dim3(256), lds, s, p);
+            if (advance_iter) hipLaunchKernelGGL(iter_advance1_kernel, dim3(1), dim3(1), 0, s, advance_iter);
+            return rdo::check_launch("wgrad_step");
+        },
+        stream, next ? "wgrad_step_gather" : "wgrad_step", 2.0 * p.M * (double)it.d.numel, bytes);
 }
 
 int rdo_adaround_grad(const rdo_ada_desc* d, const float* w, const float* alpha, const float* delta, const float* zp,
diff --git a/rdo-ptq_amd/csrc/conv_wgrad.hip b/rdo-ptq_amd/csrc/conv_wgrad.hip
--- a/rdo-ptq_amd/csrc/conv_wgrad.hip
+++ b/rdo-ptq_amd/csrc/conv_wgrad.hip
@@ -260,6 +260,25 @@
     return (int)ns;
 }
 
+enum WgPath { WG_THINCOUT, WG_THIN, WG_LINEAR_H2, WG_X6, WG_FP32_192, WG_FP32_64 };
+static WgPath wgrad_path(const rdo_conv_desc* d, const float* x, const float* dy, int nsplit, int mchunk, bool vec) {
+    const long M = (long)d->B * d->Ho * d->Wo;
+    if (g_force_big < 0 && rdo_conv_is_thincout(d, false) && nsplit == rdo_thincout_patches(d)) return WG_THINCOUT;
+    if (rdo_conv_is_thin(d, false)) return WG_THIN;
+    if (g_force_big != 0 && rdo_linear_wgrad_h2_ok(d, x, dy) && (long)nsplit * mchunk >= M) return WG_LINEAR_H2;
+    if (vec && rdo_conv2d_wgrad_uses_bf16x6(d)) return WG_X6;
+    return big_tiles(d) ? WG_FP32_192 : WG_FP32_64;
+}
+
+int rdo_wgrad_mchunk(long M, int nsplit) { return (int)(rdo::ceil_div(rdo::ceil_div(M, nsplit), PK) * PK); }
+
+bool rdo_wgrad_is_generic64(const rdo_conv_desc* d) {
+    if (!d || g_force_big >= 0 || g_force_ns >= 1) return false;
+    if (d->Cin % 4 != 0 || d->Cout % 4 != 0) return false;
+    const int ns = rdo_conv2d_wgrad_nsplit(d);
+    return wgrad_path(d, nullptr, nullptr, ns, rdo_wgrad_mchunk((long)d->B * d->Ho * d->Wo, ns), true) == WG_FP32_64;
+}
+
 extern "C" int rdo_conv2d_wgrad(const rdo_conv_desc* d, const float* x, const float* dy, float* slabs, int nsplit,
                                 void* stream) {
     RDO_REQUIRE(d && x && dy && slabs, "rdo_conv2d_wgrad: null argument");
@@ -272,38 +291,35 @@
     a.KH = d->KH; a.KW = d->KW; a.stride = d->stride; a.pad = d->pad;
     a.M = d->B * d->Ho * d->Wo;
     a.nsplit = nsplit;
-    a.mchunk = (int)(rdo::ceil_div(rdo::ceil_div(a.M, nsplit), PK) * PK);
+    a.mchunk = rdo_wgrad_mchunk(a.M, nsplit);
     a.square_input = d->square_input;
     a.tiles_co = a.tiles_ci = 0;
     const bool vec = (d->Cin % 4 == 0) && (d->Cout % 4 == 0) &&
                      ((reinterpret_cast<uintptr_t>(x) | reinterpret_cast<uintptr_t>(dy)) % 16 == 0);
-    const bool big = big_tiles(d);
-    if (g_force_big < 0 && rdo_conv_is_thincout(d, false) && nsplit == rdo_thincout_patches(d)) {
-        const rdo_conv_desc dd = *d;
+    const rdo_conv_desc dd = *d;
+    const int mchunk = a.mchunk;
+    switch (wgrad_path(d, x, dy, nsplit, a.mchunk, vec)) {
+    case WG_THINCOUT:
         return rdo::dispatch([=](hipStream_t s) { return rdo_launch_thincout_wgrad(&dd, x, dy, slabs, s); }, stream, "conv_thincout_wgrad",
                              2.0 * a.M * (double)a.Cout * a.Cin * 9.0,
                              4.0 * ((double)a.B * a.H * a.W * a.Cin + (double)a.M * a.Cout + (double)nsplit * a.Cout * 9.0 * a.Cin));
-    }
-    if (rdo_conv_is_thin(d, false)) {
-        const rdo_conv_desc dd = *d;
+    case WG_THIN:
         return rdo::dispatch([=](hipStream_t s) { return rdo_launch_thin_wgrad(&dd, x, dy, slabs, nsplit, s); }, stream,
                              "conv_thin_wgrad", 2.0 * a.M * (double)a.Cout * a.Cin * a.KH * a.KW,
                              4.0 * ((double)a.B * a.H * a.W * a.Cin + (double)a.M * a.Cout + (double)nsplit * a.Cout * a.KH * a.KW * a.Cin));
-    }
-    if (g_force_big != 0 && rdo_linear_wgrad_h2_ok(d, x, dy) && (long)nsplit * a.mchunk >= a.M) {
-        const rdo_conv_desc dd = *d;
-        const int mchunk = a.mchunk;
+    case WG_LINEAR_H2:
         return rdo::dispatch([=](hipStream_t s) { return rdo_launch_linear_wgrad_h2(&dd, x, dy, slabs, nsplit, mchunk, s); }, stream,
                              "linear_wgrad_h2", 2.0 * a.M * (double)a.Cout * a.Cin,
                              4.0 * ((double)a.M * a.Cin + (double)a.M * a.Cout + (double)nsplit * a.Cout * a.Cin));
-    }
-    if (vec && rdo_conv2d_wgrad_uses_bf16x6(d)) {
-        const rdo_conv_desc dd = *d;
-        const int mchunk = a.mchunk;
+    case WG_X6:
         return rdo::dispatch([=](hipStream_t s) { return rdo_launch_wgrad_x6(&dd, x, dy, slabs, nsplit, mchunk, s); }, stream,
                              "conv_wgrad_x6_192x192", 2.0 * a.M * (double)a.Cout * a.Cin * a.KH * a.KW,
                              4.0 * ((double)a.B * a.H * a.W * a.Cin + (double)a.M * a.Cout + (double)nsplit * a.Cout * a.KH * a.KW * a.Cin));
-    }
+    case WG_FP32_192:
+    case WG_FP32_64:
+        break;
+    }
+    const bool big = big_tiles(d);
     return rdo::dispatch(
         [a, vec, big](hipStream_t s) {
             if (big) return vec ? launch<192, 192, true>(a, s) : launch<192, 192, false>(a, s);
diff --git a/rdo-ptq_amd/hipops/_lib.py b/rdo-ptq_amd/hipops/_lib.py
--- a/rdo-ptq_amd/hipops/_lib.py
+++ b/rdo-ptq_amd/hipops/_lib.py
@@ -64,6 +64,8 @@
     "rdo_adaround_step_batch": (C.c_int, [C.POINTER(AdaStepItem), C.c_int32, C.c_int32, C.c_float, C.c_float, P, P, P, P, P, P]),
     "rdo_adaround_step_batch_gather": (C.c_int, [C.POINTER(AdaStepItem), C.c_int32, C.c_int32, C.c_float, C.c_float, P, P, P, P, C.POINTER(GatherDesc), P]),
     "rdo_iter_bind_publish": (C.c_int, [P]),
+    "rdo_wgrad_adaround_step_supported": (C.c_int, [C.POINTER(ConvDesc)]),
+    "rdo_wgrad_adaround_step": (C.c_int, [C.POINTER(ConvDesc), P, P, C.POINTER(AdaStepItem), C.c_float, C.c_float, P, P, P, P, P, C.POINTER(GatherDesc), P, P]),
     "rdo_unit1x1_supported": (C.c_int, [C.c_int64, C.c_int32, C.c_int32]),
     "rdo_unit1x1_nslab": (C.c_int, [C.c_int64, C.c_int32]),
     "rdo_unit1x1_form": (C.c_int, [C.c_int32]),
diff --git a/rdo-ptq_amd/hipops/ops.py b/rdo-ptq_amd/hipops/ops.py
--- a/rdo-ptq_amd/hipops/ops.py
+++ b/rdo-ptq_amd/hipops/ops.py
@@ -226,14 +226,17 @@
     return bool(L.lib().rdo_iter_bind_publish(_ptr(word)))
 
 
-def adaround_step_batch(items, grad_scale, round_weight, sched, iter_ptr, round_log, advance_iter=None, mode=0, iter_shadow=None, gather=None):
-    _bind_out(None)
+def _dp(t):
+    return None if t is None else _ptr(t).value
+
+
+def _step_items(items):
     arr = (L.AdaStepItem * len(items))()
-    dp = lambda t: None if t is None else _ptr(t).value
+    dp = _dp
     for k, it in enumerate(items):
         a = arr[k]
         a.d = it["d"]
-        a.w, a.delta, a.zp, a.slabs = dp(it["w"]), dp(it["delta"]), dp(it["zp"]), dp(it["slabs"])
+        a.w, a.delta, a.zp, a.slabs = dp(it["w"]), dp(it["delta"]), dp(it["zp"]), dp(it.get("slabs"))
         a.nsplit = it["slabs"].shape[0] if it.get("slabs") is not None else 0
         a.alpha, a.adam_m, a.adam_v, a.wq, a.wd = dp(it["alpha"]), dp(it["m"]), dp(it["v"]), dp(it["wq"]), dp(it.get("wd"))
         a.wq_planes, a.wd_planes = dp(it.get("wq_planes")), dp(it.get("wd_planes"))
@@ -242,16 +245,43 @@
         lf, lb = it.get("lin_fwd"), it.get("lin_bwd")
         a.lin_fwd_planes, a.lin_bwd_planes = dp(lf), dp(lb)
         a.lin_plane_scale = float((lf if lf is not None else lb).scale) if (lf is not None or lb is not None) else 0.0
+    return arr
+
+
+def _gather_desc(gather):
+    dp = _dp
+    cq, pl = gather["cache_q"], gather.get("out_planes")
+    g = L.GatherDesc()
+    g.cache_q, g.cache_fp, g.idx_table = dp(cq), dp(gather["cache_fp"]), dp(gather["idx_table"])
+    g.n_iters, g.B, g.batch_offset = int(gather["idx_table"].shape[0]), int(gather["B"]), int(gather.get("batch_offset", 0))
+    g.per_image, g.C, g.prob, g.seed = cq[0].numel(), int(cq.shape[-1]), float(gather["prob"]), int(gather["seed"])
+    g.out, g.out_planes, g.out_scale = dp(gather.get("out")), dp(pl), (float(pl.scale) if pl is not None else 0.0)
+    g.overflow_flag = dp(getattr(pl, "flag", None))
+    return g
+
+
+def wgrad_step_supported(x_shape, w_shape, stride, pad, square_input=False):
+    d = conv_desc(x_shape, w_shape, stride, pad, square_input=square_input)
+    return bool(L.lib().rdo_wgrad_adaround_step_supported(C.byref(d)))
+
+
+def wgrad_adaround_step(x, dy, w_shape, stride, pad, item, grad_scale, round_weight, sched, iter_ptr, round_log, advance_iter=None,
+                        iter_shadow=None, gather=None, sync=None):
+    _bind_out(None)
+    d = conv_desc(x.shape, w_shape, stride, pad)
+    g = _gather_desc(gather) if gather is not None else None
+    L.check(L.lib().rdo_wgrad_adaround_step(C.byref(d), _ptr(x), _ptr(dy), _step_items([item]), grad_scale, round_weight, _ptr(sched), _ptr(iter_ptr),
+                                            _ptr(round_log), _ptr(advance_iter), _ptr(iter_shadow), C.byref(g) if g is not None else None, _ptr(sync), _stream()),
+            "rdo_wgrad_adaround_step")
+
+
+def adaround_step_batch(items, grad_scale, round_weight, sched, iter_ptr, round_log, advance_iter=None, mode=0, iter_shadow=None, gather=None):
+    _bind_out(None)
+    arr = _step_items(items)
     if gather is not None:
         if advance_iter is not None:
             raise ValueError("adaround_step_batch: the gather form moves the counter by hand-over (iter_shadow), not advance_iter")
-        cq, pl = gather["cache_q"], gather.get("out_planes")
-        g = L.GatherDesc()
-        g.cache_q, g.cache_fp, g.idx_table = dp(cq), dp(gather["cache_fp"]), dp(gather["idx_table"])
-        g.n_iters, g.B, g.batch_offset = int(gather["idx_table"].shape[0]), int(gather["B"]), int(gather.get("batch_offset", 0))
-        g.per_image, g.C, g.prob, g.seed = cq[0].numel(), int(cq.shape[-1]), float(gather["prob"]), int(gather["seed"])
-        g.out, g.out_planes, g.out_scale = dp(gather.get("out")), dp(pl), (float(pl.scale) if pl is not None else 0.0)
-        g.overflow_flag = dp(getattr(pl, "flag", None))
+        g = _gather_desc(gather)
         L.check(L.lib().rdo_adaround_step_batch_gather(arr, len(items), int(mode), grad_scale, round_weight, _ptr(sched), _ptr(iter_ptr),
                                                        _ptr(round_log), _ptr(iter_shadow), C.byref(g), _stream()), "rdo_adaround_step_batch_gather")
         return
diff --git a/rdo-ptq_amd/quantization/engine.py b/rdo-ptq_amd/quantization/engine.py
--- a/rdo-ptq_amd/quantization/engine.py
+++ b/rdo-ptq_amd/quantization/engine.py
@@ -242,6 +242,8 @@
         self.fold_iter = os.environ.get("RDO_FOLD_ITER", "1") != "0"
         self.fold_gather = os.environ.get("RDO_GATHER_IN_STEP", "1") != "0"
         self._next_gather = None
+        self._wg_sync = None
+        self._wgrad_step_of = None
         self.rd = rd
         if rd is not None:
             metric = rd.get("metric", "mse")
@@ -433,6 +435,16 @@
         M, K = math.prod(x.shape[:-1]), x.shape[-1]
         return (self.unit1x1 == 2 or M <= 4096 or K <= 96) and ops.unit1x1_supported(M, K, op.w4[0])
 
+    wgrad_step = os.environ.get("RDO_WGRAD_STEP", "1") != "0"
+
+    def _wgrad_step_ok(self, op, x, dpre):
+        x, dpre = _act_of(x), _act_of(dpre)
+        if not (self.wgrad_step and self.kind == "layer" and self.fused and not self.split and self.rd is None and not self._probing
+                and op.qm.kind == "conv" and not op.is_gdn and op.tconv is None and not self._unit1x1_ok(op, x)
+                and x.planes is None and dpre.planes is None and x.f32 is not None and dpre.f32 is not None and self._batchable([op])):
+            return False
+        return ops.wgrad_step_supported(tuple(x.shape), op.w4, op.stride, op.pad)
+
     def _conv(self, op, x, out, epilogue=L.EPI_NONE, aux=None, residual=None, pre=None, square=False, bias=True):
         x, out = _act_of(x), _act_of(out)
         b = (op.beta if op.is_gdn else op.bias) if bias else None
@@ -711,7 +723,10 @@
             self._tconv_wgrad(op, x, t["dpre"])
         elif self.fused:
             self._conv_tail(op, x, t["y"], None, act, dpre)
-            self._wgrad(op, x, dpre)
+            if self._wgrad_step_ok(op, x, dpre):
+                self._wgrad_step_of = (_f32(x), _f32(dpre))
+            else:
+                self._wgrad(op, x, dpre)
         else:
             if phase:
                 self._tconv_forward(op, x, t["y"], epilogue=L.EPI_NONE if epi is None else epi)
@@ -985,6 +1000,8 @@
 
     def _prime(self):
         if self._next_gather is not None:
+            if self._wg_sync is not None:
+                self._wg_sync.zero_()
             self.it_shadow.copy_(self.it)
             self._gather_now(self._next_gather, self.it)
 
@@ -1000,6 +1017,20 @@
     def _step_ops(self, apply=False):
         opl = list(self.ops.values())
         scale = self.bucket.scale if apply else 1.0
+        if self._wgrad_step_of is not None and not apply:
+            x, dy = self._wgrad_step_of
+            op, = opl
+            if self._folded:
+                if self._wg_sync is None:
+                    self._wg_sync = torch.zeros(2, dtype=torch.int32, device=self.dev)
+                it, kw = self.it_shadow, dict(iter_shadow=self.it, gather=self._next_gather, sync=self._wg_sync)
+            elif self._handover:
+                it, kw = self.it, dict(iter_shadow=self.it_shadow)
+            else:
+                it, kw = self.it, dict(advance_iter=self.it)
+            ops.wgrad_adaround_step(x, dy, op.w4, op.stride, op.pad, self._items(opl)[0], scale, self.weight, self.sched, it, self.round_log, **kw)
+            self._after_step(lin_done=True)
+            return
         if self._batchable(opl):
             self._step_batches(opl, scale, 2 if apply else 0)
             self._after_step(lin_done=True)
@@ -1030,6 +1061,7 @@
         self._rec_ctx = self.plan_a.record()
         self._rec_ctx.__enter__()
         self._next_gather = None
+        self._wgrad_step_of = None
         try:
             if self._folded:
                 ops.iter_bind_publish(self.it_shadow)
```

After: 19640. -4.0%, worse.
